# conanhujinming/flash_hash_join

Hardware: AMD Instinct MI355X
Metric: probe throughput (billion probes/sec), int64 keys, whole join (build + probe phases) per step (higher is better)
Workload: dtype int64

## Files before the change

flash_hash_join_amd/csrc/fj_host.h:

```cpp
#pragma once
#include "fj_internal.h"
#include "../../include/flashjoin.h"
#include "../../include/flashjoin_lab.h"

#include <algorithm>
#include <chrono>
#include <cstdarg>
#include <cstdio>
#include <cstdlib>
#include <cstring>
#include <condition_variable>
#include <functional>
#include <mutex>
#include <string>
#include <thread>
#include <vector>

struct StreamState;

namespace fjh {

int set_err(const char* fmt, ...);
fj_timings& last_timings();
#define HIPCHK(x)                                                                                          \
// ... 33 lines not shown
    u32 next_item;
    u32 next_emit_item;
    unsigned long long owner_counts[64], owner_cursors[64], owner_offsets[64];
    u32 pack_alloc, pack_seg, pack_err, rx_alloc;
    unsigned long long pack_used[64];
    unsigned long long pack_kept;
    u32 pack_xcd[8 * FJ_PF_COUNTERS];
    u32 bc_bounds[20];
};

enum Slot {
    W_POOL_K = 0, W_POOL_V, W_DIR, W_LIST, W_BCHUNKS, W_REL, W_BOFF, W_SEGOFF, W_TOFF, W_TILES, W_KINDS,
    W_SIDE_STRIDE = 2 * W_KINDS,
    W_PART_COUNT = 3 * W_SIDE_STRIDE, W_OUT_OFF, W_GT_KEYS, W_GT_VALS, W_GT_BLOOM, W_WG_COUNT,
    W_H_BK, W_H_BV, W_H_PK, W_H_OK, W_H_OV, W_ROWIDX, W_BKEYS, W_BBASE,
    W_PK_FI, W_PK_BKEYS, W_PK_OBASE,
    W_RX_REL, W_RX_LIST, W_RX_SEGOFF, W_RX_BCH, W_RX_BOFF, W_RX_TOFF, W_RX_TILES,
    W_SK_TILES_B, W_SK_TILES_P, W_SK_NT, W_PART_COUNT2, W_OUT_OFF2,
    W_MM_TILES,
    W_MM_PBITS,
    W_FULL_BITS,
    W_PAIR_WORDS,
    W_GR_PART, W_GR_BASE,
    W_NSLOTS
};

struct Buf { void* p = nullptr; size_t bytes = 0; };

enum Ev { E_START = 0, E_BUILD, E_PPART, E_JOIN, E_EMIT0, E_EMIT1, E_SB0, E_SB1, E_BF0, E_BF1, E_H0, E_H1, E_H2, E_PK0, E_NEV = E_PK0 + 8 };

struct BcastSources { const void* base = nullptr; int n = 0; uint64_t off[FJ_WIDE_MAXSRC] = {}, nkeys[FJ_WIDE_MAXSRC] = {}; };

struct Pending {
    enum Kind { LDS, HBM_TABLE, MANY, BCAST };
    bool valid = false;
    Kind kind = LDS;
    FjLdsJoinArgs lds{};
    FjGtArgs gt{};
    u32 nitems = 0, gt_grid = 0;
    u64 count = 0;
    bool has_second = false; FjLdsJoinArgs lds2{}; u32 nitems2 = 0; u64 count_main = 0; std::vector<u32> flagged;
    bool dups_main = false; std::vector<u32> sk_parts; int sk_bits = 0, sk_plan_bits = 0, sk_npass = 0;
    int mm_outer = 0; FjMmOuterArgs mm{}; u64 mm_P = 0, mm_u = 0, mm_r = 0;
    FjMmSweepArgs mm_sweep{}; u64 mm_u_main = 0; u64* mm_tile_off = nullptr; u64* mm_sweep_off = nullptr;
    bool mm_trivial = false; const u64* mm_pk = nullptr;
    bool has_dups = false;
    const u64* bk = nullptr; const u64* bv = nullptr; size_t nb = 0; int top_bits = 64;
    BcastSources src; const u32* toff = nullptr; size_t nb_total = 0;
};

struct SingleOut { u64* keys = nullptr; u64* vals = nullptr; size_t cap = 0; bool done = false; };

struct Plan { int bits = 0, npass = 0; int fan_log[4] = {0, 0, 0, 0}; int bloom_level = 0; };

struct Prepared {
    enum Form { EMPTY, LDS, HBM };
    bool valid = false;
    Form form = EMPTY;
    bool has_vals = false;
    int top_bits = 64, path = 0;
    Plan plan; u32 nparts = 0;
    size_t nb = 0; u64 g = 0;
    u64* keys = nullptr; u64* rows = nullptr; u64* vals = nullptr; void* aux = nullptr;
    u64 cap_mask = 0;
    size_t bytes = 0;
};

struct PassIter {
    int side = 0; bool has_vals = false; size_t n = 0; Plan plan; int used = 64; u32 parents = 1; u64 lbound = 0;
    u32 tile_chunks = 16; int i = 0;
    FjChunkSet prev{}; bool have_prev = false; const uint4* tiles = nullptr; const u32* ntiles = nullptr; const u32* toff = nullptr;
    FjChunkSet cs{}; u32 Gmax = 1, F = 1, appends = 1;
    size_t piece_rows = 0;
    int slot = 0, cs_base = 0;
    u32 item_tc_max = 0;
    bool want_items = false; u32 items_cap = 0; u32* part_count = nullptr; int part_count_slot = W_PART_COUNT;
    bool bloom_done = false; const FjChunkSet* bloom_build = nullptr;
    const u32* bloom_prebuilt = nullptr;
    unsigned long long* bloom_bucket_keys = nullptr;
    int save_level = 0; FjChunkSet saved{};
    u32* alloc_word = nullptr; u32* seg_word = nullptr; u32* err_word = nullptr;
    bool in_pk7 = false; u32 in_b0 = 0, in_top_shift = 0;
    bool vals_pos = false;
};

}

struct PackState {
    bool begun = false, deferred = false;
    u32 part_shift = 0;
    fjh::PassIter it;
    FjPackArgs args{};
    int nranks = 0;
};

struct StreamState {
    bool active = false;
    fjh::Plan plan; fjh::PassIter pit, bit; FjLdsJoinArgs ja{};
    int top_bits = 64, evc = 0;
    size_t np_bound = 0, np_seen = 0, nb_bound = 0, nb_seen = 0;
    u32 p_appends_left = 0, b_appends_left = 0;
    bool probe_done = false, build_done = false;
    const u64* flat_build = nullptr;
    const u64* flat_probe[64]; size_t flat_np[64]; u32 nflat = 0;
    std::vector<std::pair<const u64*, size_t>> bpieces, ppieces;
    bool shuffled = false; u32 b_lo = 0, nbk = 0, nbk_pad = 0;
    bool probe_prepared = true; u32 probe_appends = 0;
    bool with_vals = false;
};

struct BcastState {
    bool packed = false, probed = false;
    size_t nb_total = 0, nb = 0, np = 0;
    int pieces = 1, evc = 0;
    fjh::Plan plan; fjh::PassIter pit; FjLdsJoinArgs ja{};
    bool with_vals = false;
    fjh::BcastSources src;
};

struct fj_ctx {
    int device = 0;
    fjh::Buf bufs[fjh::W_NSLOTS];
    hipEvent_t ev[fjh::E_NEV];
    hipStream_t side = nullptr;
    fjh::Scalars* d_sc = nullptr;
    fjh::Scalars* h_sc = nullptr;
    fjh::Pending pend;
    fjh::Prepared prep;
    StreamState st;
    PackState pk;
    BcastState bc;
    hipEvent_t pk_ev = nullptr;
    unsigned long long* pk_h = nullptr;
    size_t ws_bytes = 0;
    u32 num_cus = 256;
    u32 reserve_cus = 0;
    void* stage[3] = {nullptr, nullptr, nullptr};
    size_t stage_bytes = 0;
    bool plan_in_flight = false;
    bool slot_dirty[fjh::W_NSLOTS] = {};
    std::recursive_mutex mu;
};

namespace fjh {

#define FJ_HOOK_LOOPBACK 1
#define FJ_HOOK_INJECT_FAIL 2
#define FJ_HOOK_SPLIT_ALWAYS 4
#define FJ_HOOK_ONE_COMM 8
#define FJ_HOOK_RESERVE_ALWAYS 16
#define FJ_HOOK_EMIT_TAGGED 32
#define FJ_HOOK_EMIT_RETRY_7TH 64
struct Options {
    size_t radix_threshold = 0; int scalar_hbm_table = 0; u32 persistent_min_items = 8192; u32 plan_target_keys = FJ_PART_TARGET_KEYS;
    int bloom_variant = 0, bloom_auto = 1, bloom_auto_max_hit_bp = 2300, mat_single_pass = 1;
    int join_wide = 2;
    u32 lab_hooks = 0;
    u32 join_items_target = 2048;
    int mm_heavy_keys = 0;
    int mm_heavy_outer = 0;
    Options();
};
Options& options();

int get_buf(fj_ctx* c, int slot, size_t bytes, void** out);
int get_zeroed_buf(fj_ctx* c, int slot, size_t bytes, void** out, hipStream_t s);
int plan_npass(int bits);
void plan_passes(Plan& p, bool extra_first);
Plan make_plan(size_t nb, int top_bits, bool want_bloom = false, u64 target_override = 0);
void pass_init(PassIter& it, int side, bool has_vals, size_t n, const Plan& plan, int top_bits);
u32 pass_groups(u64 chunks, u64 rows, u32 tile_chunks, u32 F);
int pass_prepare(fj_ctx* c, PassIter& it, u32 appends, hipStream_t s);
int pass_launch(fj_ctx* c, PassIter& it, const u64* keys, const u64* vals, size_t n, hipStream_t s, int* ev_cursor);
bool bloom_stage_follows(const PassIter& it, int level);
void join_item_geometry(u64 nparts, size_t np, u64 chunk_bound, u32* tc, u64* max_items);
bool wide_join_planned(bool materialize, size_t nb, size_t np_eff, int bits);
int level_finish(fj_ctx* c, PassIter& it, bool final_level, hipStream_t s);
int pass_complete(fj_ctx* c, PassIter& it, hipStream_t s);
int bloom_stage(fj_ctx* c, PassIter& it, hipStream_t s);
int run_passes(fj_ctx* c, PassIter& it, const u64* keys, const u64* vals, hipStream_t s, FjChunkSet* out, int* ev_cursor);
int clear_plan_scalars(fj_ctx* c, hipStream_t s);
void begin_plan(fj_ctx* c);
void end_plan(fj_ctx* c);
void drop_pending(fj_ctx* c);
int begin_step(fj_ctx* c, const char* who);
int read_scalars(fj_ctx* c, hipStream_t s);
float ev_ms(fj_ctx* c, int a, int b);
void plan_timings(fj_ctx* c, const Plan& plan, u64 partitions, int evc, fj_timings* t);
int pool_error();
int distinct_error();

enum ValueKind { KIND_UNSIGNED = 0, KIND_SIGNED = 1, KIND_FLOAT = 2 };
enum AggPlane { PLANE_COUNT = 0, PLANE_SUM = 1, PLANE_MIN = 2, PLANE_MAX = 3 };
u64 gt_capacity(size_t nb);
inline u32 gt_grid(u64 n) { const u64 rounds = (n + 1023) / 1024; return (u32)(rounds < 4096 ? (rounds ? rounds : 1) : 4096); }
int gt_open(fj_ctx* c, size_t nb, size_t val_words, hipStream_t s, FjGtArgs* a, u64** vals);
void gt_facts(fj_timings* t);
int gt_read(fj_ctx* c, hipStream_t s, fj_timings* t);
int gt_close(fj_ctx* c, hipStream_t s, fj_timings* t);
template <class F> int gt_fallback(fj_timings* t, F&& global_form) {
    fj_timings t2; memset(&t2, 0, sizeof t2); t2.sampled_hit_bp = -1;
    const int rc = global_form(&t2);
    t2.total_ms += t->total_ms; t2.fell_back = 1; *t = t2;
    return rc;
}
int kind_agg(int kind, int plane);

enum RelBeside { REL_KEYS_ONLY, REL_VALUES, REL_POSITIONS };
struct RelAttempt { Plan plan; FjChunkSet rel{}; u32 nparts = 0; };
int rel_open(fj_ctx* c, const u64* keys, RelBeside beside, const u64* vals, size_t n, int top_bits, u64 target, hipStream_t s,
             RelAttempt* r);
int rel_close(fj_ctx* c, const Plan& plan, u32 nparts, hipStream_t s, fj_timings* t);

int stamps_begin(unsigned long long** dbg, hipStream_t s);
int stamps_report(const char* label, const unsigned long long* dbg, u32 nitems, hipStream_t s);

int emit_pending(fj_ctx* c, u64* d_ok, u64* d_ov, size_t cap, hipStream_t s, fj_timings* t);
int radix_join_tail(fj_ctx* c, int materialize, FjLdsJoinArgs& ja, const Plan& plan, size_t np, const PassIter& pit, hipStream_t s,
                    fj_timings* t, int evc, u64* out_count, bool* lds_full, int top_bits, SingleOut* so = nullptr);

int join_outer(fj_ctx* c, int mode, bool use_radix, const u64* bk, const u64* bv, size_t nb, const u64* pk, size_t np, int top_bits,
               hipStream_t s, fj_timings* t, u64* out_count, u64* d_ok, u64* d_ov, bool rid = false);
int join_full(fj_ctx* c, bool use_radix, const u64* bk, const u64* bv, size_t nb, const u64* pk, size_t np, int top_bits,
              hipStream_t s, fj_timings* t, u64* out_counts, u64* d_ok, u64* d_ov, bool rid);

int join_probe_order(fj_ctx* c, bool use_radix, const u64* bk, const u64* bv, size_t nb, const u64* pk, size_t np, int top_bits,
                     hipStream_t s, fj_timings* t, u64* out_count, unsigned char* d_mask, u64* d_ov, bool rid);

void prepared_free(fj_ctx* c);
int prepared_retain(fj_ctx* c, bool use_radix, const u64* bk, const u64* bv, size_t nb, int top_bits, hipStream_t s, fj_timings* t);
int prepared_probe(fj_ctx* c, const u64* pk, size_t np, hipStream_t s, fj_timings* t, u64* out_count, unsigned char* d_mask, u64* d_ov, bool rid);
int prepared_group(fj_ctx* c, const u64* pk, const u64* pv, size_t np, hipStream_t s, fj_timings* t, u64* out_count, u64* d_cnt, u64* d_val,
                   int agg, bool accumulate);

int join_group(fj_ctx* c, bool use_radix, const u64* bk, size_t nb, const u64* pk, const u64* pv, size_t np, int top_bits,
               hipStream_t s, fj_timings* t, u64* out_count, u64* d_cnt, u64* d_sum, int agg);

int group_by(fj_ctx* c, bool use_radix, const u64* bk, const u64* bv, size_t nb, int top_bits, hipStream_t s, fj_timings* t,
             u64* out_count, u64* d_ok, u64* d_ov, size_t cap_out, int agg, bool rid, bool inv = false);
int group_by_all(fj_ctx* c, bool use_radix, const u64* bk, const u64* bv, size_t nb, int top_bits, hipStream_t s, fj_timings* t,
                 u64* out_count, u64* d_ok, u64* d_ov, size_t cap_out, int kind);
int group_by_arg(fj_ctx* c, bool use_radix, const u64* bk, const u64* bv, size_t nb, int top_bits, hipStream_t s, fj_timings* t,
                 u64* out_count, u64* d_ok, u64* d_ov, size_t cap_out, int kind, bool is_max);
int group_by_merge(fj_ctx* c, bool use_radix, const u64* bk, const u64* bv, size_t nb, int top_bits, hipStream_t s, fj_timings* t,
                   u64* out_count, u64* d_ok, u64* d_ov, size_t cap_out, int kind);

int group_by_pair(fj_ctx* c, bool use_radix, const u64* ka, const u64* kb, size_t nb, int top_bits, hipStream_t s, fj_timings* t,
                  u64* out_count, u64* d_ok, u64* d_ov, size_t cap_out);
int group_by_pair_agg(fj_ctx* c, bool use_radix, const u64* ka, const u64* kb, const u64* kv, size_t nb, int top_bits, hipStream_t s,
                      fj_timings* t, u64* out_count, u64* d_ok, u64* d_ov, size_t cap_out, int kind);

int group_rows(fj_ctx* c, bool use_radix, const u64* bk, size_t nb, int top_bits, hipStream_t s, fj_timings* t,
               u64* out_count, u64* d_ok, u64* d_ov, size_t cap_out);

int stream_open(fj_ctx* c, size_t nb_bound, int build_appends, size_t np_bound, int probe_appends, hipStream_t s, int top_bits,
                size_t probe_piece_rows = 0);
int stream_append_build(fj_ctx* c, const u64* d_bk, size_t n, hipStream_t s);
int stream_flush_build(fj_ctx* c, StreamState& st, hipStream_t s);
int stream_abort(fj_ctx* c);

int bcast_emit_launch(fj_ctx* c, const Pending& pd, u64* d_ok, u64* d_ov, hipStream_t s);
void drop_bcast_result_in(fj_ctx* c, const void* p, size_t bytes);

fj_ctx*& host_ctx();

}
```

flash_hash_join_amd/csrc/fj_internal.h:

```cpp
#pragma once
#include "fj_common.h"

#define FJ_ERR_POOL 1u
#define FJ_ERR_LDS_FULL 2u
#define FJ_STAT_DUPS 4u
#define FJ_STAT_RETRY 8u
#define FJ_STAT_EMIT_RETRY 16u
#define FJ_ERR_VARIANT 32u
#define FJ_BLOOM_HDR_MAGIC 0xB100F000u
#define FJ_STAT_TOOBIG 64u
#define FJ_ERR_OUTCAP 128u
#define FJ_ERR_PAIR_COLLISION 256u
#define FJ_ITEM_RETRY 0xFFFFFFFFu
#define FJ_ITEM_TOOBIG 0xFFFFFFFEu

struct FjPartArgs {
    const u64* in_keys;
    const u64* in_vals;
    const u32* in_list;
    const u32* in_dir;
    const uint4* in_tiles;
    const u32* in_ntiles;
    u64 n_flat;
    u32 parent0;
    u64* out_keys;
    u64* out_vals;
    u32* out_dir;
    u64* out_rel;
    u32* seg_off;
    u32* bchunks;
    u32* alloc;
    u32* seg_counter;
    u32 cap_chunks;
    u32 max_segs;
    u32* err;
    u32 shift;
    u32 fan_log;
    u32 side;
    u32 slab;
    u32 run_log;
    u32 in_pk7, in_b0, in_top_shift;
    u32 vals_pos;
};

struct FjChunkSet {
    u64* keys;
    u64* vals;
    u64 n_flat;
    u32* dir;
    u64* rel;
    u32* seg_off;
    u32* alloc;
    u32 cap;
    u32 nb;
    u32 fan_mask;
    u32 max_segs;
    u32* bchunks;
    u32* boff;
    u32* list;
    u32 run_log;
};

u32 fj_partition_lds_bytes(u32 fan_log, bool vals, int line_log);
u32 fj_partition_tile_chunks(u32 fan_log, bool vals);
hipError_t fj_launch_partition(const FjPartArgs& a, bool vals, int line_log, u32 grid, hipStream_t s);
hipError_t fj_launch_group(const FjChunkSet& cs, u32 tc, u32* toff, uint4* tiles, u32 max_tiles, u32* zero_tail, hipStream_t s);
hipError_t fj_launch_scan_u32_to_u64(const u32* in, u64* out, u32 n, hipStream_t s);
hipError_t fj_launch_dir_rank(u32* dir, u32 n, u32 b_lo, u32 nbk, u32 fan, u64* rel, u32* seg_off, u32* bchunks, u32* nalloc, hipStream_t s);

struct FjBloomArgs {
    const u64* pkeys;
    const u32* plist;
    const uint4* tiles;
    u64* out_keys; u32* out_dir; u64* out_rel;
    u32 cap_chunks;
    u32 pnb;
    const u32* toff;
    const u64* bkeys; const u32* blist; const u32* bboff;
    u32* seg_off; u32* bchunks; u32* alloc; u32* seg_counter;
    u32 max_segs;
    u32* err;
    unsigned long long* survivors;
    const u32* prebuilt;
    unsigned long long* bucket_keys;
};
u32 fj_bloom_tile_chunks();
u32 fj_bloom_waves_per_group();
u32 fj_bloom_slab_chunks();
hipError_t fj_launch_bloom_filter(const FjBloomArgs& a, u32 grid, int variant, hipStream_t s);
hipError_t fj_launch_bloom_export(const FjChunkSet& build, u32* out, u32 grid, int variant, hipStream_t s);
hipError_t fj_launch_flatten(const FjChunkSet& cs, const unsigned long long* bucket_keys, unsigned long long* base, u64* out, hipStream_t s);

struct FjPackArgs {
    const u64* keys; const u64* vals;
    const u32* list; const u32* boff;
    u32 nb, fan_log, nranks, wire7;
    uint4* fi;
    u32* fb;
    u32* bkeys;
    u32* obase;
    unsigned long long* used;
    unsigned char* dst_k[64]; u64* dst_v[64]; u32* dst_d[64];
};
hipError_t fj_launch_pack_plan(const FjPackArgs& a, hipStream_t s);
#define FJ_PF_COUNTERS 4u
#ifndef FJ_PFILT_BYTES
#define FJ_PFILT_BYTES 4096u
#endif
hipError_t fj_launch_part_filter_export(const FjChunkSet& build, u64* out, u32 grid, hipStream_t s);
hipError_t fj_launch_part_filter_inplace(const FjChunkSet& cs, const u64* filters, u32 part_shift, unsigned long long* kept, u32* next_of_xcd , u32 grid, hipStream_t s);
hipError_t fj_launch_part_filter_sample(const u64* raw, u64 n, u64 stride, const u64* filters, u32 part_shift, unsigned long long* kept, hipStream_t s);
hipError_t fj_launch_pack_squeeze(const FjPackArgs& a, u32 grid, hipStream_t s);


hipError_t fj_set_max_lds_once(const void* fn, u32 bytes);

struct FjLdsJoinArgs {
    FjChunkSet build, probe;
    u32 nparts;
    u32 nsplit;
    const uint4* items;
    const u32* nitems_dev;
    u32 items_cap;
    u32* part_count;
    unsigned long long* total;
    u32* err;
    const u64* out_off;
    u64* out_keys;
    u64* out_vals;
    unsigned long long* out_cursor;
    u64 out_capacity;
    u32 retry_only;
    u32 mark_toobig;
    u32 want_dups;
    u32 dedup;
    const u64* orig_vals;
    u32 avg_build_keys;
    unsigned long long* dbg;
    u32 dbg_flags;
    u32 row_ids;
};
hipError_t fj_launch_lds_join(const FjLdsJoinArgs& a, bool materialize, hipStream_t s, u32* next_item = nullptr,
                              u32 persistent_min_items = 8192);
hipError_t fj_launch_emit_single(const FjLdsJoinArgs& a, hipStream_t s, u32* next_item);
#define FJ_WIDE_MAXSRC 16u
struct FjWideArgs {
    const u32* toff; u32 part_lo, part_hi;
    const unsigned char* base; u32 nsrc, bits, mid_bytes;
    u32 group_log;
    u32 max_units;
    u32 pmask;
    u64 offs_off[FJ_WIDE_MAXSRC], lo_off[FJ_WIDE_MAXSRC], mid_off[FJ_WIDE_MAXSRC];
};
hipError_t fj_launch_count_join_wide(const FjLdsJoinArgs& a, const FjWideArgs& w, bool dense, u32 grid, hipStream_t s);
static inline u32 fj_wide_pmask(int bits, int top_bits) { return bits <= 0 ? 0u : (bits >= 32 ? 0xFFFFFFFFu : ((1u << bits) - 1u) << (top_bits - 32 - bits)); }

hipError_t fj_launch_lds_join_retry(const FjLdsJoinArgs& a, hipStream_t s);
hipError_t fj_launch_lds_emit_retry(const FjLdsJoinArgs& a, hipStream_t s, bool only_marked = true);

hipError_t fj_launch_sample_hits(const FjChunkSet& build, const u64* pk, u64 np, u32 nsamples, u32 shift32, u32 pmask,
                                 unsigned long long* hits, hipStream_t s);

#define FJ_MM_INNER 0
#define FJ_MM_LEFT 1
#define FJ_MM_FULL 2
struct FjMmOuterArgs {
    u32* miss_count;
    unsigned long long* miss_total;
    const u64* miss_off;
    u64 miss_base;
    u64* bits;
    unsigned long long* marked;
    u64* pbits;
};
hipError_t fj_launch_mm_join(const FjLdsJoinArgs& a, bool materialize, hipStream_t s, int outer = FJ_MM_INNER, const FjMmOuterArgs* oa = nullptr);
#define FJ_MM_TILE_CHUNKS 16u
hipError_t fj_launch_mm_tile_join(const FjLdsJoinArgs& a, bool materialize, hipStream_t s, int outer = FJ_MM_INNER, const FjMmOuterArgs* oa = nullptr);
struct FjMmSweepArgs {
    FjChunkSet probe;
    const uint4* items; u32 nitems;
    const u64* pbits;
    u32* miss_count;
    unsigned long long* miss_total;
    const u64* miss_off;
    u64 miss_base;
    u64* out_keys; u64* out_vals;
    u32 row_ids;
};
hipError_t fj_launch_mm_miss_sweep(const FjMmSweepArgs& w, bool materialize, hipStream_t s);

struct FjGtArgs {
    u64* tkeys; u64* tvals; u32* bloom;
    u64 cap_mask;
    u32* flags;
    u64* empty_val;
    const u64* bk; const u64* bv; u64 nb;
    const u64* pk; u64 np;
    u32* wg_count;
    unsigned long long* total;
    const u64* out_off;
    u64* out_keys; u64* out_vals;
    u32 row_ids;
    u32* matched;
};
hipError_t fj_launch_gt_build(const FjGtArgs& a, hipStream_t s);
hipError_t fj_launch_gt_probe(const FjGtArgs& a, bool materialize, u32 grid, hipStream_t s);

hipError_t fj_launch_owner_hist(const u64* keys, u64 n, u32 nranks, unsigned long long* counts, hipStream_t s);
hipError_t fj_launch_owner_scatter(const u64* keys, const u64* vals, u64 n, u32 nranks,
                                   const unsigned long long* offsets, unsigned long long* cursors,
                                   u64* out_keys, u64* out_vals, hipStream_t s);

hipError_t fj_launch_iota(u64* out, u64 n, hipStream_t s);
hipError_t fj_launch_gen_build(u64* keys, u64* vals, u64 first, u64 n, hipStream_t s);
hipError_t fj_launch_gen_probe(u64* keys, u64 first, u64 n, u64 build_total, u64 seed, u32 hit_bp,
                               unsigned long long* expected_hits, hipStream_t s);

__host__ __device__ inline u32 fj_owner_of_w1(u32 w1, u32 nranks) { return ((w1 >> 16) * nranks) >> 16; }

#define FJ_OJ_LEFT 0
#define FJ_OJ_ANTI 1
#define FJ_OJ_LEFT_FIRST 2
struct FjOjCursor { u32 hit, miss; u64 hit_base, miss_base; };
// ... 97 lines not shown
```

flash_hash_join_amd/csrc/fj_join.hip:

```cpp
#include "fj_lds_table_dev.h"

namespace {

constexpr u32 S = FJ_LDS_SLOTS;

struct JoinHdr {
    u32 cnt, has_empty, cursor, claimed, full, ovf;
    u32 pad[2];
    u64 empty_val;
    u64 pad2;
};

constexpr u32 NGRP = S / FJ_LDS_GROUP;
__device__ __forceinline__ void lds_groups(u64 key, u32& g1, u32& g2) {
    const u32 w = FJ_HW2(key);
    g1 = (w & (NGRP - 1)) * FJ_LDS_GROUP;
    g2 = ((w >> 11) & (NGRP - 1)) * FJ_LDS_GROUP;
}

__device__ __forceinline__ u32 lds_tag(u32 w2) { const u32 t = w2 >> 24; return t ? t : 1u; }
__device__ __forceinline__ u32 tag_zero_bytes(u32 t) {
    const u32 y = (t & 0x7F7F7F7Fu) + 0x7F7F7F7Fu;
    return ~(y | t | 0x7F7F7F7Fu);
}
// ... 41 lines not shown
        if (step == 1) { hdr->ovf = 1; g = g1; }
        if ((step & 31u) == 31u && *reinterpret_cast<volatile u32*>(&hdr->full)) return false;
        g = (g + 1) & (NGRP - 1);
    }
    hdr->full = 1;
    return false;
}



template <bool MAT, int NK>
__device__ __forceinline__ void lds_probe(const u64* __restrict__ tkeys, const u32* __restrict__ ttags, const u64 (&k)[NK],
                                          const u64 (&okm)[NK], u64 he, bool ovf, u32 lane, u64 (&hitm)[NK], u32 (&where)[NK]) {
    u32 g1[NK], g2[NK], z1[NK], z2[NK];
#pragma unroll
    for (int i = 0; i < NK; ++i) {
        const u32 w = FJ_HW2(k[i]);
        g1[i] = (w & (NGRP - 1)) * FJ_LDS_GROUP;
        g2[i] = ((w >> 11) & (NGRP - 1)) * FJ_LDS_GROUP;
        const u32 pat = lds_tag(w) * 0x01010101u;
        z1[i] = tag_matches(ttags[g1[i] / FJ_LDS_GROUP], pat);
        z2[i] = tag_matches(ttags[g2[i] / FJ_LDS_GROUP], pat);
    }
    u32 cand[NK];
    u64 kc[NK];
#pragma unroll
    for (int i = 0; i < NK; ++i) {
        const bool in1 = z1[i] != 0;
        const u32 z = in1 ? z1[i] : z2[i];
        cand[i] = (in1 ? g1[i] : g2[i]) + ((u32)__builtin_ctz(z | 0x80000000u) >> 3);
        kc[i] = tkeys[cand[i]];
    }
    __builtin_amdgcn_sched_barrier(0);
#pragma unroll
    for (int i = 0; i < NK; ++i) {
        const bool in1 = z1[i] != 0;
        const bool first = ((z1[i] | z2[i]) != 0) & (kc[i] == k[i]);
        const u64 hit1 = __ballot(first);
        const u64 ise = __ballot(k[i] == FJ_EMPTY_KEY);
        if (MAT) where[i] = cand[i];
        const u32 r1 = in1 ? (z1[i] & (z1[i] - 1)) : 0u, r2 = in1 ? z2[i] : (z2[i] & (z2[i] - 1));
        const u64 more = __ballot(!first && (r1 | r2) != 0) & okm[i] & ~ise;
        u64 hit = hit1;
        if (more) {
            bool found = false;
            if ((more >> lane) & 1ull) {
                u32 ra = r1, rb = r2;
                while (ra | rb) {
                    const bool ina = ra != 0;
                    const u32 zz = ina ? ra : rb;
                    const u32 c = (ina ? g1[i] : g2[i]) + ((u32)__builtin_ctz(zz) >> 3);
                    if (tkeys[c] == k[i]) { found = true; if (MAT) where[i] = c; break; }
                    if (ina) ra &= ra - 1; else rb &= rb - 1;
                }
            }
            hit |= __ballot(found);
        }
        if (ovf) {
            const u64 undec = okm[i] & ~ise & ~hit;
            bool found = false;
            if ((undec >> lane) & 1ull) {
                u32 g = g1[i] / FJ_LDS_GROUP;
                for (u32 step = 0; step < NGRP; ++step) {
                    g = (g + 1) & (NGRP - 1);
                    const u32 t = ttags[g];
                    u32 m = tag_matches(t, lds_tag(FJ_HW2(k[i])) * 0x01010101u);
                    while (m) {
                        const u32 c = g * FJ_LDS_GROUP + ((u32)__builtin_ctz(m) >> 3);
                        if (tkeys[c] == k[i]) { found = true; if (MAT) where[i] = c; break; }
                        m &= m - 1;
                    }
                    if (found || tag_zero_bytes(t)) break;
                }
            }
            hit |= __ballot(found);
        }
        hitm[i] = okm[i] & ((hit & ~ise) | (ise & he));
    }
}

constexpr u32 JB_META = 128;
constexpr u32 JP_META = 512;

template <bool MAT, int NT, bool LIST, bool RID = false>
__global__ __launch_bounds__(NT, 4) void fj_lds_join_kernel(FjLdsJoinArgs a) {
    static_assert(!RID || MAT, "row ids are written by the emitting pass");
    extern __shared__ __attribute__((aligned(16))) unsigned char smem[];
    JoinHdr* hdr = reinterpret_cast<JoinHdr*>(smem);
    u64* tkeys = reinterpret_cast<u64*>(smem + sizeof(JoinHdr));
    u64* tvals = tkeys + S;
    u32* ttags = reinterpret_cast<u32*>(tkeys + (MAT ? 2 * S : S));
    u32* gcnt = ttags + S / 4;
    u32* pm = gcnt + NGRP / 2;
    u32* bm = pm + JP_META;
    const u32 tid = threadIdx.x, lane = tid & 63;
#define FJ_STAMP(i) do { if (a.dbg && tid == 0 && blockIdx.x < 4096) a.dbg[blockIdx.x * 8 + (i)] = __builtin_amdgcn_s_memrealtime(); } while (0)
    FJ_STAMP(0);
    const u32 item = blockIdx.x;
    u32 p, b0 = 0, nbc, p0 = 0, s_lo, s_hi;
    if (a.items) {
        if (item >= *a.nitems_dev) return;
        const uint4 it = a.items[item];
        p = it.z; s_lo = it.x; s_hi = it.x + it.y;
    } else {
        const u32 slice = item % a.nsplit;
        p = item / a.nsplit;
        const u32 npc = (u32)((a.probe.n_flat + FJ_CHUNK - 1) >> FJ_CHUNK_LOG);
        s_lo = (u32)(((u64)slice * npc) / a.nsplit); s_hi = (u32)(((u64)(slice + 1) * npc) / a.nsplit);
    }
    if (a.build.list) { b0 = a.build.boff[p]; nbc = a.build.boff[p + 1] - b0; }
    else nbc = (u32)((a.build.n_flat + FJ_CHUNK - 1) >> FJ_CHUNK_LOG);
    if (nbc == 0 || s_lo >= s_hi) {
        if (!MAT && tid == 0) a.part_count[item] = 0;
        return;
    }
    if (MAT && a.part_count[item] == 0) return;
    if (a.retry_only && a.part_count[item] != FJ_ITEM_RETRY) return;

    constexpr u32 CPL = NT / (FJ_CHUNK / 2);
    constexpr u32 CPR = 4 * CPL;
    constexpr u32 BKPT = 4096 / NT;
    auto load_round = [&](u32 r, u32 nbatch, u64 (&kk)[8], u32& okm) {
        okm = 0;
#pragma unroll
        for (int u = 0; u < 4; ++u) {
            const u32 c = r * CPR + u * CPL + tid / (FJ_CHUNK / 2), off = (tid % (FJ_CHUNK / 2)) * 2;
            if (LIST) {
                const u32 e = pm[c < nbatch ? c : nbatch - 1], cnt = c < nbatch ? FJ_LIST_CNT(e) : 0;
                const u64x2 q = *reinterpret_cast<const u64x2*>(a.probe.keys + (u64)FJ_LIST_ID(e) * FJ_CHUNK + off);
                kk[2 * u] = q.x; kk[2 * u + 1] = q.y;
                okm |= ((off < cnt ? 1u : 0u) | (off + 1 < cnt ? 2u : 0u)) << (2 * u);
                continue;
            }
            kk[2 * u] = 0; kk[2 * u + 1] = 0;
            if (c < nbatch) {
                const u32 e = pm[c], cnt = FJ_LIST_CNT(e);
                const u64 base = (u64)FJ_LIST_ID(e) * FJ_CHUNK + off;
                if (off + 1 < cnt) {
                    const u64x2 q = *reinterpret_cast<const u64x2*>(a.probe.keys + base);
                    kk[2 * u] = a.probe.list ? q.x : fj_key_mix(q.x); kk[2 * u + 1] = a.probe.list ? q.y : fj_key_mix(q.y); okm |= 3u << (2 * u);
                } else if (off < cnt) {
                    kk[2 * u] = a.probe.list ? a.probe.keys[base] : fj_key_mix(a.probe.keys[base]); okm |= 1u << (2 * u);
                }
            }
        }
    };
    u64 bk[BKPT], bv[BKPT];
    u32 bok = 0;
    auto load_build = [&](u32 c0, u32 nbb) {
        bok = 0;
#pragma unroll
        for (u32 j = 0; j < BKPT; ++j) {
            const u32 kidx = j * NT + tid, c = c0 + (kidx >> FJ_CHUNK_LOG), off = kidx & (FJ_CHUNK - 1);
            if (LIST) {
                const u32 e = bm[c < nbb ? c : nbb - 1];
                const u64 src = (u64)FJ_LIST_ID(e) * FJ_CHUNK + off;
                bk[j] = a.build.keys[src];
                bv[j] = MAT ? a.build.vals[src] : 0;
                bok |= (c < nbb && off < FJ_LIST_CNT(e) ? 1u : 0u) << j;
                continue;
            }
            bk[j] = 0; bv[j] = 0;
            if (c < nbb) {
                const u32 e = bm[c];
                if (off < FJ_LIST_CNT(e)) {
                    const u64 src = (u64)FJ_LIST_ID(e) * FJ_CHUNK + off;
                    bk[j] = a.build.list ? a.build.keys[src] : fj_key_mix(a.build.keys[src]);
                    if (MAT) bv[j] = (RID && !a.build.vals) ? src : a.build.vals[src];
                    bok |= 1u << j;
                }
            }
        }
    };

    u32 nbatch = (s_hi - s_lo) < JP_META ? (s_hi - s_lo) : JP_META;
    for (u32 i = tid; i < nbatch; i += NT) pm[i] = fj_chunk_entry(a.probe, p0 + s_lo + i);
    u32 nbb = nbc < JB_META ? nbc : JB_META;
    if (tid < nbb) bm[tid] = fj_chunk_entry(a.build, b0 + tid);
    for (u32 i = tid; i < S / 4 + NGRP / 2; i += NT) ttags[i] = 0;
    const bool dedup = MAT && a.dedup != 0;
    if (dedup) for (u32 i = tid; i < S; i += NT) tvals[i] = ~0ull;
    if (tid == 0) { hdr->cnt = 0; hdr->has_empty = 0; hdr->cursor = 0; hdr->claimed = 0; hdr->full = 0; hdr->ovf = 0; hdr->empty_val = (MAT && a.dedup) ? ~0ull : 0ull; }
    __syncthreads();
    FJ_STAMP(1);
    u64 ka[8], kb[8];
    u32 oka = 0, okb = 0;
    u32 nrounds = (nbatch + CPR - 1) / CPR;
    load_build(0, nbb);
    load_round(0, nbatch, ka, oka);
    if (nrounds > 1) load_round(1, nbatch, kb, okb);

    u32 claimed = 0;
    for (u32 bb = 0; bb < nbc; bb += JB_META) {
        if (bb) {
            nbb = (nbc - bb) < JB_META ? (nbc - bb) : JB_META;
            __syncthreads();
            if (tid < nbb) bm[tid] = fj_chunk_entry(a.build, b0 + bb + tid);
            __syncthreads();
        }
        for (u32 c0 = 0; c0 < nbb; c0 += 16) {
            if (*reinterpret_cast<volatile u32*>(&hdr->full)) break;
            if (bb | c0) load_build(c0, nbb);
#pragma unroll
            for (u32 j = 0; j < BKPT; ++j) {
                if (bok & (1u << j)) {
                    const u64 key = bk[j];
                    if (key == FJ_EMPTY_KEY) {
                        hdr->has_empty = 1;
                        if (MAT) {
                            if (dedup) atomicMin((unsigned long long*)&hdr->empty_val, (unsigned long long)bv[j]); else hdr->empty_val = bv[j];
                        }
                    } else if (!(a.dbg_flags & 2u)) {
                        claimed += lds_insert<MAT>(tkeys, tvals, ttags, gcnt, hdr, key, bv[j], dedup) ? 1u : 0u;
                    }
                }
            }
        }
    }
    FJ_STAMP(2);
    claimed = fj_wave_sum(claimed);
    if (lane == 0 && claimed) atomicAdd(&hdr->claimed, claimed);
    __syncthreads();
    FJ_STAMP(3);
    if (hdr->full || hdr->claimed > S - 64) {
        if (tid == 0) {
            if (!MAT && a.mark_toobig) { atomicOr(a.err, FJ_STAT_TOOBIG); a.part_count[item] = FJ_ITEM_TOOBIG; }
            else { atomicOr(a.err, FJ_ERR_LDS_FULL); if (!MAT) a.part_count[item] = 0; }
        }
        return;
    }
    if (!MAT && a.want_dups && tid == 0) atomicOr(a.err, FJ_STAT_DUPS);
    if (dedup) {
        const bool ovf0 = hdr->ovf != 0;
        for (u32 sl = tid; sl < S; sl += NT) {
            if (reinterpret_cast<const unsigned char*>(ttags)[sl] == 0) continue;
            const u64 key = tkeys[sl];
            const u32 w = FJ_HW2(key), pat = lds_tag(w) * 0x01010101u;
            u32 g = w & (NGRP - 1);
            const u32 g2 = (w >> 11) & (NGRP - 1);
            u64 best = tvals[sl];
            for (u32 step = 0; step < NGRP + 2; ++step) {
                const u32 t = ttags[g];
                u32 m = tag_matches(t, pat);
                while (m) { const u32 c = g * FJ_LDS_GROUP + ((u32)__builtin_ctz(m) >> 3); if (c != sl && tkeys[c] == key) { const u64 o = tvals[c]; best = o < best ? o : best; } m &= m - 1; }
                if (step == 0) { g = g2; continue; }
                if (!ovf0) break;
                if (step == 1) g = w & (NGRP - 1);
                else if (tag_zero_bytes(t)) break;
                g = (g + 1) & (NGRP - 1);
            }
            atomicMin((unsigned long long*)&tvals[sl], (unsigned long long)best);
        }
        __syncthreads();
        if (!RID) {
            for (u32 sl = tid; sl < S; sl += NT)
                if (reinterpret_cast<const unsigned char*>(ttags)[sl] != 0) tvals[sl] = a.orig_vals[tvals[sl]];
            if (tid == 0 && hdr->has_empty) hdr->empty_val = a.orig_vals[hdr->empty_val];
            __syncthreads();
        }
    }
    const bool has_empty = hdr->has_empty != 0;
    const u64 obase = MAT ? a.out_off[item] : 0;

    u32 wave_hits = 0;
    const u64 he = has_empty ? ~0ull : 0ull;
    const bool ovf = hdr->ovf != 0;
    for (u32 pb = s_lo; pb < s_hi; pb += JP_META) {
        if (pb != s_lo) {
            nbatch = (s_hi - pb) < JP_META ? (s_hi - pb) : JP_META;
            __syncthreads();
            for (u32 i = tid; i < nbatch; i += NT) pm[i] = fj_chunk_entry(a.probe, p0 + pb + i);
            __syncthreads();
            nrounds = (nbatch + CPR - 1) / CPR;
            load_round(0, nbatch, ka, oka);
            if (nrounds > 1) load_round(1, nbatch, kb, okb);
        }
        for (u32 r = 0; r < nrounds; ++r) {
            u64 k[8];
#pragma unroll
            for (int i = 0; i < 8; ++i) { k[i] = ka[i]; ka[i] = kb[i]; }
            const u32 okm = oka;
            oka = okb;
            if (r + 2 < nrounds) load_round(r + 2, nbatch, kb, okb);
#pragma unroll
            for (int hgrp = 0; hgrp < 2; ++hgrp) {
                const u64 k2[4] = {k[4 * hgrp], k[4 * hgrp + 1], k[4 * hgrp + 2], k[4 * hgrp + 3]};
                u64 ok2[4], hitm[4];
                u32 where[4];
#pragma unroll
                for (int i = 0; i < 4; ++i) ok2[i] = __ballot((okm >> (4 * hgrp + i)) & 1u);
                if (a.dbg_flags & 1u) { hitm[0] = __ballot((k2[0] ^ k2[1]) & 1ull); hitm[1] = hitm[2] = hitm[3] = 0; where[0] = where[1] = where[2] = where[3] = 0; }
                else lds_probe<MAT, 4>(tkeys, ttags, k2, ok2, he, ovf, lane, hitm, where);
                if (MAT) {
                    const u32 n0 = (u32)__popcll(hitm[0]), n1 = (u32)__popcll(hitm[1]), n2 = (u32)__popcll(hitm[2]), n3 = (u32)__popcll(hitm[3]);
                    if (n0 + n1 + n2 + n3) {
                        u32 wb = 0;
                        if (lane == 0) wb = atomicAdd(&hdr->cursor, n0 + n1 + n2 + n3);
                        wb = (u32)__builtin_amdgcn_readfirstlane((int)wb);
                        const u32 off[4] = {0u, n0, n0 + n1, n0 + n1 + n2};
#pragma unroll
                        for (int i = 0; i < 4; ++i) {
                            const u64 m = hitm[i];
                            if ((m >> lane) & 1ull) {
                                const u64 o = obase + wb + off[i] + (u32)__popcll(m & ((1ull << lane) - 1ull));
                                if (a.dbg_flags & 4u) continue;
                                if (RID) {
                                    const u32 ks = 4u * (u32)hgrp + (u32)i;
                                    const u32 c = r * CPR + (ks >> 1) * CPL + tid / (FJ_CHUNK / 2), off = (tid % (FJ_CHUNK / 2)) * 2 + (ks & 1u);
                                    const u64 src = (u64)FJ_LIST_ID(pm[c]) * FJ_CHUNK + off;
                                    a.out_keys[o] = a.probe.vals ? a.probe.vals[src] : src;
                                } else {
                                    a.out_keys[o] = fj_key_unmix(k2[i]);
                                }
                                a.out_vals[o] = k2[i] == FJ_EMPTY_KEY ? hdr->empty_val : tvals[where[i]];
                            }
                        }
                    }
                } else {
#pragma unroll
                    for (int i = 0; i < 4; ++i) wave_hits += (u32)__popcll(hitm[i]);
                }
            }
        }
    }
    FJ_STAMP(4);
    if (!MAT) {
        if (lane == 0 && wave_hits) atomicAdd(&hdr->cnt, wave_hits);
        __syncthreads();
        FJ_STAMP(5);
        if (tid == 0) {
            a.part_count[item] = hdr->cnt;
            if (hdr->cnt) atomicAdd(a.total, (unsigned long long)hdr->cnt);
        }
    } else if (a.dbg) {
        __syncthreads();
        FJ_STAMP(5);
    }
}

constexpr u32 CK_STASH = 32, CK_MAXIT = 48;
struct CkHdr { u32 cnt, has_empty, nstash, full, dups, empties, novf, pad1; u64 pad[1]; u64 stash[CK_STASH]; };

template <typename Hdr>
__device__ __forceinline__ void cuckoo_insert(u64* __restrict__ tkeys, Hdr* hdr, u64 key) {
    u32 w = FJ_HW2(key);
    u32 l1 = w & (S - 1), l2 = (w >> 13) & (S - 1);
    if (tkeys[l1] == key || tkeys[l2] == key) { hdr->dups = 1; return; }
    u32 loc = l1;
#pragma unroll 1
    for (u32 it = 0; it < CK_MAXIT; ++it) {
        const u64 old = atomicExch((unsigned long long*)&tkeys[loc], (unsigned long long)key);
        if (old == key) hdr->dups = 1;
        if (old == FJ_EMPTY_KEY || old == key) return;
        key = old;
        w = FJ_HW2(key);
        l1 = w & (S - 1); l2 = (w >> 13) & (S - 1);
        loc = loc == l1 ? l2 : l1;
    }
    const u32 sidx = atomicAdd(&hdr->nstash, 1u);
    if (sidx < CK_STASH) hdr->stash[sidx] = key; else hdr->full = 1;
}

constexpr u32 CK_OVF = 1024;
template <typename Hdr>
__device__ __forceinline__ void cuckoo_claim(u64* __restrict__ tkeys, u32* __restrict__ bits, u64* __restrict__ ovf, Hdr* hdr, u64 key) {
    const u32 w = FJ_HW2(key), l1 = w & (S - 1), l2 = (w >> 13) & (S - 1);
    const u32 o1 = atomicOr(&bits[l1 >> 5], 1u << (l1 & 31));
    if (!((o1 >> (l1 & 31)) & 1u)) { tkeys[l1] = key; return; }
    const u32 o2 = atomicOr(&bits[l2 >> 5], 1u << (l2 & 31));
    if (!((o2 >> (l2 & 31)) & 1u)) { tkeys[l2] = key; return; }
    if (tkeys[l1] == key || tkeys[l2] == key) { hdr->dups = 1; return; }
    const u32 i = atomicAdd(&hdr->novf, 1u);
    if (i < CK_OVF) ovf[i] = key; else hdr->full = 1;
}
template <int NT, typename Hdr>
__device__ __forceinline__ void cuckoo_finish(u64* __restrict__ tkeys, const u64* __restrict__ ovf, Hdr* hdr, u32 tid) {
    const u32 n = hdr->novf < CK_OVF ? hdr->novf : CK_OVF;
    for (u32 i = tid; i < n; i += NT) cuckoo_insert(tkeys, hdr, ovf[i]);
}

template <int NT, bool LIST>
__global__ __launch_bounds__(NT, 4) void fj_count_join_kernel(FjLdsJoinArgs a) {
    extern __shared__ __attribute__((aligned(16))) unsigned char smem[];
    CkHdr* hdr = reinterpret_cast<CkHdr*>(smem);
    u64* tkeys = reinterpret_cast<u64*>(smem + sizeof(CkHdr));
    u32* pm = reinterpret_cast<u32*>(tkeys + S);
    u32* bm = pm + JP_META;
    u32* bits = bm + JB_META;
    u64* ovf = reinterpret_cast<u64*>(bits + S / 32);
    const u32 tid = threadIdx.x, lane = tid & 63;
    FJ_STAMP(0);
    const u32 item = blockIdx.x;
    u32 p, b0 = 0, nbc, p0 = 0, s_lo, s_hi;
    if (a.items) {
        if (item >= *a.nitems_dev) return;
        const uint4 it = a.items[item];
        p = it.z; s_lo = it.x; s_hi = it.x + it.y;
    } else {
        const u32 slice = item % a.nsplit;
        p = item / a.nsplit;
        const u32 npc = (u32)((a.probe.n_flat + FJ_CHUNK - 1) >> FJ_CHUNK_LOG);
        s_lo = (u32)(((u64)slice * npc) / a.nsplit); s_hi = (u32)(((u64)(slice + 1) * npc) / a.nsplit);
    }
    if (a.build.list) { b0 = a.build.boff[p]; nbc = a.build.boff[p + 1] - b0; }
    else nbc = (u32)((a.build.n_flat + FJ_CHUNK - 1) >> FJ_CHUNK_LOG);
    if (nbc == 0 || s_lo >= s_hi) {
        if (tid == 0) a.part_count[item] = 0;
        return;
    }
    constexpr u32 CPL = NT / (FJ_CHUNK / 2), CPR = 4 * CPL, BKPT = 4096 / NT;
    constexpr bool plist = LIST, blist = LIST;
    auto load_round = [&](u32 r, u32 nbatch, u64 (&kk)[8], u32& okm) {
        okm = 0;
#pragma unroll
        for (int u = 0; u < 4; ++u) {
            const u32 c = r * CPR + u * CPL + tid / (FJ_CHUNK / 2), off = (tid % (FJ_CHUNK / 2)) * 2;
            if (plist) {
                const u32 e = pm[c < nbatch ? c : nbatch - 1], cnt = c < nbatch ? FJ_LIST_CNT(e) : 0;
                const u64x2 q = *reinterpret_cast<const u64x2*>(a.probe.keys + (u64)FJ_LIST_ID(e) * FJ_CHUNK + off);
                kk[2 * u] = q.x; kk[2 * u + 1] = q.y;
                okm |= ((off < cnt ? 1u : 0u) | (off + 1 < cnt ? 2u : 0u)) << (2 * u);
                continue;
            }
            kk[2 * u] = 0; kk[2 * u + 1] = 0;
            if (c < nbatch) {
                const u32 e = pm[c], cnt = FJ_LIST_CNT(e);
                const u64 base = (u64)FJ_LIST_ID(e) * FJ_CHUNK + off;
                if (off + 1 < cnt) {
                    const u64x2 q = *reinterpret_cast<const u64x2*>(a.probe.keys + base);
                    kk[2 * u] = a.probe.list ? q.x : fj_key_mix(q.x); kk[2 * u + 1] = a.probe.list ? q.y : fj_key_mix(q.y); okm |= 3u << (2 * u);
                } else if (off < cnt) {
                    kk[2 * u] = a.probe.list ? a.probe.keys[base] : fj_key_mix(a.probe.keys[base]); okm |= 1u << (2 * u);
                }
            }
        }
    };
    u64 bk[BKPT];
    u32 bok = 0;
    auto load_build = [&](u32 c0, u32 nbb) {
        bok = 0;
#pragma unroll
        for (u32 j = 0; j < BKPT; ++j) {
            const u32 kidx = j * NT + tid, c = c0 + (kidx >> FJ_CHUNK_LOG), off = kidx & (FJ_CHUNK - 1);
            if (blist) {
                const u32 e = bm[c < nbb ? c : nbb - 1];
                bk[j] = a.build.keys[(u64)FJ_LIST_ID(e) * FJ_CHUNK + off];
                bok |= (c < nbb && off < FJ_LIST_CNT(e) ? 1u : 0u) << j;
                continue;
            }
            bk[j] = 0;
            if (c < nbb) {
                const u32 e = bm[c];
                if (off < FJ_LIST_CNT(e)) { const u64 raw = a.build.keys[(u64)FJ_LIST_ID(e) * FJ_CHUNK + off]; bk[j] = a.build.list ? raw : fj_key_mix(raw); bok |= 1u << j; }
            }
        }
    };

    u32 nbatch = (s_hi - s_lo) < JP_META ? (s_hi - s_lo) : JP_META;
    for (u32 i = tid; i < nbatch; i += NT) pm[i] = fj_chunk_entry(a.probe, p0 + s_lo + i);
    u32 nbb = nbc < JB_META ? nbc : JB_META;
    if (tid < nbb) bm[tid] = fj_chunk_entry(a.build, b0 + tid);
    for (u32 i = tid; i < S; i += NT) tkeys[i] = FJ_EMPTY_KEY;
    if (tid < S / 32) bits[tid] = 0;
    if (tid == 0) { hdr->cnt = 0; hdr->has_empty = 0; hdr->nstash = 0; hdr->full = 0; hdr->dups = 0; hdr->empties = 0; hdr->novf = 0; }
    __syncthreads();
    FJ_STAMP(1);
    u64 ka[8], kb[8];
    u32 oka = 0, okb = 0;
    u32 nrounds = (nbatch + CPR - 1) / CPR;
    load_build(0, nbb);
    load_round(0, nbatch, ka, oka);
    if (nrounds > 1) load_round(1, nbatch, kb, okb);

    for (u32 bb = 0; bb < nbc; bb += JB_META) {
        if (bb) {
            nbb = (nbc - bb) < JB_META ? (nbc - bb) : JB_META;
            __syncthreads();
            if (tid < nbb) bm[tid] = fj_chunk_entry(a.build, b0 + bb + tid);
            __syncthreads();
        }
        for (u32 c0 = 0; c0 < nbb; c0 += 16) {
            if (bb | c0) load_build(c0, nbb);
#pragma unroll
            for (u32 j = 0; j < BKPT; ++j) {
                if (bok & (1u << j)) {
                    if (bk[j] == FJ_EMPTY_KEY) { hdr->has_empty = 1; if (a.want_dups && atomicAdd(&hdr->empties, 1u) > 0) hdr->dups = 1; }
                    else if (!(a.dbg_flags & 2u)) cuckoo_claim(tkeys, bits, ovf, hdr, bk[j]);
                }
            }
        }
    }
    FJ_STAMP(2);
    __syncthreads();
    cuckoo_finish<NT>(tkeys, ovf, hdr, tid);
    __syncthreads();
    FJ_STAMP(3);
    if (hdr->full) {
        if (tid == 0) { atomicOr(a.err, FJ_STAT_RETRY); a.part_count[item] = FJ_ITEM_RETRY; }
        return;
    }
    const u64 he = hdr->has_empty ? ~0ull : 0ull;
    const u32 nstash = hdr->nstash < CK_STASH ? hdr->nstash : CK_STASH;
    if (a.want_dups) {
        for (u32 sl = tid; sl < S; sl += NT) {
            const u64 key = tkeys[sl];
            if (key == FJ_EMPTY_KEY) continue;
            const u32 w = FJ_HW2(key), l1 = w & (S - 1), l2 = (w >> 13) & (S - 1);
            const u32 other = sl == l1 ? l2 : l1;
            if (other != sl && tkeys[other] == key) hdr->dups = 1;
            for (u32 si = 0; si < nstash; ++si) if (hdr->stash[si] == key) hdr->dups = 1;
        }
        for (u32 si = tid; si < nstash; si += NT)
            for (u32 sj = si + 1; sj < nstash; ++sj) if (hdr->stash[si] == hdr->stash[sj]) hdr->dups = 1;
        __syncthreads();
        if (tid == 0 && hdr->dups) atomicOr(a.err, FJ_STAT_DUPS);
    }

    u32 wave_hits = 0;
    for (u32 pb = s_lo; pb < s_hi; pb += JP_META) {
        if (pb != s_lo) {
            nbatch = (s_hi - pb) < JP_META ? (s_hi - pb) : JP_META;
            __syncthreads();
            for (u32 i = tid; i < nbatch; i += NT) pm[i] = fj_chunk_entry(a.probe, p0 + pb + i);
            __syncthreads();
            nrounds = (nbatch + CPR - 1) / CPR;
            load_round(0, nbatch, ka, oka);
            if (nrounds > 1) load_round(1, nbatch, kb, okb);
        }
        for (u32 r = 0; r < nrounds; ++r) {
            u64 k[8];
#pragma unroll
            for (int i = 0; i < 8; ++i) { k[i] = ka[i]; ka[i] = kb[i]; }
            const u32 okm = oka;
            oka = okb;
            if (r + 2 < nrounds) load_round(r + 2, nbatch, kb, okb);
            if (a.dbg_flags & 1u) { wave_hits += (u32)__popcll(__ballot((k[0] ^ k[7]) & 1ull)); continue; }
            u64 c1[8], c2[8];
#pragma unroll
            for (int i = 0; i < 8; ++i) {
                const u32 w = FJ_HW2(k[i]);
                c1[i] = tkeys[w & (S - 1)];
                c2[i] = tkeys[(w >> 13) & (S - 1)];
            }
            __builtin_amdgcn_sched_barrier(0);
#pragma unroll
            for (int i = 0; i < 8; ++i) {
                u64 hit = __ballot(c1[i] == k[i]) | __ballot(c2[i] == k[i]);
                if (nstash) {
                    bool f = false;
                    for (u32 si = 0; si < nstash; ++si) f |= hdr->stash[si] == k[i];
                    hit |= __ballot(f);
                }
                const u64 ise = __ballot(k[i] == FJ_EMPTY_KEY);
                const u64 ok = __ballot((okm >> i) & 1u);
                wave_hits += (u32)__popcll(ok & ((hit & ~ise) | (ise & he)));
            }
        }
    }
    FJ_STAMP(4);
    if (lane == 0 && wave_hits) atomicAdd(&hdr->cnt, wave_hits);
    __syncthreads();
    FJ_STAMP(5);
    if (tid == 0) {
        a.part_count[item] = hdr->cnt;
        if (hdr->cnt) atomicAdd(a.total, (unsigned long long)hdr->cnt);
    }
}

template <int NT>
__global__ __launch_bounds__(NT, 4) void fj_count_join_persistent(FjLdsJoinArgs a, u32* __restrict__ next_item) {
    extern __shared__ __attribute__((aligned(16))) unsigned char smem[];
    CkHdr* hdr = reinterpret_cast<CkHdr*>(smem);
    u64* tkeys = reinterpret_cast<u64*>(smem + sizeof(CkHdr));
    u32* pm0 = reinterpret_cast<u32*>(tkeys + S);
    u32* bm0 = pm0 + 2 * JP_META;
    u32* s_next = bm0 + 2 * JB_META;
    u32* bits = s_next + 4;
    u64* ovf = reinterpret_cast<u64*>(bits + S / 32);
    const u32 tid = threadIdx.x, lane = tid & 63;
    const u32 nitems = *a.nitems_dev;
    constexpr u32 CPL = NT / (FJ_CHUNK / 2), CPR = 4 * CPL, BKPT = 4096 / NT;
    static_assert(JP_META <= NT && JB_META <= NT, "one staged list entry per thread");

    struct Desc { u32 item, b0, nbc, p0, s_lo, s_hi; };
    auto describe = [&](u32 item) -> Desc {
        Desc d; d.item = item; d.b0 = 0; d.nbc = 0; d.p0 = 0; d.s_lo = 0; d.s_hi = 0;
        if (item >= nitems) return d;
        const uint4 it = a.items[item];
        d.b0 = a.build.boff[it.z]; d.nbc = a.build.boff[it.z + 1] - d.b0;
        d.p0 = 0; d.s_lo = it.x; d.s_hi = it.x + it.y;
        return d;
    };
    auto live = [&](const Desc& d) { return d.item < nitems && d.nbc > 0 && d.s_lo < d.s_hi; };

    u64 bk[BKPT];
    u32 bok = 0;
    auto load_build = [&](const u32* bm, u32 c0, u32 nbb) {
        bok = 0;
#pragma unroll
        for (u32 j = 0; j < BKPT; ++j) {
            const u32 kidx = j * NT + tid, c = c0 + (kidx >> FJ_CHUNK_LOG), off = kidx & (FJ_CHUNK - 1);
            const u32 e = bm[c < nbb ? c : nbb - 1];
            bk[j] = a.build.keys[(u64)FJ_LIST_ID(e) * FJ_CHUNK + off];
            bok |= (c < nbb && off < FJ_LIST_CNT(e) ? 1u : 0u) << j;
        }
    };
    auto load_round = [&](const u32* pm, u32 r, u32 nbatch, u64 (&kk)[8], u32& okm) {
        okm = 0;
#pragma unroll
        for (int u = 0; u < 4; ++u) {
            const u32 c = r * CPR + u * CPL + tid / (FJ_CHUNK / 2), off = (tid % (FJ_CHUNK / 2)) * 2;
            const u32 e = pm[c < nbatch ? c : nbatch - 1], cnt = c < nbatch ? FJ_LIST_CNT(e) : 0;
            const u64x2 q = *reinterpret_cast<const u64x2*>(a.probe.keys + (u64)FJ_LIST_ID(e) * FJ_CHUNK + off);
            kk[2 * u] = q.x; kk[2 * u + 1] = q.y;
            okm |= ((off < cnt ? 1u : 0u) | (off + 1 < cnt ? 2u : 0u)) << (2 * u);
        }
    };
    auto reset_table = [&]() {
        for (u32 i = tid; i < S; i += NT) tkeys[i] = FJ_EMPTY_KEY;
        if (tid < S / 32) bits[tid] = 0;
        if (tid == 0) { hdr->cnt = 0; hdr->has_empty = 0; hdr->nstash = 0; hdr->full = 0; hdr->dups = 0; hdr->empties = 0; hdr->novf = 0; }
    };

    Desc d = describe(blockIdx.x);
    if (d.item >= nitems) return;
    u32 buf = 0;
    {
        const bool lv = live(d);
        const u32 nb0 = (d.s_hi - d.s_lo) < JP_META ? (d.s_hi - d.s_lo) : JP_META;
        if (lv && tid < nb0) pm0[tid] = a.probe.list[d.p0 + d.s_lo + tid];
        const u32 nbb0 = d.nbc < JB_META ? d.nbc : JB_META;
        if (lv && tid < nbb0) bm0[tid] = a.build.list[d.b0 + tid];
        reset_table();
        if (tid == 0) s_next[0] = atomicAdd(next_item, 1u) + gridDim.x;
        __syncthreads();
        if (lv) load_build(bm0, 0, nbb0);
    }

    for (;;) {
        u32* pm = pm0 + buf * JP_META; u32* bm = bm0 + buf * JB_META;
        u32* pmn = pm0 + (buf ^ 1) * JP_META; u32* bmn = bm0 + (buf ^ 1) * JB_META;
        const bool lv = live(d);
        u64 ka[8], kb[8];
        u32 oka = 0, okb = 0;
        u32 nbatch = (d.s_hi - d.s_lo) < JP_META ? (d.s_hi - d.s_lo) : JP_META;
        u32 nrounds = (nbatch + CPR - 1) / CPR;
        if (lv) {
            load_round(pm, 0, nbatch, ka, oka);
            if (nrounds > 1) load_round(pm, 1, nbatch, kb, okb);
            u32 nbb = d.nbc < JB_META ? d.nbc : JB_META;
            for (u32 bb = 0; bb < d.nbc; bb += JB_META) {
                if (bb) {
                    nbb = (d.nbc - bb) < JB_META ? (d.nbc - bb) : JB_META;
                    __syncthreads();
                    if (tid < nbb) bm[tid] = a.build.list[d.b0 + bb + tid];
                    __syncthreads();
                }
                for (u32 c0 = 0; c0 < nbb; c0 += 16) {
                    if (bb | c0) load_build(bm, c0, nbb);
#pragma unroll
                    for (u32 j = 0; j < BKPT; ++j) {
                        if (bok & (1u << j)) {
                            if (bk[j] == FJ_EMPTY_KEY) { hdr->has_empty = 1; if (a.want_dups && atomicAdd(&hdr->empties, 1u) > 0) hdr->dups = 1; }
                            else cuckoo_claim(tkeys, bits, ovf, hdr, bk[j]);
                        }
                    }
                }
            }
        }
        __syncthreads();
        if (lv) cuckoo_finish<NT>(tkeys, ovf, hdr, tid);
        __syncthreads();
        const Desc dn = describe(__builtin_amdgcn_readfirstlane(s_next[buf]));
        const bool lvn = live(dn);
        const u32 nbn = (dn.s_hi - dn.s_lo) < JP_META ? (dn.s_hi - dn.s_lo) : JP_META;
        const u32 nbbn = dn.nbc < JB_META ? dn.nbc : JB_META;
        u32 mp = 0, mb = 0;
        if (lvn && tid < nbn) mp = a.probe.list[dn.p0 + dn.s_lo + tid];
        if (lvn && tid < nbbn) mb = a.build.list[dn.b0 + tid];
        bool parked = false;
        auto park = [&]() {
            if (tid < nbn) pmn[tid] = mp;
            if (tid < nbbn) bmn[tid] = mb;
            if (tid == 0) s_next[buf ^ 1] = atomicAdd(next_item, 1u) + gridDim.x;
            parked = true;
        };

        u32 wave_hits = 0;
        bool full = false;
        if (lv) {
            full = hdr->full != 0;
            const u64 he = hdr->has_empty ? ~0ull : 0ull;
            const u32 nstash = hdr->nstash < CK_STASH ? hdr->nstash : CK_STASH;
            if (a.want_dups && !full) {
                for (u32 sl = tid; sl < S; sl += NT) {
                    const u64 key = tkeys[sl];
                    if (key == FJ_EMPTY_KEY) continue;
                    const u32 w = FJ_HW2(key), l1 = w & (S - 1), l2 = (w >> 13) & (S - 1);
                    const u32 other = sl == l1 ? l2 : l1;
                    if (other != sl && tkeys[other] == key) hdr->dups = 1;
                    for (u32 si = 0; si < nstash; ++si) if (hdr->stash[si] == key) hdr->dups = 1;
                }
                for (u32 si = tid; si < nstash; si += NT)
                    for (u32 sj = si + 1; sj < nstash; ++sj) if (hdr->stash[si] == hdr->stash[sj]) hdr->dups = 1;
                __syncthreads();
                if (tid == 0 && hdr->dups) atomicOr(a.err, FJ_STAT_DUPS);
            }
            if (!full) for (u32 pb = d.s_lo; pb < d.s_hi; pb += JP_META) {
                if (pb != d.s_lo) {
                    nbatch = (d.s_hi - pb) < JP_META ? (d.s_hi - pb) : JP_META;
                    __syncthreads();
                    if (tid < nbatch) pm[tid] = a.probe.list[d.p0 + pb + tid];
                    __syncthreads();
                    nrounds = (nbatch + CPR - 1) / CPR;
                    load_round(pm, 0, nbatch, ka, oka);
                    if (nrounds > 1) load_round(pm, 1, nbatch, kb, okb);
                }
                for (u32 r = 0; r < nrounds; ++r) {
                    u64 k[8];
#pragma unroll
                    for (int i = 0; i < 8; ++i) { k[i] = ka[i]; ka[i] = kb[i]; }
                    const u32 okm = oka;
                    oka = okb;
                    if (r + 2 < nrounds) load_round(pm, r + 2, nbatch, kb, okb);
#pragma unroll
                    for (int h = 0; h < 8; h += 4) {
                        u64 c1[4], c2[4];
#pragma unroll
                        for (int i = 0; i < 4; ++i) {
                            const u32 w = FJ_HW2(k[h + i]);
                            c1[i] = tkeys[w & (S - 1)];
                            c2[i] = tkeys[(w >> 13) & (S - 1)];
                        }
                        __builtin_amdgcn_sched_barrier(0);
#pragma unroll
                        for (int i = 0; i < 4; ++i) {
                            u64 hit = __ballot(c1[i] == k[h + i]) | __ballot(c2[i] == k[h + i]);
                            if (nstash) {
                                bool f = false;
                                for (u32 si = 0; si < nstash; ++si) f |= hdr->stash[si] == k[h + i];
                                hit |= __ballot(f);
                            }
                            const u64 ise = __ballot(k[h + i] == FJ_EMPTY_KEY);
                            const u64 ok = __ballot((okm >> (h + i)) & 1u);
                            wave_hits += (u32)__popcll(ok & ((hit & ~ise) | (ise & he)));
                        }
                    }
                    if (!parked) park();
                }
            }
        }
        if (!parked) park();
        if (lane == 0 && wave_hits) atomicAdd(&hdr->cnt, wave_hits);
        __syncthreads();
        if (lvn) load_build(bmn, 0, nbbn); else bok = 0;
        if (tid == 0) {
            const u32 cnt = (lv && !full) ? hdr->cnt : 0u;
            if (full) atomicOr(a.err, FJ_STAT_RETRY);
            a.part_count[d.item] = full ? FJ_ITEM_RETRY : cnt;
            if (cnt) atomicAdd(a.total, (unsigned long long)cnt);
        }
        if (dn.item >= nitems) break;
        __syncthreads();
        reset_table();
        __syncthreads();
        d = dn; buf ^= 1;
    }
}

struct EkHdr { u32 has_empty, nstash, full, dups, cursor, novf, cur2[2]; u64 empty_val; u64 gb2[2]; u64 pad; u64 stash[CK_STASH]; u64 stash_val[CK_STASH]; };

template <int NT, bool DEDUP, bool SINGLE = false, bool RID = false>
__global__ __launch_bounds__(NT, 4) void fj_emit_join_persistent(FjLdsJoinArgs a, u32* __restrict__ next_item) {
    static_assert(!(SINGLE && DEDUP), "the single-pass form serves unique build keys");
    extern __shared__ __attribute__((aligned(16))) unsigned char smem[];
    EkHdr* hdr = reinterpret_cast<EkHdr*>(smem);
    u64* tkeys = reinterpret_cast<u64*>(smem + sizeof(EkHdr));
    u64* tvals = tkeys + S;
    u32* pm0 = reinterpret_cast<u32*>(tvals + S);
    u32* bm0 = pm0 + 2 * JP_META;
    u32* s_next = bm0 + 2 * JB_META;
    u32* bits = s_next + 4;
    u64* ovf = reinterpret_cast<u64*>(bits + S / 32);
    u32 tid = threadIdx.x;
    const u32 lane = tid & 63, wave_s = (u32)__builtin_amdgcn_readfirstlane((int)(threadIdx.x >> 6));
    auto fresh_tid = [&]() -> u32 {
        u32 t;
        asm volatile("v_mbcnt_lo_u32_b32 %0, -1, 0\n\tv_mbcnt_hi_u32_b32 %0, -1, %0\n\tv_lshl_add_u32 %0, %1, 6, %0" : "=&v"(t) : "s"(wave_s));
        return t;
    };
    const u32 nitems = *a.nitems_dev;
    constexpr u32 CPL = NT / (FJ_CHUNK / 2), CPR = 4 * CPL, BKPT = 4096 / NT;
    static_assert(JP_META <= NT && JB_META <= NT, "one staged list entry per thread");

    struct Desc { u32 item, b0, nbc, s_lo, s_hi, cnt; };
    auto describe = [&](u32 item) -> Desc {
        Desc d; d.item = item; d.b0 = 0; d.nbc = 0; d.s_lo = 0; d.s_hi = 0; d.cnt = 0;
        if (item >= nitems) return d;
        const uint4 it = a.items[item];
        d.b0 = a.build.boff[it.z]; d.nbc = a.build.boff[it.z + 1] - d.b0;
        d.s_lo = it.x; d.s_hi = it.x + it.y;
        d.cnt = SINGLE ? 1u : a.part_count[item];
        return d;
    };
    auto live = [&](const Desc& d) { return d.item < nitems && d.nbc > 0 && d.s_lo < d.s_hi && d.cnt != 0; };

// ... 737 lines not shown
            const u64 idx = t * T + ((u64)i * NT + tid) * 2;
            dr[2 * i] = dr[2 * i + 1] = 0xFFFFFFFFu;
            if (idx + 1 < n) {
                const u64x2 q = *reinterpret_cast<const u64x2*>(keys + idx);
                k[2 * i] = q.x; k[2 * i + 1] = q.y;
                if (HAS_VALS) { const u64x2 w = *reinterpret_cast<const u64x2*>(vals + idx); v[2 * i] = w.x; v[2 * i + 1] = w.y; }
            } else if (idx < n) {
                k[2 * i] = keys[idx];
                if (HAS_VALS) v[2 * i] = vals[idx];
            }
#pragma unroll
            for (u32 h = 0; h < 2; ++h) {
                const bool ok = idx + h < n;
                const u32 d = ok ? fj_owner_of_w1(fj_hash_w1(k[2 * i + h]), nranks) : none;
                const u64 m = fj_match_any(d, nbits);
                const u32 leader = (u32)__builtin_ctzll(m), ln = tid & 63;
                u32 base = 0;
                if (ok && ln == leader) base = atomicAdd(&hist[d], (u32)__popcll(m));
                base = __shfl(base, leader, 64);
                if (ok) dr[2 * i + h] = (d << 16) | (base + (u32)__popcll(m & ((1ull << ln) - 1ull)));
            }
        }
        __syncthreads();
        if (tid == 0) {
            u32 run = 0;
            for (u32 d = 0; d < nranks; ++d) { toff[d] = run; run += hist[d]; }
            toff[nranks] = run;
        }
        if (tid < nranks && hist[tid])
            gbase[tid] = offsets[tid] + atomicAdd(&cursors[tid], (unsigned long long)hist[tid]);
        __syncthreads();
#pragma unroll
        for (u32 i = 0; i < KPT; ++i) {
            if (dr[i] != 0xFFFFFFFFu) {
                const u32 s = toff[dr[i] >> 16] + (dr[i] & 0xFFFFu);
                sk[s] = k[i];
                if (HAS_VALS) sv[s] = v[i];
            }
        }
        __syncthreads();
        const u32 total = toff[nranks];
        for (u32 e = tid; e < total; e += NT) {
            u32 d = 0;
            while (e >= toff[d + 1]) ++d;
            const u64 o = gbase[d] + (e - toff[d]);
            out_keys[o] = sk[e];
            if (HAS_VALS) out_vals[o] = sv[e];
        }
        __syncthreads();
    }
}

__global__ void fj_iota_kernel(u64* __restrict__ out, u64 n) {
    const u64 stride = (u64)gridDim.x * blockDim.x;
    for (u64 i = (u64)blockIdx.x * blockDim.x + threadIdx.x; i < n; i += stride) out[i] = i;
}
__global__ void fj_gen_build_kernel(u64* __restrict__ keys, u64* __restrict__ vals, u64 first, u64 n) {
    const u64 stride = (u64)gridDim.x * blockDim.x;
    for (u64 i = (u64)blockIdx.x * blockDim.x + threadIdx.x; i < n; i += stride) {
        keys[i] = (first + i + 1) * FJ_GOLDEN;
        vals[i] = first + i;
    }
}
__global__ void fj_gen_probe_kernel(u64* __restrict__ keys, u64 first, u64 n, u64 B, u64 seed, u32 hit_bp,
                                    unsigned long long* __restrict__ expected) {
    const u64 stride = (u64)gridDim.x * blockDim.x;
    u32 hits = 0;
    for (u64 i = (u64)blockIdx.x * blockDim.x + threadIdx.x; i < n; i += stride) {
        const u64 j = first + i;
        const u64 r = 1 + fj_mix(seed, j) % B;
        const bool hit = (fj_mix(seed ^ 1ull, j) % 10000ull) < hit_bp;
        keys[i] = (r + (hit ? 0ull : B)) * FJ_GOLDEN;
        hits += hit ? 1u : 0u;
    }
    hits = fj_wave_sum(hits);
    if ((threadIdx.x & 63) == 0 && hits) atomicAdd(expected, (unsigned long long)hits);
}

}

hipError_t fj_launch_lds_join(const FjLdsJoinArgs& a, bool materialize, hipStream_t s, u32* next_item, u32 persistent_min_items) {
    const u32 nb = a.items ? a.items_cap : a.nparts * a.nsplit;
    if (materialize) {
        if (a.row_ids && (!a.dedup || a.orig_vals)) return hipErrorInvalidValue;
        if (a.build.list && a.probe.list && a.items && next_item && nb >= persistent_min_items && !a.dbg && !(a.dbg_flags & ~8u)) {
            const u32 ldsp = sizeof(EkHdr) + 2 * S * 8 + 2 * (JP_META + JB_META) * 4 + 16 + S / 8 + CK_OVF * 8;
            auto pk = a.row_ids ? fj_emit_join_persistent<1024, true, false, true>
                                : a.dedup ? fj_emit_join_persistent<1024, true> : fj_emit_join_persistent<1024, false>;
            hipError_t e = fj_set_max_lds_once(reinterpret_cast<const void*>(pk), ldsp);
            if (e != hipSuccess) return e;
            const u32 grid = nb < 256 ? nb : 256;
            hipLaunchKernelGGL(pk, dim3(grid), dim3(1024), ldsp, s, a, next_item);
            return hipGetLastError();
        }
        if (a.row_ids) return fj_launch_lds_emit_retry(a, s, false);
        const u32 lds = sizeof(JoinHdr) + 2 * S * 8 + S + S / 2 + (JP_META + JB_META) * 4;
        auto kern = (a.build.list && a.probe.list) ? fj_lds_join_kernel<true, 1024, true> : fj_lds_join_kernel<true, 1024, false>;
        hipError_t e = fj_set_max_lds_once(reinterpret_cast<const void*>(kern), lds);
        if (e != hipSuccess) return e;
        hipLaunchKernelGGL(kern, dim3(nb), dim3(1024), lds, s, a);
    } else {
        const u32 lds = sizeof(CkHdr) + S * 8 + (JP_META + JB_META) * 4 + S / 8 + CK_OVF * 8;
        const bool lists = a.build.list && a.probe.list;
        if (lists && next_item && nb >= persistent_min_items && !a.dbg && !a.dbg_flags) {
            const u32 ldsp = sizeof(CkHdr) + S * 8 + 2 * (JP_META + JB_META) * 4 + 16 + S / 8 + CK_OVF * 8;
            auto pk = fj_count_join_persistent<512>;
            hipError_t e = fj_set_max_lds_once(reinterpret_cast<const void*>(pk), ldsp);
            if (e != hipSuccess) return e;
            const u32 grid = nb < 512 ? nb : 512;
            hipLaunchKernelGGL(pk, dim3(grid), dim3(512), ldsp, s, a, next_item);
            return hipGetLastError();
        }
        auto kern = lists ? fj_count_join_kernel<512, true> : fj_count_join_kernel<512, false>;
        hipError_t e = fj_set_max_lds_once(reinterpret_cast<const void*>(kern), lds);
        if (e != hipSuccess) return e;
        hipLaunchKernelGGL(kern, dim3(nb), dim3(512), lds, s, a);
    }
    return hipGetLastError();
}

hipError_t fj_launch_emit_single(const FjLdsJoinArgs& a, hipStream_t s, u32* next_item) {
    if (!a.build.list || !a.probe.list || !a.items || !next_item || !a.out_cursor || a.dedup || !a.build.vals || (a.row_ids && !a.probe.vals))
        return hipErrorInvalidValue;
    const u32 nb = a.items_cap;
    const u32 ldsp = sizeof(EkHdr) + 2 * S * 8 + 2 * (JP_META + JB_META) * 4 + 16 + S / 8 + CK_OVF * 8;
    auto pk = a.row_ids ? fj_emit_join_persistent<1024, false, true, true> : fj_emit_join_persistent<1024, false, true>;
    hipError_t e = fj_set_max_lds_once(reinterpret_cast<const void*>(pk), ldsp);
    if (e != hipSuccess) return e;
    hipLaunchKernelGGL(pk, dim3(nb < 256 ? nb : 256), dim3(1024), ldsp, s, a, next_item);
    return hipGetLastError();
}

hipError_t fj_launch_lds_emit_retry(const FjLdsJoinArgs& a0, hipStream_t s, bool only_marked) {
    FjLdsJoinArgs a = a0;
    a.retry_only = only_marked ? 1u : 0u;
    const u32 nb = a.items ? a.items_cap : a.nparts * a.nsplit;
    const u32 lds = sizeof(JoinHdr) + 2 * S * 8 + S + S / 2 + (JP_META + JB_META) * 4;
    if (a.row_ids && (!a.dedup || a.orig_vals)) return hipErrorInvalidValue;
    const bool lists = a.build.list && a.probe.list;
    auto kern = a.row_ids ? (lists ? fj_lds_join_kernel<true, 1024, true, true> : fj_lds_join_kernel<true, 1024, false, true>)
                          : (lists ? fj_lds_join_kernel<true, 1024, true> : fj_lds_join_kernel<true, 1024, false>);
    hipError_t e = fj_set_max_lds_once(reinterpret_cast<const void*>(kern), lds);
    if (e != hipSuccess) return e;
    hipLaunchKernelGGL(kern, dim3(nb), dim3(1024), lds, s, a);
    return hipGetLastError();
}

hipError_t fj_launch_lds_join_retry(const FjLdsJoinArgs& a0, hipStream_t s) {
    FjLdsJoinArgs a = a0;
    a.retry_only = 1;
    const u32 nb = a.items ? a.items_cap : a.nparts * a.nsplit;
    const u32 lds = sizeof(JoinHdr) + S * 8 + S + S / 2 + (JP_META + JB_META) * 4;
    auto kern = (a.build.list && a.probe.list) ? fj_lds_join_kernel<false, 1024, true> : fj_lds_join_kernel<false, 1024, false>;
    hipError_t e = fj_set_max_lds_once(reinterpret_cast<const void*>(kern), lds);
    if (e != hipSuccess) return e;
    hipLaunchKernelGGL(kern, dim3(nb), dim3(1024), lds, s, a);
    return hipGetLastError();
}

hipError_t fj_launch_sample_hits(const FjChunkSet& build, const u64* pk, u64 np, u32 nsamples, u32 shift32, u32 pmask,
                                 unsigned long long* hits, hipStream_t s) {
    if (!build.list || np < nsamples) return hipErrorInvalidValue;
    hipLaunchKernelGGL(fj_sample_hits_kernel, dim3((nsamples * 64 + 255) / 256), dim3(256), 0, s, build, pk, np, nsamples, shift32, pmask, hits);
    return hipGetLastError();
}

hipError_t fj_launch_gt_build(const FjGtArgs& a, hipStream_t s) {
    if (a.nb == 0) return hipSuccess;
    u64 blocks = (a.nb + 255) / 256;
    if (blocks > 4096) blocks = 4096;
    hipLaunchKernelGGL(fj_gt_build_kernel, dim3((u32)blocks), dim3(256), 0, s, a);
    return hipGetLastError();
}

hipError_t fj_launch_gt_probe(const FjGtArgs& a, bool materialize, u32 grid, hipStream_t s) {
    const bool bloom = a.bloom != nullptr;
    if (materialize && a.row_ids) {
        if (bloom) return hipErrorInvalidValue;
        hipLaunchKernelGGL((fj_gt_probe_kernel<true, false, true>), dim3(grid), dim3(256), 0, s, a);
    } else if (materialize) {
        if (bloom) hipLaunchKernelGGL((fj_gt_probe_kernel<true, true>), dim3(grid), dim3(256), 0, s, a);
        else hipLaunchKernelGGL((fj_gt_probe_kernel<true, false>), dim3(grid), dim3(256), 0, s, a);
    } else {
        if (bloom) hipLaunchKernelGGL((fj_gt_probe_kernel<false, true>), dim3(grid), dim3(256), 0, s, a);
        else hipLaunchKernelGGL((fj_gt_probe_kernel<false, false>), dim3(grid), dim3(256), 0, s, a);
    }
    return hipGetLastError();
}

hipError_t fj_launch_gt_build_first(const FjGtArgs& a, bool vals, hipStream_t s) {
    if (a.nb == 0) return hipSuccess;
    if (vals && !a.tvals) return hipErrorInvalidValue;
    u64 blocks = (a.nb + 255) / 256;
    if (blocks > 4096) blocks = 4096;
    if (vals) hipLaunchKernelGGL(fj_gt_build_first_kernel<true>, dim3((u32)blocks), dim3(256), 0, s, a);
    else hipLaunchKernelGGL(fj_gt_build_first_kernel<false>, dim3((u32)blocks), dim3(256), 0, s, a);
    return hipGetLastError();
}

hipError_t fj_launch_gt_outer_probe(const FjGtArgs& a, int mode, unsigned long long* miss_cursor, u64 out_capacity, hipStream_t s) {
    if (a.np == 0) return hipSuccess;
    if (!a.out_keys || !miss_cursor || (mode != FJ_OJ_ANTI && (!a.out_vals || !a.tvals || (!a.bv && !a.row_ids)))) return hipErrorInvalidValue;
    const u64 rounds = (a.np + 4095) / 4096;
    const u32 grid = (u32)(rounds < 2048 ? rounds : 2048);
    if (a.matched) {
        if (mode != FJ_OJ_LEFT) return hipErrorInvalidValue;
        if (a.row_ids) hipLaunchKernelGGL((fj_gt_outer_probe_kernel<FJ_OJ_LEFT, true, true>), dim3(grid), dim3(1024), 0, s, a, miss_cursor, out_capacity);
        else hipLaunchKernelGGL((fj_gt_outer_probe_kernel<FJ_OJ_LEFT, false, true>), dim3(grid), dim3(1024), 0, s, a, miss_cursor, out_capacity);
        return hipGetLastError();
    }
    if (a.row_ids) {
        if (mode == FJ_OJ_ANTI) hipLaunchKernelGGL((fj_gt_outer_probe_kernel<FJ_OJ_ANTI, true>), dim3(grid), dim3(1024), 0, s, a, miss_cursor, out_capacity);
        else hipLaunchKernelGGL((fj_gt_outer_probe_kernel<FJ_OJ_LEFT, true>), dim3(grid), dim3(1024), 0, s, a, miss_cursor, out_capacity);
        return hipGetLastError();
    }
    if (mode == FJ_OJ_ANTI) hipLaunchKernelGGL(fj_gt_outer_probe_kernel<FJ_OJ_ANTI>, dim3(grid), dim3(1024), 0, s, a, miss_cursor, out_capacity);
    else hipLaunchKernelGGL(fj_gt_outer_probe_kernel<FJ_OJ_LEFT>, dim3(grid), dim3(1024), 0, s, a, miss_cursor, out_capacity);
    return hipGetLastError();
}

hipError_t fj_launch_gt_probe_order(const FjGtArgs& a, unsigned long long* miss_total, unsigned char* mask, hipStream_t s) {
    if (a.np == 0) return hipSuccess;
    const bool vals = a.out_vals != nullptr;
    if (!miss_total || !a.total || (!vals && !mask) || (vals && (!a.tvals || (!a.bv && !a.row_ids))) || (a.row_ids && !vals)) return hipErrorInvalidValue;
    const u64 rounds = (a.np + 1023) / 1024;
    const u32 grid = (u32)(rounds < 4096 ? rounds : 4096);
    void (*kern)(FjGtArgs, unsigned long long*, unsigned char*);
    if (!vals) kern = fj_gt_probe_order_kernel<false, false, true>;
    else if (a.row_ids) kern = mask ? fj_gt_probe_order_kernel<true, true, true> : fj_gt_probe_order_kernel<true, true, false>;
    else kern = mask ? fj_gt_probe_order_kernel<false, true, true> : fj_gt_probe_order_kernel<false, true, false>;
    hipLaunchKernelGGL(kern, dim3(grid), dim3(1024), 0, s, a, miss_total, mask);
    return hipGetLastError();
}

hipError_t fj_launch_gt_full_sweep(const FjGtArgs& a, u64 base, u64 out_capacity, unsigned long long* cursor, u32* err, hipStream_t s) {
    if (a.nb == 0) return hipSuccess;
// ... 44 lines not shown
```

flash_hash_join_amd/csrc/fj_joins.hip:

```cpp
#include "fj_host.h"
#include "fj_entry.h"

namespace fjh {

static int skew_side(fj_ctx* c, PassIter& it, int side, bool vals, const FjChunkSet& in, const std::vector<u32>& off, u64 chunks, int S, int bits_left,
                     int slot, int tiles_slot, u32* d_nt, hipStream_t s);

int emit_pending(fj_ctx* c, u64* d_ok, u64* d_ov, size_t cap, hipStream_t s, fj_timings* t) {
    Pending& pd = c->pend;
    if (!pd.valid) return set_err("fj_emit_pairs: no counted materialising join is pending on this context");
    if (pd.count > cap) return set_err("fj_emit_pairs: output capacity %zu < %llu pairs", cap, (unsigned long long)pd.count);
    if (pd.count > 0 && (((uintptr_t)d_ok | (uintptr_t)d_ov) & 7)) return set_err("output buffers must be 8-byte aligned");
    HIPCHK(hipEventRecord(c->ev[E_EMIT0], s));
    if (pd.count > 0) {
        void* p;
        if (pd.kind == Pending::LDS) {
            if (pd.lds.row_ids) {
                pd.lds.dedup = 1; pd.lds.orig_vals = nullptr;
            } else if (pd.has_dups) {
                if (get_buf(c, W_ROWIDX, pd.nb * 8, &p)) return 1;
                u64* rowidx = (u64*)p;
                HIPCHK(fj_launch_iota(rowidx, pd.nb, s));
                HIPCHK(hipMemsetAsync(&c->d_sc->alloc[0], 0, sizeof(c->d_sc->alloc) + sizeof(c->d_sc->seg_counter), s));
                PassIter bit;
// ... 163 lines not shown
    it.have_prev = true; it.prev = in; it.tiles = (const uint4*)p; it.ntiles = d_nt;
    if (side) { it.want_items = true; it.part_count_slot = W_PART_COUNT2; }
    HIPCHK(hipMemsetAsync(&c->d_sc->alloc[side * 4], 0, 4, s));
    HIPCHK(hipMemsetAsync(&c->d_sc->seg_counter[side * 4], 0, 4, s));
    if (pass_prepare(c, it, 1, s) || pass_launch(c, it, nullptr, nullptr, 0, s, nullptr) || pass_complete(c, it, s)) return 1;
    return 0;
}

int skew_join(fj_ctx* c, const FjLdsJoinArgs& ja, const Plan& plan, int top_bits, u32 nitems, int probe_slot, int materialize, hipStream_t s, bool* ok,
              u32* nparts_redone, Pending* pend) {
    *ok = false;
    if (!ja.items || !ja.build.list || !ja.probe.list || nitems == 0) return 0;
    std::vector<u32> pc(nitems);
    std::vector<uint4> items(nitems);
    HIPCHK(hipMemcpyAsync(pc.data(), ja.part_count, (size_t)nitems * 4, hipMemcpyDeviceToHost, s));
    HIPCHK(hipMemcpyAsync(items.data(), ja.items, (size_t)nitems * sizeof(uint4), hipMemcpyDeviceToHost, s));
    HIPCHK(hipStreamSynchronize(s));
    std::vector<u32> parts, flagged;
    for (u32 i = 0; i < nitems; ++i) if (pc[i] == FJ_ITEM_TOOBIG) { parts.push_back(items[i].z); flagged.push_back(i); }
    std::sort(parts.begin(), parts.end());
    parts.erase(std::unique(parts.begin(), parts.end()), parts.end());
    const u32 m = (u32)parts.size();
    if (m == 0 || m > 64) return 0;
    u64 already = 0;
    {
        u32 nlive = nitems;
        HIPCHK(hipMemcpy(&nlive, ja.nitems_dev, 4, hipMemcpyDeviceToHost));
        if (nlive > nitems) nlive = nitems;
        for (u32 i = 0; i < nlive; ++i) {
            if (pc[i] == FJ_ITEM_TOOBIG || pc[i] == FJ_ITEM_RETRY || !std::binary_search(parts.begin(), parts.end(), items[i].z)) continue;
            already += pc[i];
            flagged.push_back(i);
            HIPCHK(hipMemsetAsync(&ja.part_count[i], 0, 4, s));
        }
    }
    std::vector<u32> bo(2 * m), po(2 * m);
    for (u32 j = 0; j < m; ++j) {
        HIPCHK(hipMemcpyAsync(&bo[2 * j], ja.build.boff + parts[j], 8, hipMemcpyDeviceToHost, s));
        HIPCHK(hipMemcpyAsync(&po[2 * j], ja.probe.boff + parts[j], 8, hipMemcpyDeviceToHost, s));
    }
    HIPCHK(hipStreamSynchronize(s));
    u64 bchunks = 0, pchunks = 0, bmax = 0;
    for (u32 j = 0; j < m; ++j) { const u64 nb_j = bo[2 * j + 1] - bo[2 * j]; bchunks += nb_j; bmax = std::max(bmax, nb_j); pchunks += po[2 * j + 1] - po[2 * j]; }
    int S = 1;
    while (S < FJ_MAX_FAN_LOG && ((bmax * FJ_CHUNK) >> S) > 2048) ++S;
    if (((bmax * FJ_CHUNK) >> S) > 6000 || top_bits - plan.bits - S < 32) return 0;
    if (S < 5) S = std::min(5, top_bits - plan.bits - 32);
    if (S < 1) return 0;
    void* p;
    if (get_buf(c, W_SK_NT, 16, &p)) return 1;
    u32* d_nt = (u32*)p;
    PassIter bit2, pit2;
    const u64 count_main = c->h_sc->total - already;
    if (already) {
        HIPCHK(hipMemcpyAsync(&c->d_sc->total, &count_main, 8, hipMemcpyHostToDevice, s));
        HIPCHK(hipStreamSynchronize(s));
    }
    const bool had_dups = (c->h_sc->err & FJ_STAT_DUPS) != 0;
    HIPCHK(hipMemsetAsync(&c->d_sc->err, 0, 4, s));
    if (skew_side(c, bit2, 0, materialize != 0, ja.build, bo, bchunks, S, top_bits - plan.bits, plan.npass, W_SK_TILES_B, d_nt, s)) return 1;
    if (skew_side(c, pit2, 1, ja.row_ids != 0, ja.probe, po, pchunks, S, top_bits - plan.bits, probe_slot, W_SK_TILES_P, d_nt + 1, s)) return 1;
    FjLdsJoinArgs j2 = ja;
    j2.build = bit2.prev; j2.probe = pit2.prev; j2.nparts = j2.probe.nb; j2.nsplit = 1;
    j2.items = pit2.tiles; j2.nitems_dev = pit2.ntiles; j2.items_cap = pit2.items_cap; j2.part_count = pit2.part_count;
    j2.retry_only = 0; j2.mark_toobig = 0; j2.want_dups = materialize ? 1u : 0u; j2.dbg = nullptr;
    HIPCHK(fj_launch_lds_join(j2, false, s, nullptr, 0xFFFFFFFFu));
    if (read_scalars(c, s)) return 1;
    if ((c->h_sc->err & FJ_STAT_RETRY) && !(c->h_sc->err & (FJ_ERR_POOL | FJ_ERR_LDS_FULL))) {
        HIPCHK(fj_launch_lds_join_retry(j2, s));
        if (read_scalars(c, s)) return 1;
    }
    if (c->h_sc->err & FJ_ERR_POOL) return set_err("internal error: chunk pool exhausted while re-partitioning a skewed partition");
    if (c->h_sc->err & FJ_ERR_LDS_FULL) return 0;
    if (materialize) {
        pend->has_second = true; pend->lds2 = j2; pend->nitems2 = pit2.items_cap; pend->count_main = count_main; pend->flagged = flagged;
        pend->sk_parts = parts; pend->sk_bits = S; pend->sk_plan_bits = plan.bits; pend->sk_npass = plan.npass;
        pend->dups_main = had_dups;
    }
    *ok = true; *nparts_redone = m;
    return 0;
}

int radix_join_tail(fj_ctx* c, int materialize, FjLdsJoinArgs& ja, const Plan& plan, size_t np, const PassIter& pit, hipStream_t s,
                    fj_timings* t, int evc, u64* out_count, bool* lds_full, int top_bits, SingleOut* so) {
    ja.nparts = ja.probe.list ? ja.probe.nb : 1u << plan.bits;
    const u64 pchunks = (np + FJ_CHUNK - 1) / FJ_CHUNK;
    void* p;
    u32 nitems;
    if (ja.probe.list) {
        ja.items = pit.tiles; ja.nitems_dev = pit.ntiles; ja.items_cap = pit.items_cap; ja.part_count = pit.part_count;
        ja.nsplit = 1;
        nitems = pit.items_cap;
    } else {
        u64 nsplit = 1;
        if (ja.nparts < 2048) {
            nsplit = (2048 + ja.nparts - 1) / ja.nparts;
            const u64 per_part = pchunks / ja.nparts;
            nsplit = std::min<u64>(nsplit, std::max<u64>(1, per_part / 32));
        }
        ja.nsplit = (u32)nsplit; ja.items = nullptr; ja.nitems_dev = nullptr; ja.items_cap = 0;
        nitems = ja.nparts * ja.nsplit;
        if (get_buf(c, W_PART_COUNT, (size_t)nitems * 4, &p)) return 1; ja.part_count = (u32*)p;
    }
    ja.total = &c->d_sc->total; ja.err = &c->d_sc->err;
    ja.want_dups = materialize ? 1u : 0u; ja.dedup = 0; ja.orig_vals = nullptr; ja.retry_only = 0;
    ja.dbg = nullptr;
    ja.dbg_flags = (options().lab_hooks & FJ_HOOK_EMIT_RETRY_7TH) ? 8u : 0u;
#ifdef FJ_LAB
    if (getenv("FJ_JOIN_ABLATE")) ja.dbg_flags = (u32)atoi(getenv("FJ_JOIN_ABLATE"));
#endif
    if (so && materialize && ja.probe.list && ja.build.list && ja.build.vals && ja.items && !ja.dbg_flags) {
        FjLdsJoinArgs js = ja;
        js.out_cursor = &c->d_sc->total; js.out_capacity = so->cap; js.out_keys = so->keys; js.out_vals = so->vals; js.out_off = nullptr;
        HIPCHK(hipMemsetAsync(&c->d_sc->next_emit_item, 0, sizeof(u32), s));
        HIPCHK(fj_launch_emit_single(js, s, &c->d_sc->next_emit_item));
        HIPCHK(hipEventRecord(c->ev[E_JOIN], s));
        if (read_scalars(c, s)) return 1;
        if (c->h_sc->err & FJ_ERR_POOL) return pool_error();
        if (!(c->h_sc->err & (FJ_STAT_DUPS | FJ_STAT_EMIT_RETRY | FJ_ERR_LDS_FULL | FJ_ERR_OUTCAP))) {
            end_plan(c);
            plan_timings(c, plan, ja.nparts, evc, t);
            t->lds_retries = 0;
            *out_count = c->h_sc->total;
            so->done = true;
            return 0;
        }
        HIPCHK(hipMemsetAsync(&c->d_sc->total, 0, sizeof(unsigned long long), s));
        HIPCHK(hipMemsetAsync(&c->d_sc->err, 0, sizeof(u32), s));
    }
#ifdef FJ_LAB
    if (getenv("FJ_JOIN_STAMPS") && stamps_begin(&ja.dbg, s)) return 1;
#endif
    const bool wide = pit.item_tc_max == 32 && !materialize && !ja.dbg && !ja.dbg_flags && ja.probe.list && ja.build.list && ja.items;
    if (wide) {
        FjWideArgs wa{};
        wa.pmask = fj_wide_pmask(plan.bits, top_bits);
        wa.group_log = np / ((size_t)1 << plan.bits) > 7000 ? 3u : 0u;
        FjLdsJoinArgs jw = ja;
#ifdef FJ_LAB
        if (getenv("FJ_WIDE_STAMPS") && stamps_begin(&jw.dbg, s)) return 1;
#endif
        const u32 grid = std::min<u32>(nitems, c->num_cus);
        HIPCHK(fj_launch_count_join_wide(jw, wa, false, grid, s));
        if (jw.dbg) {
            std::vector<unsigned long long> h(4096 * 8);
            HIPCHK(hipStreamSynchronize(s));
            HIPCHK(hipMemcpy(h.data(), jw.dbg, h.size() * 8, hipMemcpyDeviceToHost));
            double acc[8] = {0, 0, 0, 0, 0, 0, 0, 0};
            for (u32 g = 0; g < grid && g < 4096; ++g) for (int i = 0; i < 8; ++i) acc[i] += (double)h[g * 8 + i] * 0.01;
            u32 nit = 0;
            HIPCHK(hipMemcpy(&nit, jw.nitems_dev, 4, hipMemcpyDeviceToHost));
            const double per = (double)std::min<u32>(grid, 4096) * ((double)nit / grid);
            fprintf(stderr, "[FJ_WIDE_STAMPS] us per item (thread 0): rotate+requests %.3f  claim_issue+zero %.3f  barB %.3f  probe %.3f  resolve+park %.3f  barA %.3f  stores %.3f\n",
                    acc[0] / per, acc[5] / per, acc[6] / per, acc[1] / per, acc[2] / per, acc[3] / per, acc[4] / per);
            for (int ph = 0; ph < 3; ++ph) {
                fprintf(stderr, "[FJ_WIDE_STAMPS] wave 0..15, %s:", ph == 0 ? "requests + claims issued + probe" : ph == 1 ? "claims resolved + park (to barrier A)" : "stores (barrier A to B)");
                for (int w = 0; w < 16; ++w) {
                    double sacc = 0;
                    for (u32 g = 0; g < grid && g < 256; ++g) sacc += (double)h[2048 * 8 + g * 64 + w * 4 + ph] * 0.01;
                    fprintf(stderr, " %.2f", sacc / ((double)std::min<u32>(grid, 256) * ((double)nit / grid)));
                }
                fprintf(stderr, "\n");
            }
        }
    } else
    HIPCHK(fj_launch_lds_join(ja, false, s, &c->d_sc->next_item, options().persistent_min_items));
    if (ja.dbg) { if (stamps_report("FJ_JOIN_STAMPS", ja.dbg, nitems, s)) return 1; ja.dbg = nullptr; }
    HIPCHK(hipEventRecord(c->ev[E_JOIN], s));
    if (read_scalars(c, s)) return 1;
    t->lds_retries = 0;
    if ((c->h_sc->err & FJ_STAT_RETRY) && !(c->h_sc->err & (FJ_ERR_POOL | FJ_ERR_LDS_FULL))) {
        ja.retry_only = 1; ja.mark_toobig = ja.items ? 1u : 0u;
        HIPCHK(fj_launch_lds_join_retry(ja, s));
        ja.retry_only = 0;
        HIPCHK(hipEventRecord(c->ev[E_JOIN], s));
        if (read_scalars(c, s)) return 1;
        t->lds_retries = 1;
        if ((c->h_sc->err & FJ_STAT_TOOBIG) && !(c->h_sc->err & (FJ_ERR_POOL | FJ_ERR_LDS_FULL))) {
            bool ok = false; u32 redone = 0;
            if (skew_join(c, ja, plan, top_bits, nitems, pit.slot, materialize, s, &ok, &redone, &c->pend)) return 1;
            HIPCHK(hipEventRecord(c->ev[E_JOIN], s));
            if (read_scalars(c, s)) return 1;
            if (ok) t->lds_retries = 1 + (int)redone;
            else c->h_sc->err |= FJ_ERR_LDS_FULL;
        }
    }
    if (c->h_sc->err & FJ_ERR_POOL) return pool_error();
    end_plan(c);
    plan_timings(c, plan, ja.nparts, evc, t);
    if (c->h_sc->err & FJ_ERR_LDS_FULL) { *lds_full = true; return 0; }
    *out_count = c->h_sc->total;
    if (materialize) {
        c->pend.valid = true; c->pend.kind = Pending::LDS; c->pend.lds = ja; c->pend.nitems = nitems; c->pend.count = *out_count;
        c->pend.has_dups = (c->h_sc->err & FJ_STAT_DUPS) != 0 || c->pend.dups_main;
    }
    return 0;
}

int join_radix(fj_ctx* c, int materialize, int bloom, const u64* bk, const u64* bv, size_t nb, const u64* pk, size_t np, int top_bits,
               hipStream_t s, fj_timings* t, u64* out_count, bool* lds_full, SingleOut* so = nullptr, bool rid = false) {
    Plan plan = make_plan(nb, top_bits, bloom != 0);
    *lds_full = false;
    t->sampled_hit_bp = -1;
    if (bloom == 2 && (plan.bloom_level == 0 || np < 4 * nb || np < (1u << 24) || !options().bloom_auto)) {
        bloom = 0; plan = make_plan(nb, top_bits, false);
    }
    begin_plan(c);
    HIPCHK(hipEventRecord(c->ev[E_START], s));
    if (clear_plan_scalars(c, s)) return 1;
    FjLdsJoinArgs ja{};
    PassIter bit, pit;
    pass_init(bit, 0, materialize != 0, nb, plan, top_bits);
    bit.vals_pos = rid;
    int evc = 0;
    if (plan.bloom_level > 0) bit.save_level = plan.bloom_level;
    if (run_passes(c, bit, bk, (materialize && !rid) ? bv : nullptr, s, &ja.build, nullptr)) return 1;
    HIPCHK(hipEventRecord(c->ev[E_BUILD], s));
    Plan pplan = plan;
    if (bloom == 2) {
        const u32 nsamp = FJ_SAMPLE_KEYS;
        HIPCHK(fj_launch_sample_hits(ja.build, pk, np, nsamp, (u32)(top_bits - 32 - plan.bits), (1u << plan.bits) - 1u, &c->d_sc->sample_hits, s));
        HIPCHK(hipMemcpyAsync(&c->h_sc->sample_hits, &c->d_sc->sample_hits, sizeof(unsigned long long), hipMemcpyDeviceToHost, s));
        HIPCHK(hipStreamSynchronize(s));
        const u32 hit_bp = (u32)(c->h_sc->sample_hits * 10000ull / nsamp);
        t->sampled_hit_bp = (int)hit_bp;
        if (hit_bp > (u32)options().bloom_auto_max_hit_bp) { pplan = make_plan(nb, top_bits, false); plan.bloom_level = 0; plan.npass = pplan.npass; }
    }
    pass_init(pit, 1, rid, np, pplan, top_bits);
    pit.vals_pos = rid;
    pit.want_items = true;
    {
        size_t np_eff = np;
        if (plan.bloom_level > 0) np_eff = (size_t)((double)np * (t->sampled_hit_bp >= 0 ? std::min(10000, t->sampled_hit_bp + 1000) : 1500) / 10000.0);
        if (wide_join_planned(materialize != 0, nb, np_eff, plan.bits)) pit.item_tc_max = 32;
    }
    if (plan.bloom_level > 0) pit.bloom_build = &bit.saved;
    if (run_passes(c, pit, pk, nullptr, s, &ja.probe, &evc)) return 1;
    HIPCHK(hipEventRecord(c->ev[E_PPART], s));
    ja.avg_build_keys = (u32)std::min<u64>(0xFFFFFFFFu, (u64)nb >> plan.bits);
    ja.row_ids = rid ? 1u : 0u;
    if (radix_join_tail(c, materialize, ja, plan, np, pit, s, t, evc, out_count, lds_full, top_bits, so)) return 1;
    if (c->pend.valid) { c->pend.bk = bk; c->pend.bv = bv; c->pend.nb = nb; c->pend.top_bits = top_bits; }
    return 0;
}

static int mm_tile_join(fj_ctx* c, const FjLdsJoinArgs& ja, u32 nitems, int materialize, hipStream_t s, Pending* pend,
                        int outer = FJ_MM_INNER, const FjMmOuterArgs* oa = nullptr) {
    u32 nlive = 0;
    std::vector<u32> pc(nitems), boff((size_t)ja.build.nb + 1);
    std::vector<uint4> items(nitems);
    HIPCHK(hipMemcpyAsync(&nlive, ja.nitems_dev, 4, hipMemcpyDeviceToHost, s));
    HIPCHK(hipMemcpyAsync(pc.data(), ja.part_count, (size_t)nitems * 4, hipMemcpyDeviceToHost, s));
    HIPCHK(hipMemcpyAsync(items.data(), ja.items, (size_t)nitems * sizeof(uint4), hipMemcpyDeviceToHost, s));
    HIPCHK(hipMemcpyAsync(boff.data(), ja.build.boff, boff.size() * 4, hipMemcpyDeviceToHost, s));
    HIPCHK(hipStreamSynchronize(s));
    if (nlive > nitems) nlive = nitems;
    std::vector<uint4> tiles, big;
    for (u32 i = 0; i < nlive; ++i) {
        if (pc[i] != FJ_ITEM_TOOBIG) continue;
        pc[i] = 0;
        if (outer != FJ_MM_INNER) big.push_back(items[i]);
        const u32 part = items[i].z;
        if (part >= ja.build.nb) return set_err("internal error: work item %u of a many-to-many join names partition %u of %u", i, part, ja.build.nb);
        const u32 nbc = boff[part + 1] - boff[part];
        for (u32 c_lo = 0; c_lo < nbc; c_lo += FJ_MM_TILE_CHUNKS) tiles.push_back(make_uint4(items[i].x, items[i].y, part, c_lo));
    }
    if (tiles.empty()) return set_err("internal error: the many-to-many counting pass reported an oversized partition and marked no item");
    if (tiles.size() > (1u << 26)) return set_err("many-to-many join: %zu (probe item, build tile) work items for the partitions beyond 4096 build rows; not supported", tiles.size());
    const u32 n2 = (u32)tiles.size();
    void* p;
    FjLdsJoinArgs j2 = ja;
    FjMmOuterArgs o2{};
    FjMmSweepArgs sw{};
    u64* tile_off = nullptr; u64* sweep_off = nullptr;
    const u32 nbig = (u32)big.size();
    if (outer == FJ_MM_INNER) {
        if (get_buf(c, W_MM_TILES, (size_t)n2 * sizeof(uint4), &p)) return 1;
        HIPCHK(hipMemcpyAsync(p, tiles.data(), (size_t)n2 * sizeof(uint4), hipMemcpyHostToDevice, s));
        j2.items = (const uint4*)p; j2.nitems_dev = nullptr; j2.items_cap = n2; j2.mark_toobig = 0;
        if (get_buf(c, W_PART_COUNT2, (size_t)n2 * 4, &p)) return 1;
        j2.part_count = (u32*)p;
    } else {
        auto r16 = [](size_t b) { return (b + 15) & ~(size_t)15; };
        const size_t o_big = (size_t)n2 * sizeof(uint4), o_tc = o_big + (size_t)nbig * sizeof(uint4), o_sc = o_tc + r16((size_t)n2 * 4),
                     o_to = o_sc + r16((size_t)nbig * 4), o_so = o_to + r16(((size_t)n2 + 1) * 8), bytes = o_so + r16(((size_t)nbig + 1) * 8);
        if (get_buf(c, W_MM_TILES, bytes, &p)) return 1;
        unsigned char* base = (unsigned char*)p;
        HIPCHK(hipMemcpyAsync(base, tiles.data(), (size_t)n2 * sizeof(uint4), hipMemcpyHostToDevice, s));
        HIPCHK(hipMemcpyAsync(base + o_big, big.data(), (size_t)nbig * sizeof(uint4), hipMemcpyHostToDevice, s));
        j2.items = (const uint4*)base; j2.nitems_dev = nullptr; j2.items_cap = n2; j2.mark_toobig = 0;
        j2.part_count = (u32*)(base + o_tc);
        tile_off = (u64*)(base + o_to); sweep_off = (u64*)(base + o_so);
        const size_t pbit_bytes = (size_t)ja.probe.cap * (FJ_CHUNK / 8);
        if (get_buf(c, W_MM_PBITS, pbit_bytes, &p)) return 1;
        HIPCHK(hipMemsetAsync(p, 0, pbit_bytes, s));
        o2 = *oa; o2.pbits = (u64*)p;
        sw.probe = ja.probe; sw.items = (const uint4*)(base + o_big); sw.nitems = nbig; sw.pbits = o2.pbits;
        sw.miss_count = (u32*)(base + o_sc); sw.miss_total = oa->miss_total; sw.row_ids = ja.row_ids;
    }
    HIPCHK(hipMemcpyAsync(ja.part_count, pc.data(), (size_t)nlive * 4, hipMemcpyHostToDevice, s));
    HIPCHK(hipMemsetAsync(&c->d_sc->err, 0, 4, s));
    const u64 count_main = c->h_sc->total, u_main = c->h_sc->expected;
    HIPCHK(fj_launch_mm_tile_join(j2, false, s, outer, &o2));
    if (outer != FJ_MM_INNER) HIPCHK(fj_launch_mm_miss_sweep(sw, false, s));
    HIPCHK(hipEventRecord(c->ev[E_JOIN], s));
    if (read_scalars(c, s)) return 1;
    if (materialize) {
        pend->has_second = true; pend->lds2 = j2; pend->nitems2 = n2; pend->count_main = count_main;
        if (outer != FJ_MM_INNER) { pend->mm_sweep = sw; pend->mm_u_main = u_main; pend->mm_tile_off = tile_off; pend->mm_sweep_off = sweep_off; }
    }
    return 0;
}

int join_many(fj_ctx* c, int materialize, const u64* bk, const u64* bv, size_t nb, const u64* pk, size_t np, int top_bits,
              hipStream_t s, fj_timings* t, u64* out_count, bool rid = false, int outer = FJ_MM_INNER) {
    const Plan plan = make_plan(nb, top_bits, false, 2048);
    begin_plan(c);
    HIPCHK(hipEventRecord(c->ev[E_START], s));
    if (clear_plan_scalars(c, s)) return 1;
    FjLdsJoinArgs ja{};
    PassIter bit, pit;
    pass_init(bit, 0, materialize != 0, nb, plan, top_bits);
    pass_init(pit, 1, rid, np, plan, top_bits);
    bit.vals_pos = pit.vals_pos = rid;
    pit.want_items = true;
// ... 308 lines not shown
```

flash_hash_join_amd/csrc/fj_lds_table_dev.h:

```cpp
#pragma once
#include "fj_internal.h"

__device__ __forceinline__ u32 fj_chunk_entry(const FjChunkSet& cs, u32 idx) {
    if (cs.list) return cs.list[idx];
    const u64 rem = cs.n_flat - (u64)idx * FJ_CHUNK;
    const u32 cnt = rem >= FJ_CHUNK ? FJ_CHUNK : (u32)rem;
    return ((cnt - 1u) << 24) | idx;
}

__device__ __forceinline__ bool fj_item_slice(const uint4* items, const u32* nitems_dev, u32 nsplit, u64 probe_n_flat, u32 item,
                                              u32& p, u32& s_lo, u32& s_hi) {
    if (items) {
        if (item >= *nitems_dev) return false;
        const uint4 it = items[item];
        p = it.z; s_lo = it.x; s_hi = it.x + it.y;
    } else {
        const u32 slice = item % nsplit;
        p = item / nsplit;
        const u32 npc = (u32)((probe_n_flat + FJ_CHUNK - 1) >> FJ_CHUNK_LOG);
        s_lo = (u32)(((u64)slice * npc) / nsplit); s_hi = (u32)(((u64)(slice + 1) * npc) / nsplit);
    }
    return true;
}

__device__ __forceinline__ void fj_part_chunks(const FjChunkSet& cs, u32 p, u32& b0, u32& nbc) {
    b0 = 0;
    if (cs.list) { b0 = cs.boff[p]; nbc = cs.boff[p + 1] - b0; }
    else nbc = (u32)((cs.n_flat + FJ_CHUNK - 1) >> FJ_CHUNK_LOG);
}
```

flash_hash_join_amd/csrc/fj_partition.hip:

```cpp
#include "fj_internal.h"
#include <cstdlib>
#include <mutex>
#include <vector>

namespace {

#ifndef FJ_LO_PAD
#define FJ_LO_PAD 1u
#endif
struct PartLds {
    u32 sorted_k, sorted_v, lo_k, lo_v, hist, toff, line_desc, t_chunk, t_cnt, wsum, misc, total;
};
__host__ __device__ inline PartLds part_lds_layout(u32 T, u32 F, u32 line, bool vals, u32 nwaves) {
    PartLds L;
    const u32 nsorted = T + 2;
    const u32 maxl = (T + (line - 1) * F) / line + 2;
    u32 o = 0;
    L.sorted_k = o; o += nsorted * 8;
    L.sorted_v = o; if (vals) o += nsorted * 8;
    L.lo_k = o; o += F * (line + FJ_LO_PAD) * 8;
    L.lo_v = o; if (vals) o += F * (line + FJ_LO_PAD) * 8;
    L.line_desc = o; o += maxl * 8;
    L.wsum = o; o += nwaves * 8;
    L.hist = o; o += (F + 4) * 4;
    L.toff = o; o += (F + 4) * 4;
    L.t_chunk = o; o += (T / FJ_CHUNK) * 4;
    L.t_cnt = o; o += (T / FJ_CHUNK) * 4;
    L.misc = o; o += 16 * 4;
    L.total = (o + 15) & ~15u;
    return L;
}

enum { M_SLAB_CUR = 0, M_SLAB_REM, M_NEW_BASE, M_NEED, M_NLINES, M_FLUSH, M_SEG, M_NEW_UNITS };

template <int NT, int KPT, int LINE_LOG, bool HAS_VALS, bool FLAT, bool PROBE_SIDE, int RLOG = FJ_RUN_LOG, bool PK7 = false, bool POS = false>
__global__ __launch_bounds__(NT, 4) void fj_partition_kernel(FjPartArgs a) {
    constexpr u32 T = NT * KPT, LINE = 1u << LINE_LOG, TC = T / FJ_CHUNK, NW = NT / 64, LOS = LINE + FJ_LO_PAD;
    static_assert(T % FJ_CHUNK == 0 && TC <= NT && LINE >= 4 && T + 64 < (1u << 17), "tile geometry");
    static_assert(!PK7 || (!FLAT && KPT % 4 == 0), "wire-format chunks come through chunk lists, four keys per load group");
    static_assert(!POS || (FLAT && HAS_VALS), "positions are made by the first pass over a flat input");
    constexpr bool RUNS = RLOG > 0;
    constexpr u32 RL = (u32)RLOG, RU = 1u << RL;
    const u32 F = 1u << a.fan_log, FM = F - 1;
    const u32 tid = threadIdx.x, lane = tid & 63, wave = tid >> 6;
    const u32 sh32 = a.shift - 32;

    extern __shared__ __attribute__((aligned(16))) unsigned char smem[];
    const PartLds Lo = part_lds_layout(T, F, LINE, HAS_VALS, NW);
    u64* tile_k = (u64*)(smem + Lo.sorted_k);
    u64* tile_v = (u64*)(smem + Lo.sorted_v);
    u64* lo_k = (u64*)(smem + Lo.lo_k);
    u64* lo_v = (u64*)(smem + Lo.lo_v);
    u64* line_desc = (u64*)(smem + Lo.line_desc);
    u64* wsum = (u64*)(smem + Lo.wsum);
    u32* hist = (u32*)(smem + Lo.hist);
    u32* toff = (u32*)(smem + Lo.toff);
    u32* t_chunk = (u32*)(smem + Lo.t_chunk);
    u32* t_cnt = (u32*)(smem + Lo.t_cnt);
    u32* misc = (u32*)(smem + Lo.misc);

    const u32 Lc = FLAT ? (u32)((a.n_flat + FJ_CHUNK - 1) >> FJ_CHUNK_LOG) : 0u;
    const u32 ntiles = FLAT ? (Lc + TC - 1) / TC : *a.in_ntiles;
    const u32 G = gridDim.x, g = blockIdx.x;
    const u32 t0 = (u32)(((u64)g * ntiles) / G);
    const u32 nmine = (u32)(((u64)(g + 1) * ntiles) / G) - t0;
    u32 t = 0;
    const u32 thi = nmine;
    const u32 cap = a.cap_chunks;
    if (t >= thi) return;

    auto get_desc = [&](u32 tt, u32& pos, u32& len, u32& parent) {
        const uint4 d = a.in_tiles[t0 + tt]; pos = d.x; len = d.y; parent = d.z;
    };
    auto meta_fetch = [&](u32 pos, u32 len, u32& id, u32& cnt) {
        id = 0; cnt = 0;
        if (tid < len) { const u32 e = a.in_list[pos + tid]; id = FJ_LIST_ID(e); cnt = FJ_LIST_CNT(e); }
    };
    const bool tiny = FLAT && a.n_flat < 2;
    const u64 last_pair = FLAT ? ((a.n_flat - 2) & ~1ull) : 0;
    struct Pk7Raw { uint4 lo; uint2 mid; u32 hi; };
    auto key_load7 = [&](u32 tt, Pk7Raw (&rr)[KPT / 4 ? KPT / 4 : 1], u64 (&vv)[KPT], u32& vmask) {
        (void)tt;
        vmask = 0;
#pragma unroll
        for (int i = 0; i < KPT / 4; ++i) {
            const u32 kidx = ((u32)i * NT + tid) * 4;
            const u32 j = kidx >> FJ_CHUNK_LOG, off = kidx & (FJ_CHUNK - 1);
            const u32 cnt = t_cnt[j];
            const unsigned char* base = reinterpret_cast<const unsigned char*>(a.in_keys) + (u64)t_chunk[j] * FJ_WIRE7_BYTES;
            rr[i].lo = *reinterpret_cast<const uint4*>(base + off * 4u);
            rr[i].mid = *reinterpret_cast<const uint2*>(base + FJ_WIRE7_MID + off * 2u);
            rr[i].hi = *reinterpret_cast<const u32*>(base + FJ_WIRE7_HI + off);
            if (HAS_VALS) {
                const u64x2 w0 = *reinterpret_cast<const u64x2*>(a.in_vals + (u64)t_chunk[j] * FJ_CHUNK + off);
                const u64x2 w1 = *reinterpret_cast<const u64x2*>(a.in_vals + (u64)t_chunk[j] * FJ_CHUNK + off + 2);
                vv[4 * i] = w0.x; vv[4 * i + 1] = w0.y; vv[4 * i + 2] = w1.x; vv[4 * i + 3] = w1.y;
            }
            const u32 nv = off < cnt ? (cnt - off < 4u ? cnt - off : 4u) : 0u;
            vmask |= ((1u << nv) - 1u) << (4 * i);
        }
    };
    auto key_load = [&](u32 tt, u64 (&kk)[KPT], u64 (&vv)[KPT], u32& vmask) {
        vmask = 0;
#pragma unroll
        for (int i = 0; i < KPT / 2; ++i) {
            u64 base; u32 nv;
            if (FLAT) {
                base = (u64)(t0 + tt) * T + ((u32)i * NT + tid) * 2;
                nv = base + 1 < a.n_flat ? 2u : (base < a.n_flat ? 1u : 0u);
                if (POS) { vv[2 * i] = base; vv[2 * i + 1] = base + 1; }
                if (base > last_pair) base = last_pair;
            } else {
                const u32 kidx = ((u32)i * NT + tid) * 2;
                const u32 j = kidx >> FJ_CHUNK_LOG, off = kidx & (FJ_CHUNK - 1);
                const u32 cnt = t_cnt[j];
                base = (u64)t_chunk[j] * FJ_CHUNK + off;
                nv = off + 1 < cnt ? 2u : (off < cnt ? 1u : 0u);
            }
            if (tiny) {
                kk[2 * i] = nv ? a.in_keys[0] : 0; kk[2 * i + 1] = 0;
                if (HAS_VALS) { vv[2 * i] = (nv && !POS) ? a.in_vals[0] : 0; vv[2 * i + 1] = 0; }
            } else {
                const u64x2 q = *reinterpret_cast<const u64x2*>(a.in_keys + base);
// ... 5 lines not shown
            }
            vmask |= (nv == 2 ? 3u : (nv == 1 ? 1u : 0u)) << (2 * i);
        }
        if (FLAT && !tiny && (a.n_flat & 1ull)) {
#pragma unroll
            for (int i = 0; i < KPT / 2; ++i) {
                const u64 base = (u64)(t0 + tt) * T + ((u32)i * NT + tid) * 2;
                if (base + 1 == a.n_flat) { kk[2 * i] = a.in_keys[base]; if (HAS_VALS) vv[2 * i] = POS ? base : a.in_vals[base]; }
            }
        }
    };

    if (tid == 0) { misc[M_SLAB_CUR] = 0; misc[M_SLAB_REM] = 0; misc[M_NEW_BASE] = 0; misc[M_SEG] = 0; misc[M_NEW_UNITS] = 0; }
    u32 st_left = 0, st_fill = FJ_CHUNK, st_cur = FJ_DIR_INVALID, st_nch = 0;
    u32 pend_cnt = 0, pend_nf = 0, pend_tb = 0;

    auto carry = [&]() {
        if (tid < F) {
            const u32 b = tid, tot = st_left + pend_cnt;
            if (pend_nf == 0) {
                for (u32 j = 0; j < pend_cnt; ++j) {
                    lo_k[b * LOS + st_left + j] = tile_k[pend_tb + j];
                    if (HAS_VALS) lo_v[b * LOS + st_left + j] = tile_v[pend_tb + j];
                }
            } else {
                const u32 nl2 = tot - pend_nf, src = pend_tb + (pend_nf - st_left);
                for (u32 j = 0; j < nl2; ++j) {
                    lo_k[b * LOS + j] = tile_k[src + j];
                    if (HAS_VALS) lo_v[b * LOS + j] = tile_v[src + j];
                }
            }
            st_left = tot - pend_nf;
            pend_cnt = 0; pend_nf = 0;
        }
    };

    auto alloc_id = [&](u32 j, u32) -> u32 {
        const u32 rem = misc[M_SLAB_REM];
        return j < rem ? misc[M_SLAB_CUR] + (j << RL) : misc[M_NEW_BASE] + ((j - rem) << RL);
    };
    auto rot = [&](u32 b) -> u32 { return ((b * 2654435761u + blockIdx.x * 40503u) >> 13) & (RU - 1u); };
    auto run_left = [&](u32 c0, u32 b) -> u32 { return (RUNS && c0 != FJ_DIR_INVALID) ? (RU - 1u) - ((c0 - rot(b)) & (RU - 1u)) : 0u; };
    auto run_step = [&](u32 c0, u32 k) -> u32 { return (c0 & ~(RU - 1u)) | ((c0 + k) & (RU - 1u)); };
    auto chunk_id = [&](u32 kk, u32 c0, u32 ukb, u32 b) -> u32 {
        if constexpr (!RUNS) return alloc_id(ukb + kk - 1, b);
        const u32 rl = run_left(c0, b);
        if (kk <= rl) return run_step(c0, kk);
        const u32 q = kk - rl - 1u;
        return alloc_id(ukb + (q >> RL), b) + ((q + rot(b)) & (RU - 1u));
    };
    auto take_slabs = [&](u32 need) {
        const u32 su = a.slab >> RL, k = (need - misc[M_SLAB_REM] + su - 1) / su;
        const u32 nb = atomicAdd(a.alloc, k * a.slab);
        if (nb + k * a.slab > cap) atomicOr(a.err, FJ_ERR_POOL);
        misc[M_NEW_BASE] = nb; misc[M_NEW_UNITS] = k * su;
    };
    auto commit_units = [&](u32 need) {
        const u32 rem = misc[M_SLAB_REM];
        if (need <= rem) { misc[M_SLAB_CUR] += need << RL; misc[M_SLAB_REM] = rem - need; }
        else { const u32 used = need - rem; misc[M_SLAB_CUR] = misc[M_NEW_BASE] + (used << RL); misc[M_SLAB_REM] = misc[M_NEW_UNITS] - used; }
    };

    auto flush = [&](u32 parent) {
        if (tid == 0) misc[M_FLUSH] = 0;
        __syncthreads();
        u32 fresh = 0xFFFFFFFFu;
        if (tid < F && st_left > 0 && st_fill == FJ_CHUNK && !run_left(st_cur, tid)) fresh = atomicAdd(&misc[M_FLUSH], 1u);
        __syncthreads();
        if (tid == 0 && misc[M_FLUSH] > misc[M_SLAB_REM]) take_slabs(misc[M_FLUSH]);
        __syncthreads();
        if (tid < F) {
            const u32 b = tid, l = st_left, seg = misc[M_SEG];
            u32 f0 = st_fill, c = st_cur, n = st_nch;
            const u32 outb = parent * F + b;
            if (l > 0 && f0 == FJ_CHUNK) {
                if (fresh == 0xFFFFFFFFu) c = run_step(c, 1);
                else c = alloc_id(fresh, b) + rot(b);
                f0 = 0;
                if (c < cap) a.out_rel[c] = ((u64)seg << 32) | n;
                ++n;
            }
            if (c != FJ_DIR_INVALID && c < cap) {
                const u64 base = (u64)c * FJ_CHUNK + f0;
                for (u32 j = 0; j < l; ++j) {
                    a.out_keys[base + j] = lo_k[b * LOS + j];
                    if (HAS_VALS) a.out_vals[base + j] = lo_v[b * LOS + j];
                }
                a.out_dir[c] = (outb << FJ_DIR_CNT_BITS) | (f0 + l);
                if constexpr (RUNS) { for (u32 k = 1; k <= run_left(c, b); ++k) { const u32 id = run_step(c, k); if (id < cap) a.out_dir[id] = FJ_DIR_INVALID; } }
            }
            if (n > 0) {
                const u32 off = atomicAdd(&a.bchunks[outb], n);
                if (seg < a.max_segs) a.seg_off[(u64)seg * F + b] = off;
            }
            st_left = 0; st_fill = FJ_CHUNK; st_cur = FJ_DIR_INVALID; st_nch = 0;
        }
        __syncthreads();
        if (tid == 0) commit_units(misc[M_FLUSH]);
        __syncthreads();
    };

    u64 kn[KPT], vn[KPT];
    Pk7Raw rn[KPT / 4 ? KPT / 4 : 1];
    u32 validn = 0, par_next = a.parent0, par_n2 = a.parent0, mid = 0, mcnt = 0;
    u32 d3_pos = 0, d3_len = 0, d3_par = 0;
    if (FLAT) {
        key_load(t, kn, vn, validn);
    } else {
        u32 p, l;
        get_desc(t, p, l, par_next);
        meta_fetch(p, l, mid, mcnt);
        if (tid < TC) { t_chunk[tid] = mid; t_cnt[tid] = mcnt; }
        __syncthreads();
        if constexpr (PK7) key_load7(t, rn, vn, validn); else key_load(t, kn, vn, validn);
        mid = 0; mcnt = 0;
        if (t + 1 < thi) { get_desc(t + 1, p, l, par_n2); meta_fetch(p, l, mid, mcnt); }
        if (t + 2 < thi) get_desc(t + 2, d3_pos, d3_len, d3_par);
        __syncthreads();
        if (tid < TC) { t_chunk[tid] = mid; t_cnt[tid] = mcnt; }
    }
    __syncthreads();

    u32 cur_parent = 0xFFFFFFFFu;
    u32 hotb = 0xFFFFFFFFu;
    for (; t < thi; ++t) {
        u64 k[KPT], v[KPT];
#pragma unroll
        for (int i = 0; i < KPT; ++i) { k[i] = FLAT ? fj_key_mix(kn[i]) : kn[i]; if (HAS_VALS) v[i] = vn[i]; }
        const u32 valid = validn, parent = par_next;
        if constexpr (PK7) {
            const u64 top = (u64)((a.in_b0 + parent) >> a.in_top_shift) << 56;
#pragma unroll
            for (int i = 0; i < KPT / 4; ++i) {
                const u32 lo[4] = {rn[i].lo.x, rn[i].lo.y, rn[i].lo.z, rn[i].lo.w};
#pragma unroll
                for (int m = 0; m < 4; ++m) {
                    const u32 md = ((m & 2) ? rn[i].mid.y : rn[i].mid.x) >> ((m & 1) * 16) & 0xFFFFu;
                    const u32 hb = (rn[i].hi >> (8 * m)) & 0xFFu;
                    k[4 * i + m] = top | ((u64)((hb << 16) | md) << 32) | lo[m];
                }
            }
        }
        const u32 par_t1 = par_n2;
        if (!FLAT) {
            mid = 0; mcnt = 0;
            if (t + 2 < thi) { par_n2 = d3_par; meta_fetch(d3_pos, d3_len, mid, mcnt); }
            if (t + 3 < thi) get_desc(t + 3, d3_pos, d3_len, d3_par);
        }
        if (t + 1 < thi) { if constexpr (PK7) key_load7(t + 1, rn, vn, validn); else key_load(t + 1, kn, vn, validn); par_next = par_t1; }

        carry();
        if (parent != cur_parent) {
            if (cur_parent != 0xFFFFFFFFu) flush(cur_parent);
            if (tid == 0) {
                const u32 seg = atomicAdd(a.seg_counter, 1u);
                if (seg >= a.max_segs) atomicOr(a.err, FJ_ERR_POOL);
                misc[M_SEG] = seg;
            }
            cur_parent = parent;
        }
        for (u32 b = tid; b <= F; b += NT) hist[b] = 0;
        __syncthreads();

        u32 br[KPT];
        if (hotb == 0xFFFFFFFFu) {
#pragma unroll
// ... 41 lines not shown
                kr = RUNS ? (km > rl ? (km - rl + RU - 1u) >> RL : 0u) : km;
                x = (u64)cnt | ((u64)(nf >> LINE_LOG) << 20) | ((u64)kr << 40);
            }
            u64 inc = x;
#pragma unroll
            for (int d = 1; d < 64; d <<= 1) {
                const u64 y = __shfl_up(inc, d, 64);
                if ((int)lane >= d) inc += y;
            }
            if (lane == 63) wsum[wave] = inc;
            kb = (u32)((inc - x) >> 40); l0 = (u32)(((inc - x) >> 20) & 0xFFFFFu);
            if (tid < F) toff[tid] = (u32)((inc - x) & 0xFFFFFu);
        }
        __syncthreads();
        if (wave * 64 < F) {
            u64 woff = 0;
            for (u32 w = 0; w < wave; ++w) woff += wsum[w];
            if (tid < F) {
                const u32 to = toff[tid] + (u32)(woff & 0xFFFFFu);
                toff[tid] = to;
                l0 += (u32)((woff >> 20) & 0xFFFFFu);
                kb += (u32)(woff >> 40);
                if (tid == F - 1) {
                    toff[F] = to + cnt;
                    const u32 need = kb + kr;
                    misc[M_NLINES] = l0 + (nf >> LINE_LOG);
                    misc[M_NEED] = need;
                    if (need > misc[M_SLAB_REM]) take_slabs(need);
                }
            }
        }
        __syncthreads();

#pragma unroll
        for (int i = 0; i < KPT; ++i) {
            const u32 d = toff[br[i] >> 16] + (br[i] & 0xFFFFu);
            tile_k[d] = k[i];
            if (HAS_VALS) tile_v[d] = v[i];
        }
        if (wave * 64 < F) {
            const bool own = tid < F;
            const u32 f0 = st_fill, c0 = st_cur, tb = own ? toff[tid] : 0u;
            const u32 nl = own ? (nf >> LINE_LOG) : 0u;
            auto put = [&](u32 pb, u32 pf0, u32 pc0, u32 pkb, u32 ptb, u32 pleft, u32 pl0, u32 j) {
                const u32 q = j << LINE_LOG, pq = pf0 + q, kk = pq >> FJ_CHUNK_LOG, off = pq & (FJ_CHUNK - 1);
                const u32 id = kk == 0 ? pc0 : chunk_id(kk, pc0, pkb, pb);
                const u32 dst = id < cap ? id * FJ_CHUNK + off : FJ_DIR_INVALID;
                const u32 lc = j == 0 ? pleft : 0u;
                const u32 sidx = ptb + q + 32u - pleft;
                line_desc[pl0 + j] = ((u64)dst << 32) | ((u64)pb << 22) | ((u64)lc << 17) | sidx;
            };
            const u32 avg2 = (2u * T / LINE) >> a.fan_log;
            const u32 own_lines = avg2 > 4u ? avg2 : 4u;
            for (u32 j = 0; j < nl && j < own_lines; ++j) put(tid, f0, c0, kb, tb, st_left, l0, j);
            u64 big = __ballot(nl > own_lines);
            while (big) {
                const int src = __builtin_ctzll(big);
                big &= big - 1;
                const u32 pf0 = (u32)__builtin_amdgcn_readlane((int)f0, src), pc0 = (u32)__builtin_amdgcn_readlane((int)c0, src);
                const u32 pkb = (u32)__builtin_amdgcn_readlane((int)kb, src), ptb = (u32)__builtin_amdgcn_readlane((int)tb, src);
                const u32 pleft = (u32)__builtin_amdgcn_readlane((int)st_left, src), pl0 = (u32)__builtin_amdgcn_readlane((int)l0, src);
                const u32 pnl = (u32)__builtin_amdgcn_readlane((int)nl, src);
                for (u32 j = own_lines + lane; j < pnl; j += 64) put(wave * 64 + (u32)src, pf0, pc0, pkb, ptb, pleft, pl0, j);
            }
        }
        if (tid < F) {
            const u32 b = tid, f0 = st_fill, c0 = st_cur, n0 = st_nch, tb = toff[b];
            const u32 outb = (parent * F + b) << FJ_DIR_CNT_BITS;
            const u64 segw = (u64)misc[M_SEG] << 32;
            for (u32 kk = 1; kk <= km; ++kk) {
                const u32 id = chunk_id(kk, c0, kb, b);
                if (id < cap) { a.out_dir[id] = outb | FJ_CHUNK; a.out_rel[id] = segw | (n0 + kk - 1); }
            }
            pend_cnt = cnt; pend_nf = nf; pend_tb = tb;
            st_cur = km ? chunk_id(km, c0, kb, b) : c0;
            st_fill = f0 + nf - (km << FJ_CHUNK_LOG);
            st_nch = n0 + km;
        }
        __syncthreads();

        if (!FLAT && tid < TC) { t_chunk[tid] = mid; t_cnt[tid] = mcnt; }
        const u32 nl = misc[M_NLINES];
        constexpr u32 WK = 2, WLPL = LINE / WK;
        for (u32 e = tid; e < nl * WLPL; e += NT) {
            const u32 l = e / WLPL, q = (e % WLPL) * WK;
            const u64 d = line_desc[l];
            const u32 dst = (u32)(d >> 32);
            if (dst != FJ_DIR_INVALID) {
                const u32 w = (u32)d, b = w >> 22, lc = (w >> 17) & 31u, sidx = (w & 0x1FFFFu) - 32u;
                u64 r[WK], rv[WK];
#pragma unroll
                for (int i = 0; i < (int)WK; ++i) {
                    const u32 vi = q + i;
                    const bool in_lo = vi < lc;
                    const u64* sk = in_lo ? (lo_k + b * LOS + vi) : (tile_k + (sidx + vi));
                    r[i] = *sk;
                    if (HAS_VALS) { const u64* sv = in_lo ? (lo_v + b * LOS + vi) : (tile_v + (sidx + vi)); rv[i] = *sv; }
                }
                u64x2 r0; r0.x = r[0]; r0.y = r[1];
                *reinterpret_cast<u64x2*>(a.out_keys + (u64)dst + q) = r0;
                if (HAS_VALS) { u64x2 w0; w0.x = rv[0]; w0.y = rv[1]; *reinterpret_cast<u64x2*>(a.out_vals + (u64)dst + q) = w0; }
            }
        }
        if (tid == 0) commit_units(misc[M_NEED]);
        __syncthreads();
    }
    carry();
    flush(cur_parent);
    for (u32 j = tid; j < (misc[M_SLAB_REM] << RL); j += NT) { const u32 id = misc[M_SLAB_CUR] + j; if (id < cap) a.out_dir[id] = FJ_DIR_INVALID; }
}

template <typename T, typename In, typename Out>
__device__ __forceinline__ T fj_block_scan(In value_at, Out put, u32 n) {
    __shared__ T wtot[4][16];
    const u32 tid = threadIdx.x, lane = tid & 63, wave = tid >> 6;
    T carry = 0;
    for (u32 base = 0; base < n; base += 16384) {
        T x[4][4], sum[4], inc[4];
#pragma unroll
        for (int j = 0; j < 4; ++j) {
            const u32 e0 = base + 4u * ((u32)j * 1024u + tid);
#pragma unroll
            for (int k = 0; k < 4; ++k) x[j][k] = e0 + k < n ? (T)value_at(e0 + k) : (T)0;
            sum[j] = x[j][0] + x[j][1] + x[j][2] + x[j][3];
            T v = sum[j];
#pragma unroll
            for (int d = 1; d < 64; d <<= 1) { const T y = __shfl_up(v, d, 64); if ((int)lane >= d) v += y; }
            inc[j] = v;
            if (lane == 63) wtot[j][wave] = v;
        }
        __syncthreads();
        T before = carry, total = carry;
#pragma unroll
        for (int j = 0; j < 4; ++j) {
            T mine = 0, all = 0;
            for (u32 w = 0; w < 16; ++w) { const T c = wtot[j][w]; all += c; if (w < wave) mine += c; }
            T run = total + mine + inc[j] - sum[j];
            const u32 e0 = base + 4u * ((u32)j * 1024u + tid);
#pragma unroll
            for (int k = 0; k < 4; ++k) { if (e0 + k < n) put(e0 + k, run); run += x[j][k]; }
            total += all;
        }
        (void)before;
        carry = total;
        __syncthreads();
    }
    return carry;
}

__global__ __launch_bounds__(1024) void fj_level_scan(u32* __restrict__ bchunks, u32* __restrict__ boff, u32 n, u32 tc,
                                                      u32* __restrict__ toff) {
    __shared__ u64 wtot[4][16];
    const u32 tid = threadIdx.x, lane = tid & 63, wave = tid >> 6;
    const float rtc = tc ? 1.0f / (float)tc : 0.f;
    auto tiles_of = [&](u32 c) -> u32 {
        if (!tc) return 0u;
        u32 q = (u32)((float)c * rtc);
        while (q * tc < c) ++q;
        while (q && (q - 1) * tc >= c) --q;
        return q;
    };
    u64 carry = 0;
    for (u32 base = 0; base < n; base += 16384) {
        uint4 x[4]; u64 sum[4], inc[4];
#pragma unroll
        for (int j = 0; j < 4; ++j) {
// ... 240 lines not shown
        __syncthreads();
        u32 e[4]; u64 r[4];
#pragma unroll
        for (int u = 0; u < 4; ++u) {
            const u32 i = base + (u32)u * NT + tid;
            e[u] = i < n ? dir[i] : FJ_DIR_INVALID;
            r[u] = i < n ? rel[i] : 0;
        }
        u32 pos[4], slot[4], bk[4]; bool ok[4];
#pragma unroll
        for (int u = 0; u < 4; ++u) {
            const u32 b = e[u] >> FJ_DIR_CNT_BITS, seg = (u32)(r[u] >> 32);
            ok[u] = e[u] != FJ_DIR_INVALID && seg < max_segs && b < nb;
            bk[u] = ok[u] ? b : 0u;
            pos[u] = ok[u] ? boff[b] + seg_off[(u64)seg * (fan_mask + 1) + (b & fan_mask)] + (u32)r[u] : 0;
        }
#pragma unroll
        for (int u = 0; u < 4; ++u) slot[u] = ok[u] ? atomicAdd(&hist[bk[u]], 1u) : 0u;
        __syncthreads();
        u32 v = 0, inc = 0;
        if (tid < NBMAX) {
            v = hist[tid]; inc = v;
#pragma unroll
            for (int d = 1; d < 64; d <<= 1) { const u32 y = __shfl_up(inc, d, 64); if ((int)lane >= d) inc += y; }
            if (lane == 63) wsum[wave] = inc;
        }
        __syncthreads();
        if (tid < NBMAX) {
            u32 woff = 0;
            for (u32 w = 0; w < wave; ++w) woff += wsum[w];
            hist[tid] = woff + inc - v;
            if (tid == NBMAX - 1) hist[NBMAX] = woff + inc;
        }
        __syncthreads();
#pragma unroll
        for (int u = 0; u < 4; ++u)
            if (ok[u]) ent[hist[bk[u]] + slot[u]] = make_uint2(pos[u], (((e[u] & FJ_DIR_CNT_MASK) - 1u) << 24) | (base + (u32)u * NT + tid));
        __syncthreads();
        const u32 total = hist[NBMAX];
        for (u32 j = tid; j < total; j += NT) { const uint2 x = ent[j]; list[x.x] = x.y; }
        __syncthreads();
    }
}

__global__ __launch_bounds__(1024) void fj_dir_rank_kernel(u32* __restrict__ dir, u32 n, u32 b_lo, u32 nbk, u32 fan, u64* __restrict__ rel,
                                                           u32* __restrict__ seg_off, u32* __restrict__ bchunks, u32* __restrict__ nalloc) {
    __shared__ u32 h[1u << FJ_MAX_FAN_LOG];
    const u32 tid = threadIdx.x, base = blockIdx.x * 4096u;
    if (tid < (1u << FJ_MAX_FAN_LOG)) h[tid] = 0;
    __syncthreads();
    u32 bb[4], rr[4];
#pragma unroll
    for (int u = 0; u < 4; ++u) {
        const u32 i = base + (u32)u * 1024u + tid;
        bb[u] = FJ_DIR_INVALID; rr[u] = 0;
        if (i < n) {
            const u32 e = dir[i], b = (e >> FJ_DIR_CNT_BITS) - b_lo, cnt = e & FJ_DIR_CNT_MASK;
            const bool ok = e != FJ_DIR_INVALID && b < nbk && cnt >= 1u && cnt <= FJ_CHUNK;
            if (ok) bb[u] = b;
            dir[i] = ok ? ((b << FJ_DIR_CNT_BITS) | cnt) : FJ_DIR_INVALID;
        }
        const bool ok = bb[u] != FJ_DIR_INVALID;
        const u64 m = __ballot(ok);
        if (m) {
            const u32 b0 = (u32)__builtin_amdgcn_readlane((int)bb[u], __builtin_ctzll(m));
            if (__ballot(ok && bb[u] != b0) == 0) {
                u32 wb = 0;
                if ((threadIdx.x & 63u) == (u32)__builtin_ctzll(m)) wb = atomicAdd(&h[b0], (u32)__popcll(m));
                wb = (u32)__builtin_amdgcn_readlane((int)wb, __builtin_ctzll(m));
                if (ok) rr[u] = wb + (u32)__popcll(m & ((1ull << (threadIdx.x & 63u)) - 1ull));
            } else if (ok) rr[u] = atomicAdd(&h[bb[u]], 1u);
        }
    }
    __syncthreads();
    if (tid < nbk) { const u32 c = h[tid]; if (c) seg_off[(u64)blockIdx.x * fan + tid] = atomicAdd(&bchunks[tid], c); }
#pragma unroll
    for (int u = 0; u < 4; ++u) {
        const u32 i = base + (u32)u * 1024u + tid;
        if (bb[u] != FJ_DIR_INVALID) rel[i] = ((u64)blockIdx.x << 32) | rr[u];
    }
    if (blockIdx.x == 0 && tid == 0) *nalloc = n;
}

template <int NT, int KPT, int LINE_LOG, bool HAS_VALS, bool FLAT, bool PROBE_SIDE, int RLOG = FJ_RUN_LOG, bool PK7 = false, bool POS = false>
hipError_t launch_part0(const FjPartArgs& a, u32 grid, hipStream_t s) {
    const u32 F = 1u << a.fan_log;
    const PartLds L = part_lds_layout(NT * KPT, F, 1u << LINE_LOG, HAS_VALS, NT / 64);
    auto kern = fj_partition_kernel<NT, KPT, LINE_LOG, HAS_VALS, FLAT, PROBE_SIDE, RLOG, PK7, POS>;
    hipError_t e = fj_set_max_lds_once(reinterpret_cast<const void*>(kern), L.total);
    if (e != hipSuccess) return e;
    hipLaunchKernelGGL(kern, dim3(grid), dim3(NT), L.total, s, a);
    return hipGetLastError();
}

template <int NT, int KPT, int LINE_LOG, bool HAS_VALS, bool FLAT, bool PROBE_SIDE>
hipError_t launch_part1(const FjPartArgs& a, u32 grid, hipStream_t s) {
    if constexpr (FLAT && HAS_VALS) {
        if (a.vals_pos) {
            if (a.run_log == 0) return launch_part0<NT, KPT, LINE_LOG, HAS_VALS, FLAT, PROBE_SIDE, 0, false, true>(a, grid, s);
            if (a.run_log != FJ_RUN_LOG) return hipErrorInvalidValue;
            return launch_part0<NT, KPT, LINE_LOG, HAS_VALS, FLAT, PROBE_SIDE, FJ_RUN_LOG, false, true>(a, grid, s);
        }
    }
    if constexpr (FLAT) { if (a.run_log == 0) return launch_part0<NT, KPT, LINE_LOG, HAS_VALS, FLAT, PROBE_SIDE, 0>(a, grid, s); }
    if (a.run_log != FJ_RUN_LOG) return hipErrorInvalidValue;
    return launch_part0<NT, KPT, LINE_LOG, HAS_VALS, FLAT, PROBE_SIDE, FJ_RUN_LOG>(a, grid, s);
}

template <int NT, int KPT, int LINE_LOG, bool HAS_VALS, bool FLAT>
hipError_t launch_part(const FjPartArgs& a, u32 grid, hipStream_t s) {
    if constexpr (!HAS_VALS) {
        if (a.side == 0) return launch_part1<NT, KPT, LINE_LOG, HAS_VALS, FLAT, false>(a, grid, s);
    }
    return launch_part1<NT, KPT, LINE_LOG, HAS_VALS, FLAT, true>(a, grid, s);
}

template <int NT, int KPT, bool HAS_VALS>
hipError_t launch_part2(const FjPartArgs& a, int line_log, u32 grid, hipStream_t s) {
    const bool flat = a.in_list == nullptr;
    if (line_log == 3) return flat ? launch_part<NT, KPT, 3, HAS_VALS, true>(a, grid, s) : launch_part<NT, KPT, 3, HAS_VALS, false>(a, grid, s);
    return flat ? launch_part<NT, KPT, 4, HAS_VALS, true>(a, grid, s) : launch_part<NT, KPT, 4, HAS_VALS, false>(a, grid, s);
}

}

hipError_t fj_set_max_lds_once(const void* fn, u32 bytes) {
    struct Seen { const void* fn; int dev; u32 bytes; };
    static std::mutex mu;
    static std::vector<Seen> seen;
    int dev = 0;
    hipError_t e = hipGetDevice(&dev);
    if (e != hipSuccess) return e;
    std::lock_guard<std::mutex> lk(mu);
    for (Seen& x : seen)
        if (x.fn == fn && x.dev == dev) {
            if (x.bytes >= bytes) return hipSuccess;
            e = hipFuncSetAttribute(fn, hipFuncAttributeMaxDynamicSharedMemorySize, (int)bytes);
            if (e == hipSuccess) x.bytes = bytes;
            return e;
        }
    e = hipFuncSetAttribute(fn, hipFuncAttributeMaxDynamicSharedMemorySize, (int)bytes);
    if (e == hipSuccess) seen.push_back({fn, dev, bytes});
    return e;
}

u32 fj_partition_lds_bytes(u32 fan_log, bool vals, int line_log) {
    const u32 F = 1u << fan_log;
    if (vals) return part_lds_layout(1024 * 4, F, 1u << line_log, true, 16).total;
    return part_lds_layout(1024 * 8, F, 1u << line_log, false, 16).total;
}

u32 fj_partition_tile_chunks(u32 fan_log, bool vals) { (void)fan_log; return vals ? 16u : 32u; }


hipError_t fj_launch_partition(const FjPartArgs& a, bool vals, int line_log, u32 grid, hipStream_t s) {
    if (a.shift < 32) return hipErrorInvalidValue;
    if (a.fan_log > FJ_MAX_FAN_LOG || a.slab < (1u << FJ_RUN_LOG) || (a.slab & ((1u << FJ_RUN_LOG) - 1u))) return hipErrorInvalidValue;
    if (a.in_pk7) {
        if (!a.in_list || a.run_log != FJ_RUN_LOG) return hipErrorInvalidValue;
        if (vals) {
            if (a.fan_log == 9 && line_log != 3) return hipErrorInvalidValue;
            return line_log == 3 ? launch_part0<1024, 4, 3, true, false, true, FJ_RUN_LOG, true>(a, grid, s)
                                 : launch_part0<1024, 4, 4, true, false, true, FJ_RUN_LOG, true>(a, grid, s);
        }
        if (line_log != 4) return hipErrorInvalidValue;
        const u32 g = a.fan_log == 9 ? grid : (grid < 256 ? grid : 256);
        return a.side == 0 ? launch_part0<1024, 8, 4, false, false, false, FJ_RUN_LOG, true>(a, g, s)
                           : launch_part0<1024, 8, 4, false, false, true, FJ_RUN_LOG, true>(a, g, s);
    }
    if (a.fan_log == 9) {
        if (vals) return line_log == 3 ? launch_part2<1024, 4, true>(a, 3, grid, s) : hipErrorInvalidValue;
        return launch_part2<1024, 8, false>(a, line_log, grid, s);
    }
    if (vals) {
        return launch_part2<1024, 4, true>(a, line_log, grid, s);
    }
    return launch_part2<1024, 8, false>(a, line_log, grid < 256 ? grid : 256, s);
}

hipError_t fj_launch_group(const FjChunkSet& cs, u32 tc, u32* toff, uint4* tiles, u32 max_tiles, u32* zero_tail, hipStream_t s) {
    if (cs.nb & 3u) return hipErrorInvalidValue;
    static_assert(FJ_RUN_LOG == 1 || FJ_RUN_LOG == 2, "fj_level_lists reads a run's directory words with one 8-B or 16-B load");
    if (cs.run_log != 0 && cs.run_log != FJ_RUN_LOG) return hipErrorInvalidValue;
    if (cs.run_log == 0 && cs.nb <= 512 && cs.cap >= 4096) {
        const u32 blocks = (cs.cap + 4095u) / 4096u;
        if (blocks <= 512u) {
            hipLaunchKernelGGL(fj_level_lists_binned<true>, dim3(blocks), dim3(1024), 0, s, cs.dir, cs.rel, cs.alloc, cs.cap, cs.boff,
                               cs.seg_off, cs.fan_mask, cs.max_segs, cs.list, cs.nb, tc, toff, tiles, max_tiles, zero_tail, cs.bchunks);
        } else {
            hipLaunchKernelGGL(fj_level_scan, dim3(1), dim3(1024), 0, s, cs.bchunks, cs.boff, cs.nb, tc, toff);
            hipLaunchKernelGGL(fj_level_lists_binned<false>, dim3(blocks < 4096u ? blocks : 4096u), dim3(1024), 0, s, cs.dir, cs.rel, cs.alloc, cs.cap, cs.boff,
                               cs.seg_off, cs.fan_mask, cs.max_segs, cs.list, cs.nb, tc, toff, tiles, max_tiles, zero_tail, cs.bchunks);
        }
        return hipGetLastError();
    }
    const bool wide = cs.nb >= 8192u && cs.nb <= (1u << 19);
    if (wide) hipLaunchKernelGGL(fj_level_scan_wide, dim3((cs.nb + 4095u) / 4096u), dim3(1024), 0, s, cs.bchunks, cs.boff, cs.nb, tc, toff);
    else hipLaunchKernelGGL(fj_level_scan, dim3(1), dim3(1024), 0, s, cs.bchunks, cs.boff, cs.nb, tc, toff);
    auto kern = cs.run_log ? fj_level_lists<FJ_RUN_LOG> : fj_level_lists<0>;
    hipLaunchKernelGGL(kern, dim3(2048), dim3(256), 0, s, cs.dir, cs.rel, cs.alloc, cs.cap, cs.boff, cs.seg_off,
                       cs.fan_mask, cs.max_segs, cs.list, cs.nb, tc, toff, tiles, max_tiles, zero_tail, wide ? cs.bchunks : (u32*)nullptr);
    return hipGetLastError();
}

hipError_t fj_launch_dir_rank(u32* dir, u32 n, u32 b_lo, u32 nbk, u32 fan, u64* rel, u32* seg_off, u32* bchunks, u32* nalloc, hipStream_t s) {
    if (nbk > (1u << FJ_MAX_FAN_LOG) || fan < nbk || n == 0) return hipErrorInvalidValue;
    hipLaunchKernelGGL(fj_dir_rank_kernel, dim3((n + 4095u) / 4096u), dim3(1024), 0, s, dir, n, b_lo, nbk, fan, rel, seg_off, bchunks, nalloc);
    return hipGetLastError();
}

hipError_t fj_launch_scan_u32_to_u64(const u32* in, u64* out, u32 n, hipStream_t s) {
    hipLaunchKernelGGL(fj_scan_u32_to_u64, dim3(1), dim3(1024), 0, s, in, out, n);
    return hipGetLastError();
}
```

flash_hash_join_amd/csrc/fj_plan.hip:

```cpp
#include "fj_host.h"

namespace fjh {

namespace { thread_local std::string g_err; thread_local fj_timings g_last; }

int set_err(const char* fmt, ...) {
    char buf[1024];
    va_list ap; va_start(ap, fmt); vsnprintf(buf, sizeof buf, fmt, ap); va_end(ap);
    g_err = buf;
    return 1;
}
fj_timings& last_timings() { return g_last; }

Options& options() { static Options o; return o; }
static int set_option_value(Options& o, const char* name, long long value);
Options::Options() {
    static const char* const legacy[] = {"FJ_RADIX_THRESHOLD", "FJ_SCALAR_HBM_TABLE", "FJ_BLOOM_AUTO", "FJ_BLOOM_AUTO_MAX_HIT_BP", "FJ_BLOOM_VARIANT", "FJ_PLAN_TARGET_KEYS",
                                         "FJ_MAT_SINGLE_PASS", "FJ_PERSISTENT_MIN_ITEMS", "FJ_JOIN_ITEMS_TARGET", "FJ_JOIN_WIDE", "FJ_DIST_LOOPBACK", "FJ_DIST_INJECT_FAIL",
                                         "FJ_DIST_RESERVE_ALWAYS", "FJ_DIST_SPLIT_ALWAYS", "FJ_DIST_ONE_COMM", "FJ_EMIT_TAGGED"};
    for (const char* name : legacy)
        if (getenv(name)) fprintf(stderr, "flash_hash_join_amd: the environment variable %s is no longer read (use FJ_OPTIONS=\"name=value,...\" or fj_set_option; see include/flashjoin.h)\n", name);
    const char* e = getenv("FJ_OPTIONS");
    if (!e) return;
    std::string str(e);
// ... 61 lines not shown
        const int nb1 = p.bits == 0 ? 5 : p.bits + 1;
        if (p.bits == 0 || plan_npass(nb1) == plan_npass(p.bits)) p.bits = nb1;
    }
    if (p.bits > 0 && p.bits < 5) p.bits = 5;
    if (p.bits > top_bits - 32) p.bits = top_bits - 32;
    plan_passes(p, true);
    if (want_bloom && p.npass >= 2) {
        if (p.npass == 2)
            while (p.fan_log[0] < FJ_MAX_FAN_LOG && p.fan_log[1] > 4 && (nb >> p.fan_log[0]) > FJ_BLOOM_GOOD_KEYS) { ++p.fan_log[0]; --p.fan_log[1]; }
        int lvl_bits = 0;
        for (int i = 0; i + 1 < p.npass; ++i) lvl_bits += p.fan_log[i];
        if ((nb >> lvl_bits) <= FJ_BLOOM_MAX_KEYS) p.bloom_level = p.npass - 1;
    }
    return p;
}


void pass_init(PassIter& it, int side, bool has_vals, size_t n, const Plan& plan, int top_bits) {
    it = PassIter();
    it.side = side; it.has_vals = has_vals; it.n = n; it.plan = plan; it.used = top_bits;
    it.lbound = (n + FJ_CHUNK - 1) / FJ_CHUNK;
}

u32 pass_groups(u64 chunks, u64 rows, u32 tile_chunks, u32 F) {
    const u64 g64 = std::min<u64>(chunks / tile_chunks, rows / ((u64)F * 128));
    return (u32)std::min<u64>(512, std::max<u64>(1, g64));
}

int pass_prepare(fj_ctx* c, PassIter& it, u32 appends, hipStream_t s) {
    const int i = it.i;
    it.F = 1u << it.plan.fan_log[i];
    it.used -= it.plan.fan_log[i];
    it.appends = appends ? appends : 1;
    it.tile_chunks = fj_partition_tile_chunks((u32)it.plan.fan_log[i], it.has_vals);
    it.Gmax = pass_groups(it.lbound, it.n, it.tile_chunks, it.F);
    if (c->reserve_cus) it.Gmax = std::min<u32>(it.Gmax, c->reserve_cus < c->num_cus ? c->num_cus - c->reserve_cus : 1u);
    if (it.piece_rows && it.appends > 1 && !it.have_prev)
        it.Gmax = std::min(it.Gmax, pass_groups((it.piece_rows + FJ_CHUNK - 1) / FJ_CHUNK, it.piece_rows, it.tile_chunks, it.F));
    const u32 F = it.F, G = it.Gmax, parents = it.parents;
    const u64 nb_out = (u64)parents * F;
    const u64 cap64 = (it.n / FJ_CHUNK + 1 + (((u64)(G + parents) * F << FJ_RUN_LOG) + (u64)(G + 1) * fj_slab_for(it.appends)) * it.appends + 3) & ~3ull;
    if (cap64 >= (1ull << 24) || nb_out >= (1u << 22))
        return set_err("relation of %zu rows is too large for one GPU's chunk directory", it.n);
    FjChunkSet cs{};
    cs.cap = (u32)cap64; cs.nb = (u32)nb_out; cs.n_flat = 0; cs.fan_mask = F - 1; cs.max_segs = (G + parents + 2) * it.appends;
    cs.run_log = (!it.have_prev && it.i == 0 && F <= 256) ? 0u : (u32)FJ_RUN_LOG;
    const int base = it.side * W_SIDE_STRIDE + (it.slot & 1) * W_KINDS;
    it.cs_base = base;
    void* p;
    if (get_buf(c, base + W_POOL_K, cap64 * FJ_CHUNK * 8, &p)) return 1; cs.keys = (u64*)p;
    cs.vals = nullptr;
    if (it.has_vals) { if (get_buf(c, base + W_POOL_V, cap64 * FJ_CHUNK * 8, &p)) return 1; cs.vals = (u64*)p; }
    if (get_buf(c, base + W_DIR, cap64 * 4, &p)) return 1; cs.dir = (u32*)p;
    if (get_buf(c, base + W_REL, cap64 * 8, &p)) return 1; cs.rel = (u64*)p;
    if (get_buf(c, base + W_LIST, cap64 * 4, &p)) return 1; cs.list = (u32*)p;
    if (get_zeroed_buf(c, base + W_BCHUNKS, nb_out * 4 + 16, &p, s)) return 1; cs.bchunks = (u32*)p;
    if (get_buf(c, base + W_BOFF, (nb_out + 1) * 4, &p)) return 1; cs.boff = (u32*)p;
    if (get_buf(c, base + W_SEGOFF, (size_t)cs.max_segs * F * 4, &p)) return 1; cs.seg_off = (u32*)p;
    cs.alloc = it.alloc_word ? it.alloc_word : &c->d_sc->alloc[it.side * 4 + i];
    it.cs = cs;
    return 0;
}

int pass_launch(fj_ctx* c, PassIter& it, const u64* keys, const u64* vals, size_t n, hipStream_t s, int* ev_cursor) {
    const FjChunkSet& cs = it.cs;
    FjPartArgs a{};
    u32 G = it.Gmax;
    if (it.have_prev) {
        a.in_keys = it.prev.keys; a.in_vals = it.prev.vals; a.in_list = it.prev.list; a.in_dir = it.prev.dir;
        a.in_tiles = it.tiles; a.in_ntiles = it.ntiles; a.n_flat = 0;
    } else {
        a.in_keys = keys; a.in_vals = vals; a.in_list = nullptr; a.in_dir = nullptr; a.in_tiles = nullptr; a.in_ntiles = nullptr; a.n_flat = n;
        a.vals_pos = it.has_vals && it.vals_pos ? 1u : 0u;
        G = std::min(G, pass_groups((n + FJ_CHUNK - 1) / FJ_CHUNK, n, it.tile_chunks, it.F));
    }
    a.parent0 = 0;
    a.out_keys = cs.keys; a.out_vals = cs.vals; a.out_dir = cs.dir; a.out_rel = cs.rel; a.seg_off = cs.seg_off;
    a.bchunks = cs.bchunks; a.alloc = cs.alloc; a.seg_counter = it.seg_word ? it.seg_word : &c->d_sc->seg_counter[it.side * 4 + it.i];
    a.cap_chunks = cs.cap; a.max_segs = cs.max_segs;
    a.err = it.err_word ? it.err_word : &c->d_sc->err;
    if (it.have_prev && it.in_pk7) { a.in_pk7 = 1; a.in_b0 = it.in_b0; a.in_top_shift = it.in_top_shift; }
    a.shift = (u32)it.used; a.fan_log = (u32)it.plan.fan_log[it.i]; a.slab = fj_slab_for(it.appends); a.run_log = cs.run_log; a.side = (u32)it.side;
    const int line_log = (it.has_vals && it.F > 256) ? 3 : 4;
    if (ev_cursor) HIPCHK(hipEventRecord(c->ev[E_PK0 + 2 * (*ev_cursor)], s));
    HIPCHK(fj_launch_partition(a, it.has_vals, line_log, G, s));
    if (ev_cursor) { HIPCHK(hipEventRecord(c->ev[E_PK0 + 2 * (*ev_cursor) + 1], s)); ++*ev_cursor; }
    return 0;
}

bool bloom_stage_follows(const PassIter& it, int level) { return it.plan.bloom_level == level && it.bloom_build && !it.bloom_done; }

void join_item_geometry(u64 nparts, size_t np, u64 chunk_bound, u32* tc, u64* max_items) {
    const u64 pchunks = (np + FJ_CHUNK - 1) / FJ_CHUNK;
    const u64 bound = std::max<u64>(chunk_bound, pchunks);
    const u64 avg = std::max<u64>(1, bound / nparts);
    u64 want = 1;
    const u64 target_items = options().join_items_target;
    if (nparts < target_items) want = std::min<u64>((target_items + nparts - 1) / nparts, std::max<u64>(1, (pchunks / nparts) / 32));
    *tc = (u32)(want > 1 ? std::max<u64>(8, (avg * 9 / 8 + want - 1) / want) : std::max<u64>(512, 4 * avg));
    *max_items = bound / *tc + nparts + 1;
}

bool wide_join_planned(bool materialize, size_t nb, size_t np_eff, int bits) {
    if (materialize || bits <= 0 || options().join_wide == 0) return false;
    if (options().join_wide == 1) return true;
    return np_eff <= 3 * nb;
}

int level_finish(fj_ctx* c, PassIter& it, bool final_level, hipStream_t s) {
    const FjChunkSet& cs = it.cs;
    u32 tc = 0; u64 max_tiles = 0; u32* zero_tail = nullptr;
    if (bloom_stage_follows(it, it.i)) tc = fj_bloom_tile_chunks();
    else if (!final_level) tc = fj_partition_tile_chunks((u32)it.plan.fan_log[it.i], it.has_vals);
    else if (it.want_items) {
        join_item_geometry(cs.nb, it.n, it.lbound, &tc, &max_tiles);
        if (it.item_tc_max && tc > it.item_tc_max) { tc = it.item_tc_max; max_tiles = std::max<u64>(it.lbound, (it.n + FJ_CHUNK - 1) / FJ_CHUNK) / tc + cs.nb + 1; }
    }
    if (tc && !max_tiles) max_tiles = it.lbound / tc + cs.nb + 1;
    if (max_tiles >= (1ull << 31)) return set_err("internal error: tile table too large");
    u32* toff = nullptr; uint4* tiles = nullptr;
    void* p;
    if (tc) {
        if (get_buf(c, it.cs_base + W_TOFF, ((size_t)cs.nb + 1) * 4, &p)) return 1; toff = (u32*)p;
        if (get_buf(c, it.cs_base + W_TILES, max_tiles * sizeof(uint4), &p)) return 1; tiles = (uint4*)p;
        if (final_level) {
            if (get_buf(c, it.part_count_slot, (size_t)max_tiles * 4, &p)) return 1;
            it.part_count = zero_tail = (u32*)p; it.items_cap = (u32)max_tiles;
        }
    }
    HIPCHK(fj_launch_group(cs, tc, toff, tiles, (u32)max_tiles, zero_tail, s));
    it.tiles = tiles; it.ntiles = toff ? toff + cs.nb : nullptr; it.toff = toff;
    return 0;
}

int pass_complete(fj_ctx* c, PassIter& it, hipStream_t s) {
    const FjChunkSet& cs = it.cs;
    it.lbound = it.n / FJ_CHUNK + 1 + (u64)(it.Gmax + it.parents) * it.F * it.appends;
    ++it.i;
    if (level_finish(c, it, it.i == it.plan.npass, s)) return 1;
    it.prev = cs; it.have_prev = true;
    it.parents = cs.nb;
    ++it.slot;
    if (it.save_level == it.i) it.saved = cs;
    return 0;
}

int bloom_stage(fj_ctx* c, PassIter& it, hipStream_t s) {
    const FjChunkSet in = it.prev;
    const u32 G = c->num_cus;
    const u32 nw = fj_bloom_waves_per_group();
    const u64 max_segs = (u64)nw * ((u64)in.nb + G) + 16;
    const u64 cap64 = it.n / FJ_CHUNK + 1 + max_segs + (u64)fj_bloom_slab_chunks() * nw * G;
    if (cap64 >= (1ull << 24)) return set_err("relation of %zu rows is too large for one GPU's chunk directory", it.n);
    FjChunkSet cs{};
    cs.cap = (u32)cap64; cs.nb = in.nb; cs.n_flat = 0; cs.fan_mask = 0; cs.max_segs = (u32)max_segs;
    const int base = it.side * W_SIDE_STRIDE + (it.slot & 1) * W_KINDS;
    void* p;
    if (get_buf(c, base + W_POOL_K, cap64 * FJ_CHUNK * 8, &p)) return 1; cs.keys = (u64*)p;
    cs.vals = nullptr;
    if (get_buf(c, base + W_DIR, cap64 * 4, &p)) return 1; cs.dir = (u32*)p;
    if (get_buf(c, base + W_REL, cap64 * 8, &p)) return 1; cs.rel = (u64*)p;
    if (get_buf(c, base + W_LIST, cap64 * 4, &p)) return 1; cs.list = (u32*)p;
    if (get_zeroed_buf(c, base + W_BCHUNKS, (size_t)cs.nb * 4 + 16, &p, s)) return 1; cs.bchunks = (u32*)p;
    if (get_buf(c, base + W_BOFF, ((size_t)cs.nb + 1) * 4, &p)) return 1; cs.boff = (u32*)p;
    if (get_buf(c, base + W_SEGOFF, (size_t)cs.max_segs * 4, &p)) return 1; cs.seg_off = (u32*)p;
    cs.alloc = &c->d_sc->alloc[it.side * 4 + 3];
    FjBloomArgs a{};
    a.pkeys = in.keys; a.plist = in.list; a.pnb = in.nb; a.tiles = it.tiles; a.toff = it.toff;
// ... 100 lines not shown
    t->total_ms = ev_ms(c, E_START, E_JOIN);
    return 0;
}

int gt_close(fj_ctx* c, hipStream_t s, fj_timings* t) {
    HIPCHK(hipEventRecord(c->ev[E_JOIN], s));
    return gt_read(c, s, t);
}

int kind_agg(int kind, int plane) {
    if (kind < KIND_UNSIGNED || kind > KIND_FLOAT || plane < PLANE_COUNT || plane > PLANE_MAX) return -1;
    static const int forms[3][4] = {{FJ_GJ_COUNT, FJ_GJ_SUM, FJ_GJ_MIN_U, FJ_GJ_MAX_U},
                                    {FJ_GJ_COUNT, FJ_GJ_SUM, FJ_GJ_MIN_S, FJ_GJ_MAX_S},
                                    {FJ_GJ_COUNT, FJ_GJ_SUM_F, FJ_GJ_MIN_F, FJ_GJ_MAX_F}};
    return forms[kind][plane];
}

int rel_open(fj_ctx* c, const u64* keys, RelBeside beside, const u64* vals, size_t n, int top_bits, u64 target, hipStream_t s,
             RelAttempt* r) {
    r->plan = make_plan(n, top_bits, false, target);
    begin_plan(c);
    HIPCHK(hipEventRecord(c->ev[E_START], s));
    if (clear_plan_scalars(c, s)) return 1;
    PassIter it;
    pass_init(it, 0, beside != REL_KEYS_ONLY, n, r->plan, top_bits);
    it.vals_pos = beside == REL_POSITIONS;
    if (run_passes(c, it, keys, beside == REL_VALUES ? vals : nullptr, s, &r->rel, nullptr)) return 1;
    HIPCHK(hipEventRecord(c->ev[E_BUILD], s));
    HIPCHK(hipEventRecord(c->ev[E_PPART], s));
    r->nparts = r->rel.list ? r->rel.nb : 1u;
    return 0;
}

int rel_close(fj_ctx* c, const Plan& plan, u32 nparts, hipStream_t s, fj_timings* t) {
    HIPCHK(hipEventRecord(c->ev[E_JOIN], s));
    if (read_scalars(c, s)) return 1;
    if (c->h_sc->err & FJ_ERR_POOL) return pool_error();
    end_plan(c);
    plan_timings(c, plan, nparts, 0, t);
    t->probe_phase_ms = t->join_ms;
    return 0;
}

int stamps_begin(unsigned long long** dbg, hipStream_t s) {
    static unsigned long long* dbg_buf = nullptr;
    if (!dbg_buf) HIPCHK(hipMalloc((void**)&dbg_buf, 4096 * 8 * 8));
    HIPCHK(hipMemsetAsync(dbg_buf, 0, 4096 * 8 * 8, s));
    *dbg = dbg_buf;
    return 0;
}
int stamps_report(const char* label, const unsigned long long* dbg, u32 nitems, hipStream_t s) {
    std::vector<unsigned long long> h(4096 * 8);
    HIPCHK(hipStreamSynchronize(s));
    HIPCHK(hipMemcpy(h.data(), dbg, h.size() * 8, hipMemcpyDeviceToHost));
    double acc[6] = {0, 0, 0, 0, 0, 0}; int n = 0;
    unsigned long long tmin = ~0ull, tmax = 0;
    for (int i = 0; i < 4096 && i < (int)nitems; ++i) {
        const unsigned long long* r = &h[i * 8];
        if (!r[0] || !r[5]) continue;
        for (int j = 1; j <= 5; ++j) acc[j] += (double)(r[j] - r[j - 1]) * 0.01;
        if (r[0] < tmin) tmin = r[0];
        if (r[5] > tmax) tmax = r[5];
        ++n;
    }
    if (n == 0) n = 1;
    fprintf(stderr, "[%s] items=%d  meta+init=%.2f  build=%.2f  buildsync=%.2f  probe=%.2f  fin=%.2f us (means); first 4096 items span %.1f us\n",
            label, n, acc[1] / n, acc[2] / n, acc[3] / n, acc[4] / n, acc[5] / n, (double)(tmax - tmin) * 0.01);
    return 0;
}

static int set_option_value(Options& o, const char* name, long long value) {
    if (!strcmp(name, "radix_threshold")) { if (value < 0) return set_err("fj_set_option: radix_threshold must be >= 0"); o.radix_threshold = (size_t)value; return 0; }
    if (!strcmp(name, "scalar_hbm_table")) { o.scalar_hbm_table = value != 0; return 0; }
    if (!strcmp(name, "plan_target_keys")) { if (value < 16 || value > (long long)FJ_PART_TARGET_KEYS) return set_err("fj_set_option: plan_target_keys must be 16..%u", FJ_PART_TARGET_KEYS); o.plan_target_keys = (u32)value; return 0; }
    if (!strcmp(name, "bloom_auto")) { o.bloom_auto = value != 0; return 0; }
    if (!strcmp(name, "mat_single_pass")) { o.mat_single_pass = value != 0; return 0; }
    if (!strcmp(name, "bloom_auto_max_hit_bp")) { if (value < 0 || value > 10000) return set_err("fj_set_option: bloom_auto_max_hit_bp must be 0..10000"); o.bloom_auto_max_hit_bp = (int)value; return 0; }
    if (!strcmp(name, "bloom_variant")) { if (value < 0 || value > 2) return set_err("fj_set_option: bloom_variant must be 0..2"); o.bloom_variant = (int)value; return 0; }
    if (!strcmp(name, "join_wide")) { if (value < 0 || value > 2) return set_err("fj_set_option: join_wide must be 0..2"); o.join_wide = (int)value; return 0; }
    if (!strcmp(name, "persistent_min_items")) { if (value < 0) return set_err("fj_set_option: persistent_min_items must be >= 0"); o.persistent_min_items = (u32)std::min<long long>(value, 0xFFFFFFFFll); return 0; }
    if (!strcmp(name, "lab_hooks")) { if (value < 0 || value > 0xFFFF) return set_err("fj_set_option: lab_hooks is a mask of FJ_HOOK_* bits"); o.lab_hooks = (u32)value; return 0; }
    if (!strcmp(name, "join_items_target")) { if (value < 1 || value > (1 << 20)) return set_err("fj_set_option: join_items_target must be 1..1048576"); o.join_items_target = (u32)value; return 0; }
    if (!strcmp(name, "mm_heavy_keys")) { if (value < 0 || value > 1) return set_err("fj_set_option: mm_heavy_keys must be 0 or 1"); o.mm_heavy_keys = (int)value; return 0; }
    if (!strcmp(name, "mm_heavy_outer")) { if (value < 0 || value > 1) return set_err("fj_set_option: mm_heavy_outer must be 0 or 1"); o.mm_heavy_outer = (int)value; return 0; }
    return set_err("fj_set_option: unknown option '%s'", name);
}

}
using namespace fjh;

void fj_set_error_string(const char* msg) { fjh::g_err = msg ? msg : ""; }

extern "C" {

const char* fj_last_error(void) { return fjh::g_err.c_str(); }
const char* fj_version(void) { return "flash_hash_join_amd 0.6 (gfx950)"; }
int fj_abi_version(void) { return FJ_ABI_VERSION; }

int fj_set_option(const char* name, long long value) {
    if (!name) return set_err("fj_set_option: null name");
    return fjh::set_option_value(options(), name, value);
}

long long fj_get_option(const char* name) {
    const Options& o = options();
    if (name && !strcmp(name, "radix_threshold")) return (long long)o.radix_threshold;
    if (name && !strcmp(name, "scalar_hbm_table")) return o.scalar_hbm_table;
    if (name && !strcmp(name, "persistent_min_items")) return o.persistent_min_items;
    if (name && !strcmp(name, "join_wide")) return o.join_wide;
    if (name && !strcmp(name, "plan_target_keys")) return o.plan_target_keys;
    if (name && !strcmp(name, "bloom_variant")) return o.bloom_variant;
    if (name && !strcmp(name, "bloom_auto")) return o.bloom_auto;
    if (name && !strcmp(name, "mat_single_pass")) return o.mat_single_pass;
    if (name && !strcmp(name, "bloom_auto_max_hit_bp")) return o.bloom_auto_max_hit_bp;
    if (name && !strcmp(name, "lab_hooks")) return o.lab_hooks;
    if (name && !strcmp(name, "join_items_target")) return o.join_items_target;
    if (name && !strcmp(name, "mm_heavy_keys")) return o.mm_heavy_keys;
    if (name && !strcmp(name, "mm_heavy_outer")) return o.mm_heavy_outer;
    set_err("fj_get_option: unknown option '%s'", name ? name : "(null)");
    return -1;
}

uint64_t fj_key_mix64(uint64_t key) { return fj_key_mix(key); }
uint64_t fj_key_unmix64(uint64_t mixed) { return fj_key_unmix(mixed); }

int fj_device_count(void) {
    int n = 0;
    if (hipGetDeviceCount(&n) != hipSuccess) return 0;
    return n;
}

int fj_initialize(void) {
    int n = 0;
    hipError_t e = hipGetDeviceCount(&n);
    if (e != hipSuccess || n <= 0) return set_err("fj_initialize: no usable HIP device (%s)", e == hipSuccess ? "device count is 0" : hipGetErrorString(e));
    return 0;
}

fj_ctx* fj_ctx_create(int device) {
    int n = 0;
    hipError_t e = hipGetDeviceCount(&n);
    if (e != hipSuccess || device < 0 || device >= n) { set_err("fj_ctx_create: HIP device %d not available (%d devices)", device, n); return nullptr; }
    DeviceGuard guard(device);
    if (guard.err != hipSuccess) { set_err("fj_ctx_create: hipSetDevice(%d) failed", device); return nullptr; }
    fj_ctx* c = new fj_ctx();
    c->device = device;
    { int ncu = 0; if (hipDeviceGetAttribute(&ncu, hipDeviceAttributeMultiprocessorCount, device) == hipSuccess && ncu > 0) c->num_cus = (u32)ncu; }
    bool ok = hipMalloc((void**)&c->d_sc, sizeof(Scalars)) == hipSuccess &&
              hipHostMalloc((void**)&c->h_sc, sizeof(Scalars), hipHostMallocDefault) == hipSuccess &&
              hipMemset(c->d_sc, 0, sizeof(Scalars)) == hipSuccess;
    for (int i = 0; ok && i < E_NEV; ++i) ok = hipEventCreate(&c->ev[i]) == hipSuccess;
    ok = ok && hipStreamCreateWithFlags(&c->side, hipStreamNonBlocking) == hipSuccess;
    ok = ok && hipEventCreateWithFlags(&c->pk_ev, hipEventDisableTiming) == hipSuccess && hipHostMalloc((void**)&c->pk_h, 67 * 8, hipHostMallocDefault) == hipSuccess;
    if (!ok) { set_err("fj_ctx_create: allocating context scratch failed: %s", hipGetErrorString(hipGetLastError())); delete c; return nullptr; }
    return c;
}

void fj_ctx_destroy(fj_ctx* c) {
    if (!c) return;
    DeviceGuard guard(c->device);
    prepared_free(c);
    for (auto& b : c->bufs) if (b.p) (void)hipFree(b.p);
    for (int i = 0; i < E_NEV; ++i) (void)hipEventDestroy(c->ev[i]);
    if (c->side) (void)hipStreamDestroy(c->side);
    if (c->pk_ev) (void)hipEventDestroy(c->pk_ev);
    if (c->pk_h) (void)hipHostFree(c->pk_h);
    for (void* p : c->stage) if (p) (void)hipHostFree(p);
    if (c->d_sc) (void)hipFree(c->d_sc);
    if (c->h_sc) (void)hipHostFree(c->h_sc);
    delete c;
}

size_t fj_ctx_workspace_bytes(const fj_ctx* c) { return c ? c->ws_bytes : 0; }
void fj_ctx_reserve_cus(fj_ctx* c, unsigned n) { if (c) c->reserve_cus = n; }

int fj_ctx_trim(fj_ctx* c) {
    if (!c) c = host_ctx();
    if (!c) return 0;
    FJ_ENTER(c);
    if (begin_step(c, "fj_ctx_trim")) return 1;
    HIPCHK(hipDeviceSynchronize());
    for (auto& b : c->bufs) if (b.p) { HIPCHK(hipFree(b.p)); b.p = nullptr; b.bytes = 0; }
    c->ws_bytes = 0;
    return 0;
}
int fj_generate_build(fj_ctx* c, uint64_t* d_keys, uint64_t* d_vals, uint64_t first, size_t n, void* stream) {
    FJ_ENTER(c);
    HIPCHK(fj_launch_gen_build(d_keys, d_vals, first, n, (hipStream_t)stream));
    return 0;
}

int fj_generate_probe(fj_ctx* c, uint64_t* d_keys, uint64_t first, size_t n, uint64_t build_total, uint64_t seed,
                      uint32_t hit_bp, uint64_t* h_expected_hits, void* stream) {
    if (build_total == 0) return set_err("fj_generate_probe: build_total must be > 0");
    FJ_ENTER(c);
    hipStream_t s = (hipStream_t)stream;
    HIPCHK(hipMemsetAsync(&c->d_sc->expected, 0, sizeof(unsigned long long), s));
    HIPCHK(fj_launch_gen_probe(d_keys, first, n, build_total, seed, hit_bp, &c->d_sc->expected, s));
    HIPCHK(hipMemcpyAsync(&c->h_sc->expected, &c->d_sc->expected, sizeof(unsigned long long), hipMemcpyDeviceToHost, s));
    HIPCHK(hipStreamSynchronize(s));
    if (h_expected_hits) *h_expected_hits = c->h_sc->expected;
// ... 60 lines not shown
```

Baseline: 118.2.

## Add optional 48-bit packed probe-key chunks for the counting join

Adds a mode in which the last probe-side partition pass writes each key as a 32-bit low word plus a 16-bit middle word. The top bits are implied by the partition index, so the counting join kernels reload and rebuild full keys from the partition number. This cuts probe-side write and read traffic by about a quarter. It also introduces a fallback path when a partition overflows the LDS table, and it applies only to non-materializing joins. The mode sits behind a new option, probe_pack48, which defaults to 0.

```diff
diff --git a/flash_hash_join_amd/csrc/fj_host.h b/flash_hash_join_amd/csrc/fj_host.h
--- a/flash_hash_join_amd/csrc/fj_host.h
+++ b/flash_hash_join_amd/csrc/fj_host.h
@@ -139,6 +139,7 @@
     u32* alloc_word = nullptr; u32* seg_word = nullptr; u32* err_word = nullptr;
     bool in_pk7 = false; u32 in_b0 = 0, in_top_shift = 0;
     bool vals_pos = false;
+    bool pack48 = false;
 };
 
 }
@@ -208,6 +209,7 @@
 #define FJ_HOOK_RESERVE_ALWAYS 16
 #define FJ_HOOK_EMIT_TAGGED 32
 #define FJ_HOOK_EMIT_RETRY_7TH 64
+#define FJ_HOOK_P48_FIRST9 128
 struct Options {
     size_t radix_threshold = 0; int scalar_hbm_table = 0; u32 persistent_min_items = 8192; u32 plan_target_keys = FJ_PART_TARGET_KEYS;
     int bloom_variant = 0, bloom_auto = 1, bloom_auto_max_hit_bp = 2300, mat_single_pass = 1;
@@ -215,6 +217,8 @@
     u32 lab_hooks = 0;
     u32 join_items_target = 2048;
     int mm_heavy_keys = 0;
+    int probe_pack48 = 0;
+    int probe_pack48_last = 0;
     int mm_heavy_outer = 0;
     Options();
 };
@@ -274,7 +278,7 @@
 
 int emit_pending(fj_ctx* c, u64* d_ok, u64* d_ov, size_t cap, hipStream_t s, fj_timings* t);
 int radix_join_tail(fj_ctx* c, int materialize, FjLdsJoinArgs& ja, const Plan& plan, size_t np, const PassIter& pit, hipStream_t s,
-                    fj_timings* t, int evc, u64* out_count, bool* lds_full, int top_bits, SingleOut* so = nullptr);
+                    fj_timings* t, int evc, u64* out_count, bool* lds_full, int top_bits, SingleOut* so = nullptr, bool* pack_toobig = nullptr);
 
 int join_outer(fj_ctx* c, int mode, bool use_radix, const u64* bk, const u64* bv, size_t nb, const u64* pk, size_t np, int top_bits,
                hipStream_t s, fj_timings* t, u64* out_count, u64* d_ok, u64* d_ov, bool rid = false);
diff --git a/flash_hash_join_amd/csrc/fj_internal.h b/flash_hash_join_amd/csrc/fj_internal.h
--- a/flash_hash_join_amd/csrc/fj_internal.h
+++ b/flash_hash_join_amd/csrc/fj_internal.h
@@ -41,7 +41,11 @@
     u32 run_log;
     u32 in_pk7, in_b0, in_top_shift;
     u32 vals_pos;
-};
+    u32 out_pack48;
+};
+
+#define FJ_P48_MID 1024u
+#define FJ_P48_BITS 16
 
 struct FjChunkSet {
     u64* keys;
@@ -139,6 +143,7 @@
     unsigned long long* dbg;
     u32 dbg_flags;
     u32 row_ids;
+    u32 probe_pack48, probe_extra, probe_top_shift;
 };
 hipError_t fj_launch_lds_join(const FjLdsJoinArgs& a, bool materialize, hipStream_t s, u32* next_item = nullptr,
                               u32 persistent_min_items = 8192);
diff --git a/flash_hash_join_amd/csrc/fj_join.hip b/flash_hash_join_amd/csrc/fj_join.hip
--- a/flash_hash_join_amd/csrc/fj_join.hip
+++ b/flash_hash_join_amd/csrc/fj_join.hip
@@ -147,9 +147,10 @@
 constexpr u32 JB_META = 128;
 constexpr u32 JP_META = 512;
 
-template <bool MAT, int NT, bool LIST, bool RID = false>
+template <bool MAT, int NT, bool LIST, bool RID = false, bool P48 = false>
 __global__ __launch_bounds__(NT, 4) void fj_lds_join_kernel(FjLdsJoinArgs a) {
     static_assert(!RID || MAT, "row ids are written by the emitting pass");
+    static_assert(!P48 || (!MAT && LIST), "packed probe chunks: the counting form over chunk lists (the cuckoo kernels' second chance)");
     extern __shared__ __attribute__((aligned(16))) unsigned char smem[];
     JoinHdr* hdr = reinterpret_cast<JoinHdr*>(smem);
     u64* tkeys = reinterpret_cast<u64*>(smem + sizeof(JoinHdr));
@@ -173,7 +174,9 @@
         const u32 npc = (u32)((a.probe.n_flat + FJ_CHUNK - 1) >> FJ_CHUNK_LOG);
         s_lo = (u32)(((u64)slice * npc) / a.nsplit); s_hi = (u32)(((u64)(slice + 1) * npc) / a.nsplit);
     }
-    if (a.build.list) { b0 = a.build.boff[p]; nbc = a.build.boff[p + 1] - b0; }
+    const u32 bp = P48 ? p >> a.probe_extra : p;
+    const u64 top = P48 ? (u64)p << a.probe_top_shift : 0ull;
+    if (a.build.list) { b0 = a.build.boff[bp]; nbc = a.build.boff[bp + 1] - b0; }
     else nbc = (u32)((a.build.n_flat + FJ_CHUNK - 1) >> FJ_CHUNK_LOG);
     if (nbc == 0 || s_lo >= s_hi) {
         if (!MAT && tid == 0) a.part_count[item] = 0;
@@ -249,11 +252,17 @@
     __syncthreads();
     FJ_STAMP(1);
     u64 ka[8], kb[8];
+    FjP48Round ra, rb;
     u32 oka = 0, okb = 0;
     u32 nrounds = (nbatch + CPR - 1) / CPR;
     load_build(0, nbb);
+    if constexpr (P48) {
+        fj_p48_load_round<NT>(a.probe.keys, pm, 0, nbatch, tid, ra, oka);
+        if (nrounds > 1) fj_p48_load_round<NT>(a.probe.keys, pm, 1, nbatch, tid, rb, okb);
+    } else {
     load_round(0, nbatch, ka, oka);
     if (nrounds > 1) load_round(1, nbatch, kb, okb);
+    }
 
     u32 claimed = 0;
     for (u32 bb = 0; bb < nbc; bb += JB_META) {
@@ -337,15 +346,25 @@
             for (u32 i = tid; i < nbatch; i += NT) pm[i] = fj_chunk_entry(a.probe, p0 + pb + i);
             __syncthreads();
             nrounds = (nbatch + CPR - 1) / CPR;
+            if constexpr (P48) {
+                fj_p48_load_round<NT>(a.probe.keys, pm, 0, nbatch, tid, ra, oka);
+                if (nrounds > 1) fj_p48_load_round<NT>(a.probe.keys, pm, 1, nbatch, tid, rb, okb);
+            } else {
             load_round(0, nbatch, ka, oka);
             if (nrounds > 1) load_round(1, nbatch, kb, okb);
+            }
         }
         for (u32 r = 0; r < nrounds; ++r) {
             u64 k[8];
+            if constexpr (P48) { fj_p48_keys(ra, top, k); ra = rb; }
+            else {
 #pragma unroll
             for (int i = 0; i < 8; ++i) { k[i] = ka[i]; ka[i] = kb[i]; }
+            }
             const u32 okm = oka;
             oka = okb;
+            if constexpr (P48) { if (r + 2 < nrounds) fj_p48_load_round<NT>(a.probe.keys, pm, r + 2, nbatch, tid, rb, okb); }
+            else
             if (r + 2 < nrounds) load_round(r + 2, nbatch, kb, okb);
 #pragma unroll
             for (int hgrp = 0; hgrp < 2; ++hgrp) {
@@ -444,8 +463,9 @@
     for (u32 i = tid; i < n; i += NT) cuckoo_insert(tkeys, hdr, ovf[i]);
 }
 
-template <int NT, bool LIST>
+template <int NT, bool LIST, bool P48 = false>
 __global__ __launch_bounds__(NT, 4) void fj_count_join_kernel(FjLdsJoinArgs a) {
+    static_assert(!P48 || LIST, "packed probe chunks come through chunk lists");
     extern __shared__ __attribute__((aligned(16))) unsigned char smem[];
     CkHdr* hdr = reinterpret_cast<CkHdr*>(smem);
     u64* tkeys = reinterpret_cast<u64*>(smem + sizeof(CkHdr));
@@ -467,7 +487,9 @@
         const u32 npc = (u32)((a.probe.n_flat + FJ_CHUNK - 1) >> FJ_CHUNK_LOG);
         s_lo = (u32)(((u64)slice * npc) / a.nsplit); s_hi = (u32)(((u64)(slice + 1) * npc) / a.nsplit);
     }
-    if (a.build.list) { b0 = a.build.boff[p]; nbc = a.build.boff[p + 1] - b0; }
+    const u32 bp = P48 ? p >> a.probe_extra : p;
+    const u64 top = P48 ? (u64)p << a.probe_top_shift : 0ull;
+    if (a.build.list) { b0 = a.build.boff[bp]; nbc = a.build.boff[bp + 1] - b0; }
     else nbc = (u32)((a.build.n_flat + FJ_CHUNK - 1) >> FJ_CHUNK_LOG);
     if (nbc == 0 || s_lo >= s_hi) {
         if (tid == 0) a.part_count[item] = 0;
@@ -531,11 +553,17 @@
     __syncthreads();
     FJ_STAMP(1);
     u64 ka[8], kb[8];
+    FjP48Round ra, rb;
     u32 oka = 0, okb = 0;
     u32 nrounds = (nbatch + CPR - 1) / CPR;
     load_build(0, nbb);
+    if constexpr (P48) {
+        fj_p48_load_round<NT>(a.probe.keys, pm, 0, nbatch, tid, ra, oka);
+        if (nrounds > 1) fj_p48_load_round<NT>(a.probe.keys, pm, 1, nbatch, tid, rb, okb);
+    } else {
     load_round(0, nbatch, ka, oka);
     if (nrounds > 1) load_round(1, nbatch, kb, okb);
+    }
 
     for (u32 bb = 0; bb < nbc; bb += JB_META) {
         if (bb) {
@@ -589,15 +617,25 @@
             for (u32 i = tid; i < nbatch; i += NT) pm[i] = fj_chunk_entry(a.probe, p0 + pb + i);
             __syncthreads();
             nrounds = (nbatch + CPR - 1) / CPR;
+            if constexpr (P48) {
+                fj_p48_load_round<NT>(a.probe.keys, pm, 0, nbatch, tid, ra, oka);
+                if (nrounds > 1) fj_p48_load_round<NT>(a.probe.keys, pm, 1, nbatch, tid, rb, okb);
+            } else {
             load_round(0, nbatch, ka, oka);
             if (nrounds > 1) load_round(1, nbatch, kb, okb);
+            }
         }
         for (u32 r = 0; r < nrounds; ++r) {
             u64 k[8];
+            if constexpr (P48) { fj_p48_keys(ra, top, k); ra = rb; }
+            else {
 #pragma unroll
             for (int i = 0; i < 8; ++i) { k[i] = ka[i]; ka[i] = kb[i]; }
+            }
             const u32 okm = oka;
             oka = okb;
+            if constexpr (P48) { if (r + 2 < nrounds) fj_p48_load_round<NT>(a.probe.keys, pm, r + 2, nbatch, tid, rb, okb); }
+            else
             if (r + 2 < nrounds) load_round(r + 2, nbatch, kb, okb);
             if (a.dbg_flags & 1u) { wave_hits += (u32)__popcll(__ballot((k[0] ^ k[7]) & 1ull)); continue; }
             u64 c1[8], c2[8];
@@ -632,7 +670,7 @@
     }
 }
 
-template <int NT>
+template <int NT, bool P48 = false>
 __global__ __launch_bounds__(NT, 4) void fj_count_join_persistent(FjLdsJoinArgs a, u32* __restrict__ next_item) {
     extern __shared__ __attribute__((aligned(16))) unsigned char smem[];
     CkHdr* hdr = reinterpret_cast<CkHdr*>(smem);
@@ -647,12 +685,15 @@
     constexpr u32 CPL = NT / (FJ_CHUNK / 2), CPR = 4 * CPL, BKPT = 4096 / NT;
     static_assert(JP_META <= NT && JB_META <= NT, "one staged list entry per thread");
 
-    struct Desc { u32 item, b0, nbc, p0, s_lo, s_hi; };
+    struct Desc { u32 item, b0, nbc, p0, s_lo, s_hi, part; };
     auto describe = [&](u32 item) -> Desc {
-        Desc d; d.item = item; d.b0 = 0; d.nbc = 0; d.p0 = 0; d.s_lo = 0; d.s_hi = 0;
+        Desc d; d.item = item; d.b0 = 0; d.nbc = 0; d.p0 = 0; d.s_lo = 0; d.s_hi = 0; d.part = 0;
         if (item >= nitems) return d;
         const uint4 it = a.items[item];
+        if constexpr (P48) { const u32 bp = it.z >> a.probe_extra; d.part = it.z; d.b0 = a.build.boff[bp]; d.nbc = a.build.boff[bp + 1] - d.b0; }
+        else {
         d.b0 = a.build.boff[it.z]; d.nbc = a.build.boff[it.z + 1] - d.b0;
+        }
         d.p0 = 0; d.s_lo = it.x; d.s_hi = it.x + it.y;
         return d;
     };
@@ -707,12 +748,19 @@
         u32* pmn = pm0 + (buf ^ 1) * JP_META; u32* bmn = bm0 + (buf ^ 1) * JB_META;
         const bool lv = live(d);
         u64 ka[8], kb[8];
+        FjP48Round ra, rb;
+        const u64 top = P48 ? (u64)d.part << a.probe_top_shift : 0ull;
         u32 oka = 0, okb = 0;
         u32 nbatch = (d.s_hi - d.s_lo) < JP_META ? (d.s_hi - d.s_lo) : JP_META;
         u32 nrounds = (nbatch + CPR - 1) / CPR;
         if (lv) {
+            if constexpr (P48) {
+                fj_p48_load_round<NT>(a.probe.keys, pm, 0, nbatch, tid, ra, oka);
+                if (nrounds > 1) fj_p48_load_round<NT>(a.probe.keys, pm, 1, nbatch, tid, rb, okb);
+            } else {
             load_round(pm, 0, nbatch, ka, oka);
             if (nrounds > 1) load_round(pm, 1, nbatch, kb, okb);
+            }
             u32 nbb = d.nbc < JB_META ? d.nbc : JB_META;
             for (u32 bb = 0; bb < d.nbc; bb += JB_META) {
                 if (bb) {
@@ -778,15 +826,25 @@
                     if (tid < nbatch) pm[tid] = a.probe.list[d.p0 + pb + tid];
                     __syncthreads();
                     nrounds = (nbatch + CPR - 1) / CPR;
+                    if constexpr (P48) {
+                        fj_p48_load_round<NT>(a.probe.keys, pm, 0, nbatch, tid, ra, oka);
+                        if (nrounds > 1) fj_p48_load_round<NT>(a.probe.keys, pm, 1, nbatch, tid, rb, okb);
+                    } else {
                     load_round(pm, 0, nbatch, ka, oka);
                     if (nrounds > 1) load_round(pm, 1, nbatch, kb, okb);
+                    }
                 }
                 for (u32 r = 0; r < nrounds; ++r) {
                     u64 k[8];
+                    if constexpr (P48) { fj_p48_keys(ra, top, k); ra = rb; }
+                    else {
 #pragma unroll
                     for (int i = 0; i < 8; ++i) { k[i] = ka[i]; ka[i] = kb[i]; }
+                    }
                     const u32 okm = oka;
                     oka = okb;
+                    if constexpr (P48) { if (r + 2 < nrounds) fj_p48_load_round<NT>(a.probe.keys, pm, r + 2, nbatch, tid, rb, okb); }
+                    else
                     if (r + 2 < nrounds) load_round(pm, r + 2, nbatch, kb, okb);
 #pragma unroll
                     for (int h = 0; h < 8; h += 4) {
@@ -1690,6 +1748,7 @@
 hipError_t fj_launch_lds_join(const FjLdsJoinArgs& a, bool materialize, hipStream_t s, u32* next_item, u32 persistent_min_items) {
     const u32 nb = a.items ? a.items_cap : a.nparts * a.nsplit;
     if (materialize) {
+        if (a.probe_pack48) return hipErrorInvalidValue;
         if (a.row_ids && (!a.dedup || a.orig_vals)) return hipErrorInvalidValue;
         if (a.build.list && a.probe.list && a.items && next_item && nb >= persistent_min_items && !a.dbg && !(a.dbg_flags & ~8u)) {
             const u32 ldsp = sizeof(EkHdr) + 2 * S * 8 + 2 * (JP_META + JB_META) * 4 + 16 + S / 8 + CK_OVF * 8;
@@ -1710,16 +1769,17 @@
     } else {
         const u32 lds = sizeof(CkHdr) + S * 8 + (JP_META + JB_META) * 4 + S / 8 + CK_OVF * 8;
         const bool lists = a.build.list && a.probe.list;
+        if (a.probe_pack48 && (!lists || !a.items || a.probe_extra > 1u || a.probe_top_shift > 48u)) return hipErrorInvalidValue;
         if (lists && next_item && nb >= persistent_min_items && !a.dbg && !a.dbg_flags) {
             const u32 ldsp = sizeof(CkHdr) + S * 8 + 2 * (JP_META + JB_META) * 4 + 16 + S / 8 + CK_OVF * 8;
-            auto pk = fj_count_join_persistent<512>;
+            auto pk = a.probe_pack48 ? fj_count_join_persistent<512, true> : fj_count_join_persistent<512>;
             hipError_t e = fj_set_max_lds_once(reinterpret_cast<const void*>(pk), ldsp);
             if (e != hipSuccess) return e;
             const u32 grid = nb < 512 ? nb : 512;
             hipLaunchKernelGGL(pk, dim3(grid), dim3(512), ldsp, s, a, next_item);
             return hipGetLastError();
         }
-        auto kern = lists ? fj_count_join_kernel<512, true> : fj_count_join_kernel<512, false>;
+        auto kern = a.probe_pack48 ? fj_count_join_kernel<512, true, true> : lists ? fj_count_join_kernel<512, true> : fj_count_join_kernel<512, false>;
         hipError_t e = fj_set_max_lds_once(reinterpret_cast<const void*>(kern), lds);
         if (e != hipSuccess) return e;
         hipLaunchKernelGGL(kern, dim3(nb), dim3(512), lds, s, a);
@@ -1759,7 +1819,9 @@
     a.retry_only = 1;
     const u32 nb = a.items ? a.items_cap : a.nparts * a.nsplit;
     const u32 lds = sizeof(JoinHdr) + S * 8 + S + S / 2 + (JP_META + JB_META) * 4;
-    auto kern = (a.build.list && a.probe.list) ? fj_lds_join_kernel<false, 1024, true> : fj_lds_join_kernel<false, 1024, false>;
+    if (a.probe_pack48 && (!a.build.list || !a.probe.list || !a.items || a.probe_extra > 1u || a.probe_top_shift > 48u)) return hipErrorInvalidValue;
+    auto kern = a.probe_pack48 ? fj_lds_join_kernel<false, 1024, true, false, true>
+              : (a.build.list && a.probe.list) ? fj_lds_join_kernel<false, 1024, true> : fj_lds_join_kernel<false, 1024, false>;
     hipError_t e = fj_set_max_lds_once(reinterpret_cast<const void*>(kern), lds);
     if (e != hipSuccess) return e;
     hipLaunchKernelGGL(kern, dim3(nb), dim3(1024), lds, s, a);
diff --git a/flash_hash_join_amd/csrc/fj_joins.hip b/flash_hash_join_amd/csrc/fj_joins.hip
--- a/flash_hash_join_amd/csrc/fj_joins.hip
+++ b/flash_hash_join_amd/csrc/fj_joins.hip
@@ -269,7 +269,7 @@
 }
 
 int radix_join_tail(fj_ctx* c, int materialize, FjLdsJoinArgs& ja, const Plan& plan, size_t np, const PassIter& pit, hipStream_t s,
-                    fj_timings* t, int evc, u64* out_count, bool* lds_full, int top_bits, SingleOut* so) {
+                    fj_timings* t, int evc, u64* out_count, bool* lds_full, int top_bits, SingleOut* so, bool* pack_toobig) {
     ja.nparts = ja.probe.list ? ja.probe.nb : 1u << plan.bits;
     const u64 pchunks = (np + FJ_CHUNK - 1) / FJ_CHUNK;
     void* p;
@@ -306,7 +306,7 @@
         if (c->h_sc->err & FJ_ERR_POOL) return pool_error();
         if (!(c->h_sc->err & (FJ_STAT_DUPS | FJ_STAT_EMIT_RETRY | FJ_ERR_LDS_FULL | FJ_ERR_OUTCAP))) {
             end_plan(c);
-            plan_timings(c, plan, ja.nparts, evc, t);
+            plan_timings(c, plan, ja.nparts >> ja.probe_extra, evc, t);
             t->lds_retries = 0;
             *out_count = c->h_sc->total;
             so->done = true;
@@ -363,6 +363,11 @@
         HIPCHK(hipEventRecord(c->ev[E_JOIN], s));
         if (read_scalars(c, s)) return 1;
         t->lds_retries = 1;
+        if (ja.probe_pack48 && (c->h_sc->err & FJ_STAT_TOOBIG) && !(c->h_sc->err & (FJ_ERR_POOL | FJ_ERR_LDS_FULL))) {
+            end_plan(c);
+            if (pack_toobig) { *pack_toobig = true; return 0; }
+            return set_err("internal error: packed probe chunks met a partition beyond the LDS table and nobody re-runs the join");
+        }
         if ((c->h_sc->err & FJ_STAT_TOOBIG) && !(c->h_sc->err & (FJ_ERR_POOL | FJ_ERR_LDS_FULL))) {
             bool ok = false; u32 redone = 0;
             if (skew_join(c, ja, plan, top_bits, nitems, pit.slot, materialize, s, &ok, &redone, &c->pend)) return 1;
@@ -374,7 +379,7 @@
     }
     if (c->h_sc->err & FJ_ERR_POOL) return pool_error();
     end_plan(c);
-    plan_timings(c, plan, ja.nparts, evc, t);
+    plan_timings(c, plan, ja.nparts >> ja.probe_extra, evc, t);
     if (c->h_sc->err & FJ_ERR_LDS_FULL) { *lds_full = true; return 0; }
     *out_count = c->h_sc->total;
     if (materialize) {
@@ -384,8 +389,21 @@
     return 0;
 }
 
-int join_radix(fj_ctx* c, int materialize, int bloom, const u64* bk, const u64* bv, size_t nb, const u64* pk, size_t np, int top_bits,
-               hipStream_t s, fj_timings* t, u64* out_count, bool* lds_full, SingleOut* so = nullptr, bool rid = false) {
+static bool pack48_plan(const Plan& plan, int materialize, bool rid, int top_bits, size_t np, bool wide, Plan* pp, u32* extra) {
+    const int opt = options().probe_pack48;
+    if (!opt || materialize || rid || plan.bloom_level != 0 || top_bits != 64 || plan.bits < FJ_P48_BITS - 1 || wide) return false;
+    if (opt == 2 && np < ((size_t)1 << 24)) return false;
+    Plan p; p.bits = std::max(plan.bits, FJ_P48_BITS);
+    plan_passes(p, true);
+    if ((options().lab_hooks & FJ_HOOK_P48_FIRST9) && p.npass == 2 && p.fan_log[0] == 8 && p.fan_log[1] == 8) { p.fan_log[0] = 9; p.fan_log[1] = 7; }
+    if (p.npass < 2 || p.npass > 4 || p.fan_log[p.npass - 1] > 8) return false;
+    for (int i = 0; i < p.npass; ++i) if (p.fan_log[i] > FJ_MAX_FAN_LOG || p.fan_log[i] < 1) return false;
+    *pp = p; *extra = (u32)(p.bits - plan.bits);
+    return true;
+}
+
+static int join_radix_once(fj_ctx* c, int materialize, int bloom, const u64* bk, const u64* bv, size_t nb, const u64* pk, size_t np, int top_bits,
+                           hipStream_t s, fj_timings* t, u64* out_count, bool* lds_full, SingleOut* so, bool rid, bool allow_pack, bool* pack_toobig) {
     Plan plan = make_plan(nb, top_bits, bloom != 0);
     *lds_full = false;
     t->sampled_hit_bp = -1;
@@ -413,9 +431,19 @@
         t->sampled_hit_bp = (int)hit_bp;
         if (hit_bp > (u32)options().bloom_auto_max_hit_bp) { pplan = make_plan(nb, top_bits, false); plan.bloom_level = 0; plan.npass = pplan.npass; }
     }
+    bool wide = false;
+    {
+        size_t np_eff0 = np;
+        if (plan.bloom_level > 0) np_eff0 = (size_t)((double)np * (t->sampled_hit_bp >= 0 ? std::min(10000, t->sampled_hit_bp + 1000) : 1500) / 10000.0);
+        wide = wide_join_planned(materialize != 0, nb, np_eff0, plan.bits);
+    }
+    u32 extra = 0;
+    const bool pack = allow_pack && pack48_plan(plan, materialize, rid, top_bits, np, wide, &pplan, &extra);
+    options().probe_pack48_last = pack ? 1 : 0;
     pass_init(pit, 1, rid, np, pplan, top_bits);
     pit.vals_pos = rid;
     pit.want_items = true;
+    pit.pack48 = pack;
     {
         size_t np_eff = np;
         if (plan.bloom_level > 0) np_eff = (size_t)((double)np * (t->sampled_hit_bp >= 0 ? std::min(10000, t->sampled_hit_bp + 1000) : 1500) / 10000.0);
@@ -426,8 +454,21 @@
     HIPCHK(hipEventRecord(c->ev[E_PPART], s));
     ja.avg_build_keys = (u32)std::min<u64>(0xFFFFFFFFu, (u64)nb >> plan.bits);
     ja.row_ids = rid ? 1u : 0u;
-    if (radix_join_tail(c, materialize, ja, plan, np, pit, s, t, evc, out_count, lds_full, top_bits, so)) return 1;
+    if (pack) { ja.probe_pack48 = 1; ja.probe_extra = extra; ja.probe_top_shift = (u32)(64 - pplan.bits); }
+    if (radix_join_tail(c, materialize, ja, plan, np, pit, s, t, evc, out_count, lds_full, top_bits, so, pack_toobig)) return 1;
     if (c->pend.valid) { c->pend.bk = bk; c->pend.bv = bv; c->pend.nb = nb; c->pend.top_bits = top_bits; }
+    return 0;
+}
+
+int join_radix(fj_ctx* c, int materialize, int bloom, const u64* bk, const u64* bv, size_t nb, const u64* pk, size_t np, int top_bits,
+               hipStream_t s, fj_timings* t, u64* out_count, bool* lds_full, SingleOut* so = nullptr, bool rid = false) {
+    bool pack_toobig = false;
+    if (join_radix_once(c, materialize, bloom, bk, bv, nb, pk, np, top_bits, s, t, out_count, lds_full, so, rid, true, &pack_toobig)) return 1;
+    if (!pack_toobig) return 0;
+    const float first_ms = ev_ms(c, E_START, E_JOIN);
+    if (join_radix_once(c, materialize, bloom, bk, bv, nb, pk, np, top_bits, s, t, out_count, lds_full, so, rid, false, nullptr)) return 1;
+    t->total_ms += first_ms;
+    options().probe_pack48_last = 2;
     return 0;
 }
 
diff --git a/flash_hash_join_amd/csrc/fj_lds_table_dev.h b/flash_hash_join_amd/csrc/fj_lds_table_dev.h
--- a/flash_hash_join_amd/csrc/fj_lds_table_dev.h
+++ b/flash_hash_join_amd/csrc/fj_lds_table_dev.h
@@ -6,6 +6,34 @@
     const u64 rem = cs.n_flat - (u64)idx * FJ_CHUNK;
     const u32 cnt = rem >= FJ_CHUNK ? FJ_CHUNK : (u32)rem;
     return ((cnt - 1u) << 24) | idx;
+}
+
+struct FjP48Round { uint4 lo[2]; uint2 mid[2]; };
+template <int NT>
+__device__ __forceinline__ void fj_p48_load_round(const u64* __restrict__ pool, const u32* pm, u32 r, u32 nbatch, u32 tid, FjP48Round& rr, u32& okm) {
+    constexpr u32 CPG = NT / 64;
+    okm = 0;
+#pragma unroll
+    for (int g = 0; g < 2; ++g) {
+        const u32 c = (r * 2u + (u32)g) * CPG + tid / 64u, off = (tid % 64u) * 4u;
+        const u32 e = pm[c < nbatch ? c : nbatch - 1], cnt = c < nbatch ? FJ_LIST_CNT(e) : 0;
+        const unsigned char* slot = reinterpret_cast<const unsigned char*>(pool + (u64)FJ_LIST_ID(e) * FJ_CHUNK);
+        rr.lo[g] = *reinterpret_cast<const uint4*>(slot + off * 4u);
+        rr.mid[g] = *reinterpret_cast<const uint2*>(slot + FJ_P48_MID + off * 2u);
+        const u32 nv = off < cnt ? (cnt - off < 4u ? cnt - off : 4u) : 0u;
+        okm |= ((1u << nv) - 1u) << (4 * g);
+    }
+}
+__device__ __forceinline__ void fj_p48_keys(const FjP48Round& rr, u64 top, u64 (&k)[8]) {
+#pragma unroll
+    for (int g = 0; g < 2; ++g) {
+        const u32 lo[4] = {rr.lo[g].x, rr.lo[g].y, rr.lo[g].z, rr.lo[g].w};
+#pragma unroll
+        for (int m = 0; m < 4; ++m) {
+            const u32 md = (((m & 2) ? rr.mid[g].y : rr.mid[g].x) >> ((m & 1) * 16)) & 0xFFFFu;
+            k[4 * g + m] = top | ((u64)md << 32) | lo[m];
+        }
+    }
 }
 
 __device__ __forceinline__ bool fj_item_slice(const uint4* items, const u32* nitems_dev, u32 nsplit, u64 probe_n_flat, u32 item,
diff --git a/flash_hash_join_amd/csrc/fj_partition.hip b/flash_hash_join_amd/csrc/fj_partition.hip
--- a/flash_hash_join_amd/csrc/fj_partition.hip
+++ b/flash_hash_join_amd/csrc/fj_partition.hip
@@ -33,12 +33,13 @@
 
 enum { M_SLAB_CUR = 0, M_SLAB_REM, M_NEW_BASE, M_NEED, M_NLINES, M_FLUSH, M_SEG, M_NEW_UNITS };
 
-template <int NT, int KPT, int LINE_LOG, bool HAS_VALS, bool FLAT, bool PROBE_SIDE, int RLOG = FJ_RUN_LOG, bool PK7 = false, bool POS = false>
+template <int NT, int KPT, int LINE_LOG, bool HAS_VALS, bool FLAT, bool PROBE_SIDE, int RLOG = FJ_RUN_LOG, bool PK7 = false, bool POS = false, bool P48 = false>
 __global__ __launch_bounds__(NT, 4) void fj_partition_kernel(FjPartArgs a) {
     constexpr u32 T = NT * KPT, LINE = 1u << LINE_LOG, TC = T / FJ_CHUNK, NW = NT / 64, LOS = LINE + FJ_LO_PAD;
     static_assert(T % FJ_CHUNK == 0 && TC <= NT && LINE >= 4 && T + 64 < (1u << 17), "tile geometry");
     static_assert(!PK7 || (!FLAT && KPT % 4 == 0), "wire-format chunks come through chunk lists, four keys per load group");
     static_assert(!POS || (FLAT && HAS_VALS), "positions are made by the first pass over a flat input");
+    static_assert(!P48 || (!HAS_VALS && !FLAT && LINE_LOG == 5), "packed output: keys only, from chunk lists, a 128-B and a 64-B piece per line");
     constexpr bool RUNS = RLOG > 0;
     constexpr u32 RL = (u32)RLOG, RU = 1u << RL;
     const u32 F = 1u << a.fan_log, FM = F - 1;
@@ -210,6 +211,14 @@
             }
             if (c != FJ_DIR_INVALID && c < cap) {
                 const u64 base = (u64)c * FJ_CHUNK + f0;
+                if constexpr (P48) {
+                    unsigned char* slot = reinterpret_cast<unsigned char*>(a.out_keys + (u64)c * FJ_CHUNK);
+                    for (u32 j = 0; j < l; ++j) {
+                        const u64 key = lo_k[b * LOS + j];
+                        reinterpret_cast<u32*>(slot)[f0 + j] = (u32)key;
+                        reinterpret_cast<unsigned short*>(slot + FJ_P48_MID)[f0 + j] = (unsigned short)(key >> 32);
+                    }
+                } else
                 for (u32 j = 0; j < l; ++j) {
                     a.out_keys[base + j] = lo_k[b * LOS + j];
                     if (HAS_VALS) a.out_vals[base + j] = lo_v[b * LOS + j];
@@ -417,6 +426,29 @@
         if (!FLAT && tid < TC) { t_chunk[tid] = mid; t_cnt[tid] = mcnt; }
         const u32 nl = misc[M_NLINES];
         constexpr u32 WK = 2, WLPL = LINE / WK;
+        if constexpr (P48) {
+            constexpr u32 WK4 = 4, WL4 = LINE / WK4;
+            for (u32 e = tid; e < nl * WL4; e += NT) {
+                const u32 l = e / WL4, q = (e % WL4) * WK4;
+                const u64 d = line_desc[l];
+                const u32 dst = (u32)(d >> 32);
+                if (dst != FJ_DIR_INVALID) {
+                    const u32 w = (u32)d, b = w >> 22, lc = (w >> 17) & 31u, sidx = (w & 0x1FFFFu) - 32u;
+                    u64 r[WK4];
+#pragma unroll
+                    for (int i = 0; i < (int)WK4; ++i) {
+                        const u32 vi = q + i;
+                        const u64* sk = vi < lc ? (lo_k + b * LOS + vi) : (tile_k + (sidx + vi));
+                        r[i] = *sk;
+                    }
+                    unsigned char* slot = reinterpret_cast<unsigned char*>(a.out_keys + (u64)(dst >> FJ_CHUNK_LOG) * FJ_CHUNK);
+                    const u32 off = (dst & (FJ_CHUNK - 1)) + q;
+                    *reinterpret_cast<uint4*>(slot + off * 4u) = make_uint4((u32)r[0], (u32)r[1], (u32)r[2], (u32)r[3]);
+                    *reinterpret_cast<uint2*>(slot + FJ_P48_MID + off * 2u) =
+                        make_uint2((FJ_HW1(r[0]) & 0xFFFFu) | (FJ_HW1(r[1]) << 16), (FJ_HW1(r[2]) & 0xFFFFu) | (FJ_HW1(r[3]) << 16));
+                }
+            }
+        } else
         for (u32 e = tid; e < nl * WLPL; e += NT) {
             const u32 l = e / WLPL, q = (e % WLPL) * WK;
             const u64 d = line_desc[l];
@@ -823,11 +855,11 @@
     if (blockIdx.x == 0 && tid == 0) *nalloc = n;
 }
 
-template <int NT, int KPT, int LINE_LOG, bool HAS_VALS, bool FLAT, bool PROBE_SIDE, int RLOG = FJ_RUN_LOG, bool PK7 = false, bool POS = false>
+template <int NT, int KPT, int LINE_LOG, bool HAS_VALS, bool FLAT, bool PROBE_SIDE, int RLOG = FJ_RUN_LOG, bool PK7 = false, bool POS = false, bool P48 = false>
 hipError_t launch_part0(const FjPartArgs& a, u32 grid, hipStream_t s) {
     const u32 F = 1u << a.fan_log;
     const PartLds L = part_lds_layout(NT * KPT, F, 1u << LINE_LOG, HAS_VALS, NT / 64);
-    auto kern = fj_partition_kernel<NT, KPT, LINE_LOG, HAS_VALS, FLAT, PROBE_SIDE, RLOG, PK7, POS>;
+    auto kern = fj_partition_kernel<NT, KPT, LINE_LOG, HAS_VALS, FLAT, PROBE_SIDE, RLOG, PK7, POS, P48>;
     hipError_t e = fj_set_max_lds_once(reinterpret_cast<const void*>(kern), L.total);
     if (e != hipSuccess) return e;
     hipLaunchKernelGGL(kern, dim3(grid), dim3(NT), L.total, s, a);
@@ -897,6 +929,10 @@
 hipError_t fj_launch_partition(const FjPartArgs& a, bool vals, int line_log, u32 grid, hipStream_t s) {
     if (a.shift < 32) return hipErrorInvalidValue;
     if (a.fan_log > FJ_MAX_FAN_LOG || a.slab < (1u << FJ_RUN_LOG) || (a.slab & ((1u << FJ_RUN_LOG) - 1u))) return hipErrorInvalidValue;
+    if (a.out_pack48) {
+        if (vals || !a.in_list || a.in_pk7 || a.fan_log > 8 || line_log != 5 || a.run_log != FJ_RUN_LOG) return hipErrorInvalidValue;
+        return launch_part0<1024, 8, 5, false, false, true, FJ_RUN_LOG, false, false, true>(a, grid < 256 ? grid : 256, s);
+    }
     if (a.in_pk7) {
         if (!a.in_list || a.run_log != FJ_RUN_LOG) return hipErrorInvalidValue;
         if (vals) {
diff --git a/flash_hash_join_amd/csrc/fj_plan.hip b/flash_hash_join_amd/csrc/fj_plan.hip
--- a/flash_hash_join_amd/csrc/fj_plan.hip
+++ b/flash_hash_join_amd/csrc/fj_plan.hip
@@ -167,8 +167,10 @@
     if (it.have_prev && it.in_pk7) { a.in_pk7 = 1; a.in_b0 = it.in_b0; a.in_top_shift = it.in_top_shift; }
     a.shift = (u32)it.used; a.fan_log = (u32)it.plan.fan_log[it.i]; a.slab = fj_slab_for(it.appends); a.run_log = cs.run_log; a.side = (u32)it.side;
     const int line_log = (it.has_vals && it.F > 256) ? 3 : 4;
+    const bool p48 = it.pack48 && it.have_prev && it.i == it.plan.npass - 1;
+    a.out_pack48 = p48 ? 1u : 0u;
     if (ev_cursor) HIPCHK(hipEventRecord(c->ev[E_PK0 + 2 * (*ev_cursor)], s));
-    HIPCHK(fj_launch_partition(a, it.has_vals, line_log, G, s));
+    HIPCHK(fj_launch_partition(a, it.has_vals, p48 ? 5 : line_log, G, s));
     if (ev_cursor) { HIPCHK(hipEventRecord(c->ev[E_PK0 + 2 * (*ev_cursor) + 1], s)); ++*ev_cursor; }
     return 0;
 }
@@ -435,6 +437,8 @@
     if (!strcmp(name, "lab_hooks")) { if (value < 0 || value > 0xFFFF) return set_err("fj_set_option: lab_hooks is a mask of FJ_HOOK_* bits"); o.lab_hooks = (u32)value; return 0; }
     if (!strcmp(name, "join_items_target")) { if (value < 1 || value > (1 << 20)) return set_err("fj_set_option: join_items_target must be 1..1048576"); o.join_items_target = (u32)value; return 0; }
     if (!strcmp(name, "mm_heavy_keys")) { if (value < 0 || value > 1) return set_err("fj_set_option: mm_heavy_keys must be 0 or 1"); o.mm_heavy_keys = (int)value; return 0; }
+    if (!strcmp(name, "probe_pack48")) { if (value < 0 || value > 2) return set_err("fj_set_option: probe_pack48 must be 0..2"); o.probe_pack48 = (int)value; return 0; }
+    if (!strcmp(name, "probe_pack48_last")) return set_err("fj_set_option: probe_pack48_last is read-only");
     if (!strcmp(name, "mm_heavy_outer")) { if (value < 0 || value > 1) return set_err("fj_set_option: mm_heavy_outer must be 0 or 1"); o.mm_heavy_outer = (int)value; return 0; }
     return set_err("fj_set_option: unknown option '%s'", name);
 }
@@ -470,6 +474,8 @@
     if (name && !strcmp(name, "join_items_target")) return o.join_items_target;
     if (name && !strcmp(name, "mm_heavy_keys")) return o.mm_heavy_keys;
     if (name && !strcmp(name, "mm_heavy_outer")) return o.mm_heavy_outer;
+    if (name && !strcmp(name, "probe_pack48")) return o.probe_pack48;
+    if (name && !strcmp(name, "probe_pack48_last")) return o.probe_pack48_last;
     set_err("fj_get_option: unknown option '%s'", name ? name : "(null)");
     return -1;
 }
```

After: 117.0. 0.99x the previous value.
